# thegedge/StereoReconstruction

Measured on AMD Instinct MI355X. Metric: Mdisparity-hypotheses/s (WxHxD), higher is better.
Workload: dtype f64; 1 GPU; C3: synthetic rectified 1920x1080 pair, 256 depth levels, GeodesicWeight r=5; TwoView WTA both directions + cross-check; one pair per GPU; width=1920, height=1080, depth_levels=256, window_radius=5, weights=geodesic, pairs_per_gpu=1, pair_seed_rank0=1592590339, pair_seed_of_rank_r=seed + 0x10000*r, parallelism=single GPU

## Files before the change

profiles/gpu_busy.py:

```python
#!/usr/bin/env python3
import csv
import sys

rows = list(csv.DictReader(open(sys.argv[1])))
ev = sorted((int(r["Start_Timestamp"]), int(r["End_Timestamp"]), r["Kernel_Name"].split("(")[0][-60:]) for r in rows)
if len(sys.argv) > 4:
    hits = [i for i, e in enumerate(ev) if sys.argv[2] in e[2]]
    ev = ev[hits[int(sys.argv[3]) - 1] + 1: hits[int(sys.argv[4]) - 1] + 1]
t0 = ev[0][0]
span = max(e for _, e, _ in ev) - t0
busy, cur, gaps = 0, t0, []
for s, e, n in ev:
    if s > cur:
        gaps.append((s - cur, n))
    busy += max(0, e - max(s, cur))
    cur = max(cur, e)
print(f"dispatches {len(ev)}  span {span/1e6:.3f} ms  busy {busy/1e6:.3f} ms ({100*busy/span:.1f} %)  "
      f"idle {(span-busy)/1e6:.3f} ms in {len(gaps)} gaps")
for g, n in sorted(gaps, reverse=True)[:10]:
    print(f"  gap {g/1e3:8.1f} us  before {n}")
```

stereoreconstruction_amd/csrc/srh_api.hip:

```cpp
#include "srh_internal.hpp"
#include "srh_geom.hpp"
#include "srh_walk.hpp"

#include <algorithm>
#include <cassert>
#include <cstdarg>
#include <cstdio>
#include <cstdlib>
#include <cstring>
#include <map>
#include <mutex>
#include <string>
#include <utility>
#include <limits>
#include <vector>

using namespace srh;

static thread_local char g_err[512] = "";

static int fail(int code, const char *fmt, ...) {
	va_list ap;
	va_start(ap, fmt);
	vsnprintf(g_err, sizeof(g_err), fmt, ap);
	va_end(ap);
	return code;
}

#define HIP_TRY(expr)                                                                   \
	do {                                                                                \
		hipError_t e_ = (expr);                                                         \
		if (e_ != hipSuccess)                                                           \
			return fail(SRH_E_DEVICE, "%s: %s (%s:%d)", #expr, hipGetErrorString(e_), __FILE__, __LINE__); \
	} while (0)

static thread_local bool g_oom = false;
static thread_local size_t g_alloc_limit = 0;

struct PoolBlock { void *p; size_t bytes; int device; };
static std::mutex g_pool_mu;
static std::vector<PoolBlock> g_pool;
static size_t g_pool_bytes = 0, g_pool_cap = (size_t)65536 << 20;
static const size_t POOL_MIN_BYTES = (size_t)4 << 20;

static void pool_flush(int device) {
	std::vector<PoolBlock> out;
	{
		std::lock_guard<std::mutex> g(g_pool_mu);
		for (size_t k = 0; k < g_pool.size();)
			if (device < 0 || g_pool[k].device == device) { out.push_back(g_pool[k]); g_pool_bytes -= g_pool[k].bytes; g_pool[k] = g_pool.back(); g_pool.pop_back(); }
			else ++k;
	}
	int cur = 0;
	const bool have = hipGetDevice(&cur) == hipSuccess;
	for (const PoolBlock &b : out) { (void)hipSetDevice(b.device); (void)hipFree(b.p); }
	if (have) (void)hipSetDevice(cur);
}
static size_t pool_bytes_on(int device) {
	std::lock_guard<std::mutex> g(g_pool_mu);
	size_t b = 0;
	for (const PoolBlock &k : g_pool) if (k.device == device) b += k.bytes;
	return b;
}
static void pool_give(void *p, size_t bytes) {
	if (!p) return;
	int dev = 0;
	if (bytes >= POOL_MIN_BYTES && hipGetDevice(&dev) == hipSuccess) {
		std::lock_guard<std::mutex> g(g_pool_mu);
		if (g_pool_bytes + bytes <= g_pool_cap) { g_pool.push_back({p, bytes, dev}); g_pool_bytes += bytes; return; }
	}
	(void)hipFree(p);
}
static void *pool_take(size_t bytes, size_t *got) {
	int dev = 0;
	if (bytes < POOL_MIN_BYTES || hipGetDevice(&dev) != hipSuccess) return nullptr;
	std::lock_guard<std::mutex> g(g_pool_mu);
	size_t best = g_pool.size();
	for (size_t k = 0; k < g_pool.size(); ++k)
		if (g_pool[k].device == dev && g_pool[k].bytes >= bytes && g_pool[k].bytes <= bytes + bytes/2 &&
		    (best == g_pool.size() || g_pool[k].bytes < g_pool[best].bytes)) best = k;
	if (best == g_pool.size()) return nullptr;
	void *p = g_pool[best].p;
	*got = g_pool[best].bytes;
	g_pool_bytes -= g_pool[best].bytes;
	g_pool[best] = g_pool.back(); g_pool.pop_back();
	return p;
}

static hipError_t dev_alloc(void **p, size_t bytes, size_t *got) {
	if ((*p = pool_take(bytes, got))) return hipSuccess;
	hipError_t e = hipMalloc(p, bytes);
	if (e == hipErrorOutOfMemory) {
		(void)hipGetLastError();
		int dev = 0;
		if (hipGetDevice(&dev) == hipSuccess && pool_bytes_on(dev)) { pool_flush(dev); e = hipMalloc(p, bytes); }
	}
	if (e != hipSuccess) { *p = nullptr; (void)hipGetLastError(); return e; }
	*got = bytes;
	return hipSuccess;
}

template <class T>
struct DevBuf {
	T *p = nullptr;
	size_t n = 0, block = 0;
	DevBuf() = default;
	DevBuf(DevBuf &&o) noexcept { *this = std::move(o); }
	DevBuf &operator=(DevBuf &&o) noexcept {
		assert(!p && "a held block is released, not overwritten");
		p = o.p; n = o.n; block = o.block;
		o.p = nullptr; o.n = o.block = 0;
		return *this;
	}
	operator T *() const { return p; }
	T *operator->() const { return p; }
	size_t bytes() const { return block; }
	hipError_t alloc(size_t count) {
		void *q = nullptr;
		size_t got = 0;
		const hipError_t e = dev_alloc(&q, count*sizeof(T), &got);
		if (e == hipSuccess) { p = (T *)q; n = got/sizeof(T); block = got; }
		return e;
	}
	int ensure(size_t need) {
		if (n >= need) return SRH_OK;
		if (p) { (void)hipDeviceSynchronize(); release(); }
		if (g_alloc_limit && need*sizeof(T) > g_alloc_limit) {
			g_oom = true;
			return fail(SRH_E_DEVICE, "band buffer of %zu bytes refused (debug_alloc_limit_mb)", need*sizeof(T));
		}
		const hipError_t e = alloc(need);
		if (e == hipErrorOutOfMemory) g_oom = true;
		if (e != hipSuccess) return fail(SRH_E_DEVICE, "hipMalloc of a %zu-byte band buffer: %s", need*sizeof(T), hipGetErrorString(e));
		return SRH_OK;
	}
	void release() { pool_give(p, block); p = nullptr; n = block = 0; }
	void free() { if (p) (void)hipFree(p); p = nullptr; n = block = 0; }
};

struct BandBuffers {
	DevBuf<double> wbuf;
	DevBuf<double> cost;
	DevBuf<double> tnum;
	DevBuf<double> pconst;
	DevBuf<PixRange> prange;
	DevBuf<uint32_t> cflag;
	DevBuf<uint8_t> stpl;
	DevBuf<uint32_t> tileflag;
	DevBuf<int32_t> lcount;
	DevBuf<uint32_t> lcand;
	DevBuf<uint32_t> lrowinfo;
	DevBuf<int32_t> lmeta;
	DevBuf<uint32_t> mvs_wdesc;
	DevBuf<int32_t> mvs_nwin;
	template <class F> void each(F f) {
		f(wbuf); f(cost); f(tnum); f(pconst); f(prange); f(cflag); f(stpl); f(tileflag);
		f(lcount); f(lcand); f(lrowinfo); f(lmeta); f(mvs_wdesc); f(mvs_nwin);
	}
	size_t bytes() { size_t b = 0; each([&](auto &x) { b += x.bytes(); }); return b; }
	void release() { each([](auto &x) { x.release(); }); }
	void free() { each([](auto &x) { x.free(); }); }
};

struct ViewHost {
	int w = 0, h = 0;
	bool present = false;
	DevBuf<uint32_t> rgba;
	DevBuf<uint8_t>  mask;
	DevBuf<double>   gray, gray_tv, depth;
	DevBuf<double>   edges;
	DevBuf<uint8_t>  full;
	int              full_r = 0;
	DevBuf<double>   tvp;   bool tvp_valid = false;
	DevBuf<double>   geo5;  bool geo5_valid = false;
	bool             geo5_denied = false;
	DevBuf<uint8_t>  fullp; int fullp_r = 0;
	DevBuf<uint8_t>  fulls; int fulls_r = 0;
	DevBuf<double>   grayp; bool grayp_valid = false;
	DevBuf<uint8_t>  fullsp; int fullsp_r = 0;
	uint8_t   list_mode[SRH_MAX_VIEWS] = {0};
	DevBuf<uint32_t> act;
	std::vector<uint32_t> act_row, act_host;
	std::vector<uint8_t> hmask;
	bool act_valid = false;
	srh_camera cam;
	DevBuf<int32_t> wta_xy;
	DevBuf<double>  wta_cost;
	int wta_flags = 0, wta_oth = -1;
	DevBuf<double> peaks; int peaks_k = 0;
	DevBuf<double> mrf;
	DevBuf<double> sgm;
};

struct ProfEntry { double ms = 0; int64_t n = 0; };
struct PendingEvt { std::string name; hipEvent_t a, b; };

#ifndef SRH_MVS_SLOTS
#define SRH_MVS_SLOTS 2
#endif
struct MvsSlot {
	hipStream_t stream = nullptr;
	hipEvent_t ev = nullptr, done = nullptr;
	int *h_maxc = nullptr;
	bool own_buffers = false;
	BandBuffers band;
	DevBuf<Counters> d_cnt; DevBuf<int> d_span;
	bool pending = false;
	int view = -1, nneigh = 0, y0 = 0, y1 = 0, cmax = 0;
	int32_t neigh[SRH_MAX_NEIGH] = {0};
	srh_params p;
};

struct srh_context {
	int device = 0;
	hipStream_t own_stream = nullptr;
	hipStream_t stream = nullptr;
	ViewHost views[SRH_MAX_VIEWS];
	DevBuf<ViewDev> d_views;
	DevBuf<int32_t> d_slots;
	int32_t slots_host[SRH_MAX_VIEWS] = {0}; int slots_n = 0;
	DevBuf<Counters> d_cnt;
	DevBuf<int> d_span;
	BandBuffers band;
	hipStream_t mrf_stream[SRH_MAX_VIEWS] = { nullptr };
	void *mrf_host = nullptr;
	DevBuf<double> mrf_peaks;
	DevBuf<double> mrf;
	int mrf_w = 0, mrf_h = 0, mrf_k = 0;
	DevBuf<double> mvsgm;
	int mvsgm_w = 0, mvsgm_h = 0, mvsgm_k = 0;
	double *mvsgm_host = nullptr;
	DevBuf<double> tvmrf;
	DevBuf<double> tvmrf_costs;
	int tvmrf_w = 0, tvmrf_h = 0, tvmrf_l = 0;
	bool tvmrf_own_costs = false;
	DevBuf<double> tvsgm;
	DevBuf<double> tvsgm_costs;
	int tvsgm_w = 0, tvsgm_h = 0, tvsgm_l = 0;
	bool tvsgm_own_costs = false;
	int geodma = 1;
	int tscan_bound = 1;
	int tscan = 1;
	int strip = 1;
	int num_cus = 256;
	bool force_walk = false;
	int list_count_pass = 0;
	int list_cmax_hint = 0;
	int list_smax_hint = 0;
	int mvs_cmax_hint = 0;
	hipStream_t side_stream = nullptr;
	hipEvent_t side_go = nullptr, side_done = nullptr;
	int mvs_async = 1;
	MvsSlot mvs_slot[SRH_MVS_SLOTS];
	int mvs_turn = 0, mvs_last = -1;
	bool in_settle = false;
	int mvs_staged = 1;
	bool list_rows = true;
	void *comm = nullptr; int comm_ranks = 0, comm_rank = 0;
	size_t wbuf_budget = (size_t)32768 << 20;
	size_t budget_cap = 0;
	size_t budget_used = 0;
	size_t mem_limit = 0;
	int debug_trace = 0;
	size_t alloc_limit = 0;
	const volatile int *cancel = nullptr;
	srh_progress_fn progress = nullptr;
	void *user = nullptr;
	bool profiling = false;
	bool force_generic = false;
 	bool use_fused = false;
	int arith = 3;
	struct TvDefer { Counters *host = nullptr; int *span = nullptr; bool queued = false, strip = false, cert = false, lists = false, guessed = false;
	                 int cmax = 0, smax = 0, ref = -1, oth = -1; };
	TvDefer tv_defer[2];
	TvDefer *defer = nullptr;
	struct TvSlot {
		hipStream_t stream = nullptr;
		hipEvent_t go = nullptr, done = nullptr;
		DevBuf<Counters> d_cnt; DevBuf<int> d_span;
		BandBuffers band;
	} tv_slot;
	int tv_overlap = 1;
	int f32_form = 0;
	int rows_masked = 1;
	int side_weights = 1;
	int cert_form = 1;
	bool force_dense = false;
	std::map<std::string, ProfEntry> prof;
	std::vector<PendingEvt> pending;
	srh_stats stats;
	bool last_fused = false;
	int filter_invalid = 0;
	int filter_gap_width = 2;
	int filter_replay = 0;
	int cost_kind = SRH_COST_NCC;
	int sad_dense = 0;
	int wta_outputs = 0;
	DevBuf<double> fuse_result, fuse_scratch;
	FuseCloud fuse_out = { nullptr, nullptr, nullptr, nullptr, nullptr, nullptr };
	int64_t fuse_n = 0;
	bool fuse_valid = false;
};

static bool cancelled(srh_context *c) { return c->cancel && *c->cancel; }
static void progress(srh_context *c, int step, const char *stage) { if (c->progress) c->progress(step, stage, c->user); }

static int drain_profile(srh_context *c) {
	for (auto &p : c->pending) {
		float ms = 0;
		HIP_TRY(hipEventSynchronize(p.b));
		HIP_TRY(hipEventElapsedTime(&ms, p.a, p.b));
		ProfEntry &e = c->prof[p.name];
		e.ms += ms; e.n += 1;
		hipEventDestroy(p.a); hipEventDestroy(p.b);
	}
	c->pending.clear();
	return SRH_OK;
}

struct Scope {
	srh_context *c; PendingEvt p; bool on;
	Scope(srh_context *c_, const char *name) : c(c_), on(c_->profiling) {
		if (on) {
			p.name = name;
			hipEventCreate(&p.a); hipEventCreate(&p.b);
			hipEventRecord(p.a, c->stream);
		}
	}
	~Scope() {
		if (on) {
			hipEventRecord(p.b, c->stream);
			c->pending.push_back(p);
			if (c->pending.size() > 4096) drain_profile(c);
		}
	}
};


static int mvs_settle_all(srh_context *c);
static int check_slot(srh_context *c, int slot, bool must_exist, bool settle = true) {
	if (!c) return fail(SRH_E_INVALID, "null context");
	if (settle) { const int rc = mvs_settle_all(c); if (rc) return rc; }
	if (slot < 0 || slot >= SRH_MAX_VIEWS) return fail(SRH_E_INVALID, "view slot %d out of range [0,%d)", slot, SRH_MAX_VIEWS);
	if (must_exist && !c->views[slot].present) return fail(SRH_E_INVALID, "view slot %d has no image", slot);
	return SRH_OK;
}

static int check_params(const srh_params *p) {
	if (!p) return fail(SRH_E_INVALID, "null params");
	if (p->num_depth_levels < 2) return fail(SRH_E_INVALID, "num_depth_levels %d < 2", p->num_depth_levels);
	if (p->window_radius < 1 || p->window_radius > 15) return fail(SRH_E_INVALID, "window_radius %d outside [1,15]", p->window_radius);
	if (!(p->image_scale > 0)) return fail(SRH_E_INVALID, "image_scale must be > 0");
	if (p->weight_kind != SRH_WEIGHT_ADAPTIVE && p->weight_kind != SRH_WEIGHT_GEODESIC)
		return fail(SRH_E_INVALID, "weight_kind %d unknown", p->weight_kind);
	return SRH_OK;
}

extern "C" int srh_hw_queues_requested(void) {
	const char *s = getenv("GPU_MAX_HW_QUEUES");
	const int n = s ? atoi(s) : 0;
	return n > 0 ? n : 4;
}

extern "C" int srh_abi_version(void) { return SRH_ABI_VERSION; }
extern "C" const char *srh_build_id(void) {
	return
#include "build_id.inc"
	;
}
extern "C" const char *srh_last_error(void) { return g_err; }

extern "C" int srh_device_count(int *count) {
	if (!count) return fail(SRH_E_INVALID, "null count");
	int n = 0;
	hipError_t e = hipGetDeviceCount(&n);
	if (e != hipSuccess) { (void)hipGetLastError(); n = 0; }
	*count = n;
	return SRH_OK;
}

extern "C" void srh_params_twoview_defaults(srh_params *p) {
	memset(p, 0, sizeof(*p));
	p->min_depth = 10; p->max_depth = 100; p->num_depth_levels = 100;
	p->window_radius = 5;
	p->image_scale = 1.0;
	p->weight_kind = SRH_WEIGHT_GEODESIC;
	p->geodesic_iters = 3; p->geodesic_sigma = 50.0; p->geodesic_init = 1000000.0;
	p->adaptive_color_sigma = 10.0;
	p->weight_cutoff = 1e-10;
	p->bad_ret = 1000; p->max_color_diff = 120;
	p->second_best_factor = 0.95; p->wta_margin = 1e-10; p->inconsistency_thresh = 1;
	p->peak_threshold = 0.95;
	p->cross_check_threshold = 1.0;
	p->neighbour_min_dot = 0.2;
	p->top_k = 9; p->num_neighbours = 3;
}

extern "C" void srh_params_mvs_defaults(srh_params *p) {
	srh_params_twoview_defaults(p);
	p->window_radius = 2;
}

extern "C" int srh_cert_bound(const srh_params *p, int mvs, srh_cert_info *out) {
	if (!p || !out) return fail(SRH_E_INVALID, "null argument");
// ... 110 lines not shown
	if (plane_normal) {
		const Vec3 n = normalized(load3(plane_normal));
		c.plane_normal[0] = n.x; c.plane_normal[1] = n.y; c.plane_normal[2] = n.z;
		c.plane_dist = plane_dist;
		c.refr_index = refr_index;
	}
	c.is_refractive = (!near_zero(c.refr_index - 1) && !near_zero(c.plane_dist));
	*out = c;
	return SRH_OK;
}

extern "C" int srh_camera_from_p(const double Pin[12], const double dist[5], const double plane_normal[3],
                                 double plane_dist, double refr_index, srh_camera *out)
{
	if (!Pin || !out) return fail(SRH_E_INVALID, "null argument");
	const double n2 = (Pin[8]*Pin[8] + Pin[9]*Pin[9]) + Pin[10]*Pin[10];
	if (!(n2 > 0)) return fail(SRH_E_INVALID, "projection matrix with a zero third row");
	double P[3][4];
	for (int i = 0; i < 3; ++i) for (int j = 0; j < 4; ++j) P[i][j] = Pin[i*4 + j] / n2;
	double A[3][3], tau[3];
	for (int i = 0; i < 3; ++i) for (int j = 0; j < 3; ++j) A[i][j] = P[2 - j][i];
	for (int k = 0; k < 3; ++k) {
		const double c0 = A[k][k];
		double tailSq = 0;
		for (int i = k + 1; i < 3; ++i) tailSq += A[i][k]*A[i][k];
		double beta;
		if (tailSq <= std::numeric_limits<double>::min()) {
			tau[k] = 0; beta = c0;
			for (int i = k + 1; i < 3; ++i) A[i][k] = 0;
		} else {
			beta = sqrt(c0*c0 + tailSq);
			if (c0 >= 0) beta = -beta;
			for (int i = k + 1; i < 3; ++i) A[i][k] /= (c0 - beta);
			tau[k] = (beta - c0)/beta;
		}
		A[k][k] = beta;
		for (int j = k + 1; j < 3; ++j) {
			double tmp = 0;
			for (int i = k + 1; i < 3; ++i) tmp += A[i][k]*A[i][j];
			tmp += A[k][j];
			A[k][j] -= tau[k]*tmp;
			for (int i = k + 1; i < 3; ++i) A[i][j] -= tau[k]*A[i][k]*tmp;
		}
	}
	double Q[3][3] = {{1, 0, 0}, {0, 1, 0}, {0, 0, 1}};
	for (int k = 2; k >= 0; --k)
		for (int j = k; j < 3; ++j) {
			double tmp = 0;
			for (int i = k + 1; i < 3; ++i) tmp += A[i][k]*Q[i][j];
			tmp += Q[k][j];
			Q[k][j] -= tau[k]*tmp;
			for (int i = k + 1; i < 3; ++i) Q[i][j] -= tau[k]*A[i][k]*tmp;
		}
	double K[9], R[9];
	for (int i = 0; i < 3; ++i)
		for (int j = 0; j < 3; ++j) {
			R[i*3 + j] = Q[j][2 - i];
			K[i*3 + j] = (2 - j <= 2 - i) ? A[2 - j][2 - i] : 0.0;
		}
	for (int axis = 2; axis >= 0; --axis) {
		if (K[axis*3 + axis] < 0) {
			K[axis*3 + axis] = -K[axis*3 + axis];
			for (int j = 0; j < 3; ++j) R[axis*3 + j] = -R[axis*3 + j];
		}
		if (K[axis*3 + 2] < 0) K[axis*3 + 2] = -K[axis*3 + 2];
	}
	srh_camera tmpc;
	const double I3[9] = {1, 0, 0, 0, 1, 0, 0, 0, 1}, z3[3] = {0, 0, 0};
	int rc = srh_camera_from_krt(K, I3, z3, nullptr, nullptr, 0.0, 1.0, &tmpc);
	if (rc) return rc;
	const Vec3 t = matvec(tmpc.Kinv, v3(P[0][3], P[1][3], P[2][3]));
	const double tt[3] = { t.x, t.y, t.z };
	return srh_camera_from_krt(K, R, tt, dist, plane_normal, plane_dist, refr_index, out);
}

extern "C" int srh_mvs_neighbours(int nviews, const srh_camera *cams, const srh_params *p,
                                  int32_t *neigh, int32_t *count)
{
	if (nviews < 0 || !cams || !p || !neigh || !count) return fail(SRH_E_INVALID, "null argument");
	if (p->num_neighbours < 0) return fail(SRH_E_INVALID, "num_neighbours < 0");
	for (int v = 0; v < nviews; ++v) {
		std::vector<std::pair<double, int>> nearViews;
		for (int v2 = 0; v2 < nviews; ++v2) {
			if (v == v2) continue;
			if (fabs(dot(load3(cams[v].pdir), load3(cams[v2].pdir))) > p->neighbour_min_dot) {
				const Vec3 d = load3(cams[v].C) - load3(cams[v2].C);
				nearViews.push_back(std::make_pair(dot(d, d), v2));
			}
		}
		size_t end = nearViews.size();
		if ((size_t)p->num_neighbours < nearViews.size()) {
			std::sort(nearViews.begin(), nearViews.end());
			end = (size_t)p->num_neighbours;
		}
		for (size_t k = 0; k < end; ++k) neigh[(size_t)v*p->num_neighbours + k] = nearViews[k].second;
		count[v] = (int32_t)end;
	}
	return SRH_OK;
}

extern "C" int srh_create(int device, srh_context **out) {
	if (!out) return fail(SRH_E_INVALID, "null out");
	*out = nullptr;
	int n = 0;
	hipError_t e = hipGetDeviceCount(&n);
	if (e != hipSuccess || n <= 0) {
		(void)hipGetLastError();
		return fail(SRH_E_NO_DEVICE, "no HIP device available (%s); this library has no CPU path",
		            e != hipSuccess ? hipGetErrorString(e) : "device count 0");
	}
	if (device < 0 || device >= n) return fail(SRH_E_INVALID, "device ordinal %d outside [0,%d)", device, n);
	HIP_TRY(hipSetDevice(device));
	srh_context *c = new srh_context();
	c->device = device;
	memset(&c->stats, 0, sizeof(c->stats));
	{ int cus = 0; if (hipDeviceGetAttribute(&cus, hipDeviceAttributeMultiprocessorCount, device) == hipSuccess && cus > 0) c->num_cus = cus; }
	hipError_t e2 = hipStreamCreateWithFlags(&c->own_stream, hipStreamNonBlocking);
	if (e2 != hipSuccess) { delete c; return fail(SRH_E_DEVICE, "hipStreamCreate: %s", hipGetErrorString(e2)); }
	c->stream = c->own_stream;
	if (c->d_views.alloc(SRH_MAX_VIEWS) != hipSuccess || c->d_slots.alloc(SRH_MAX_VIEWS) != hipSuccess ||
	    c->d_cnt.alloc(1) != hipSuccess || c->d_span.alloc(4) != hipSuccess) {
		srh_destroy(c);
		return fail(SRH_E_DEVICE, "allocating the context tables failed");
	}
	if (hipMemsetAsync(c->d_views, 0, sizeof(ViewDev)*SRH_MAX_VIEWS, c->stream) != hipSuccess ||
	    hipMemsetAsync(c->d_cnt, 0, sizeof(Counters), c->stream) != hipSuccess ||
	    hipStreamSynchronize(c->stream) != hipSuccess) {
		srh_destroy(c);
		return fail(SRH_E_DEVICE, "initialising the context tables failed");
	}
	*out = c;
	return SRH_OK;
}

static void free_view(ViewHost &v) {
	if (v.rgba || v.gray || v.edges || v.tvp || v.geo5) (void)hipDeviceSynchronize();
	v.rgba.release(); v.mask.release(); v.gray.release(); v.gray_tv.release(); v.depth.release(); v.edges.release();
	v.full.release(); v.fulls.release(); v.grayp.release(); v.fullsp.release(); v.tvp.release(); v.geo5.release(); v.fullp.release(); v.act.release(); v.peaks.release(); v.mrf.release(); v.sgm.release();
	v.wta_xy.release(); v.wta_cost.release();
	v = ViewHost();
}

extern "C" void srh_destroy(srh_context *c) {
	if (!c) return;
	hipSetDevice(c->device);
	if (c->own_stream) hipStreamSynchronize(c->own_stream);
	for (MvsSlot &S : c->mvs_slot) {
		if (S.stream) { hipStreamSynchronize(S.stream); }
		S.pending = false;
	}
	if (c->side_stream) { hipStreamSynchronize(c->side_stream); hipStreamDestroy(c->side_stream); }
	if (c->side_go) hipEventDestroy(c->side_go);
	if (c->side_done) hipEventDestroy(c->side_done);
	drain_profile(c);
	for (MvsSlot &S : c->mvs_slot) {
		if (S.stream) hipStreamDestroy(S.stream);
		if (S.ev) hipEventDestroy(S.ev);
		if (S.done) hipEventDestroy(S.done);
		if (S.h_maxc) hipHostFree(S.h_maxc);
		S.band.release(); S.d_cnt.release(); S.d_span.release();
	}
	for (auto &v : c->views) free_view(v);
	c->d_views.release(); c->d_slots.release(); c->d_cnt.release(); c->d_span.release();
	(void)hipDeviceSynchronize();
	(void)hipStreamSynchronize(c->stream);
	if (c->tv_slot.stream) (void)hipStreamSynchronize(c->tv_slot.stream);
	c->band.release();
	for (auto &d : c->tv_defer) { if (d.host) hipHostFree(d.host); if (d.span) hipHostFree(d.span); }
	{
		srh_context::TvSlot &T = c->tv_slot;
		if (T.stream) { hipStreamSynchronize(T.stream); hipStreamDestroy(T.stream); }
		if (T.go) hipEventDestroy(T.go);
		if (T.done) hipEventDestroy(T.done);
		T.d_cnt.release(); T.d_span.release(); T.band.release();
	}
	c->mrf.release(); c->mrf_peaks.release(); c->mvsgm.release();
	c->tvmrf.release(); c->tvmrf_costs.release();
	c->tvsgm.release(); c->tvsgm_costs.release();
	c->fuse_result.release(); c->fuse_scratch.release();
	for (int i = 0; i < SRH_MAX_VIEWS; ++i) if (c->mrf_stream[i]) hipStreamDestroy(c->mrf_stream[i]);
	if (c->mrf_host) hipHostFree(c->mrf_host);
	if (c->mvsgm_host) hipHostFree(c->mvsgm_host);
	if (c->comm) (void)rccl_comm_destroy(c->comm);
	if (c->own_stream) hipStreamDestroy(c->own_stream);
	delete c;
}

extern "C" int srh_set_stream(srh_context *c, void *hip_stream) {
	if (!c) return fail(SRH_E_INVALID, "null context");
	{ const int rc = mvs_settle_all(c); if (rc) return rc; }
	c->stream = hip_stream ? (hipStream_t)hip_stream : c->own_stream;
	return SRH_OK;
}

extern "C" int srh_set_hooks(srh_context *c, const volatile int *cancel, srh_progress_fn progress_fn, void *user) {
	if (!c) return fail(SRH_E_INVALID, "null context");
	c->cancel = cancel; c->progress = progress_fn; c->user = user;
	return SRH_OK;
}

static void release_band_buffers(srh_context *c);

extern "C" int srh_set_option(srh_context *c, const char *name, long value) {
	if (!c || !name) return fail(SRH_E_INVALID, "null argument");
	{ const int rc = mvs_settle_all(c); if (rc) return rc; }
	if (!strcmp(name, "list_rows")) { c->list_rows = value != 0; return SRH_OK; }
	if (!strcmp(name, "list_count_pass")) { c->list_count_pass = value != 0; return SRH_OK; }
	if (!strcmp(name, "force_generic")) { c->force_generic = value != 0; c->force_walk = value == 2; return SRH_OK; }
	if (!strcmp(name, "fused")) { c->use_fused = value != 0; return SRH_OK; }
	if (!strcmp(name, "arith")) {
		if (value < 0 || value > 3) return fail(SRH_E_INVALID, "arith must be 0 (exact), 1 (fma), 2 (f32) or 3 (certified fma)");
		c->arith = (int)value; return SRH_OK;
	}
	if (!strcmp(name, "force_dense")) { c->force_dense = value != 0; return SRH_OK; }
	if (!strcmp(name, "cert_form")) {
		if (value != 1 && value != 2) return fail(SRH_E_INVALID, "cert_form must be 1 (one-pass) or 2 (two fused sweeps)");
		c->cert_form = (int)value; return SRH_OK;
	}
	if (!strcmp(name, "strip")) {
		if (value != 0 && value != 1 && value != 4 && value != 8) return fail(SRH_E_INVALID, "strip must be 0, 1, 4 or 8");
		c->strip = (int)value; return SRH_OK;
	}
	if (!strcmp(name, "mvs_staged")) { c->mvs_staged = value != 0; return SRH_OK; }
	if (!strcmp(name, "mvs_async")) { c->mvs_async = value != 0; return SRH_OK; }
	if (!strcmp(name, "band_budget_mb")) {
		if (value < 1) return fail(SRH_E_INVALID, "band_budget_mb must be >= 1");
		c->wbuf_budget = (size_t)value << 20;
		c->budget_cap = 0;
		return SRH_OK;
	}
	if (!strcmp(name, "mem_limit_mb")) { c->mem_limit = value > 0 ? (size_t)value << 20 : 0; return SRH_OK; }
	if (!strcmp(name, "debug_trace")) { c->debug_trace = (int)value; return SRH_OK; }
	if (!strcmp(name, "band_pool_mb")) {
		if (value < 0) return fail(SRH_E_INVALID, "band_pool_mb must be >= 0");
		{ std::lock_guard<std::mutex> g(g_pool_mu); g_pool_cap = (size_t)value << 20; }
		if (value == 0) pool_flush(-1);
		return SRH_OK;
	}
	if (!strcmp(name, "debug_alloc_limit_mb")) {
		c->alloc_limit = g_alloc_limit = value > 0 ? (size_t)value << 20 : 0;
		for (MvsSlot &S : c->mvs_slot) if (S.stream) HIP_TRY(hipStreamSynchronize(S.stream));
		if (c->side_stream) HIP_TRY(hipStreamSynchronize(c->side_stream));
		HIP_TRY(hipStreamSynchronize(c->stream));
		release_band_buffers(c);
		return SRH_OK;
	}
	if (!strcmp(name, "tv_overlap")) { c->tv_overlap = value != 0; return SRH_OK; }
	if (!strcmp(name, "filter_invalid")) {
		if (value < 0 || value > 3) return fail(SRH_E_INVALID, "filter_invalid must be 0..3 (SRH_FILTER_GAPS | SRH_FILTER_MEDIAN)");
		c->filter_invalid = (int)value; return SRH_OK;
	}
	if (!strcmp(name, "filter_gap_width")) { c->filter_gap_width = (int)value; return SRH_OK; }
	if (!strcmp(name, "filter_replay")) { c->filter_replay = value != 0; return SRH_OK; }
	if (!strcmp(name, "cost")) {
		if (value != SRH_COST_NCC && value != SRH_COST_SAD) return fail(SRH_E_INVALID, "cost must be 0 (SRH_COST_NCC) or 1 (SRH_COST_SAD)");
		c->cost_kind = (int)value; return SRH_OK;
	}
	if (!strcmp(name, "sad_dense")) { c->sad_dense = value != 0; return SRH_OK; }
	if (!strcmp(name, "wta_outputs")) {
		if (value != 0 && value != SRH_WTA_WINNERS && value != (SRH_WTA_WINNERS | SRH_WTA_COSTS))
			return fail(SRH_E_INVALID, "wta_outputs must be 0, 1 (SRH_WTA_WINNERS) or 3 (SRH_WTA_WINNERS | SRH_WTA_COSTS): the costs are those of the kept winners");
		c->wta_outputs = (int)value; return SRH_OK;
	}
	if (!strcmp(name, "tscan")) { c->tscan = value != 0; return SRH_OK; }
	if (!strcmp(name, "tscan_bound")) { c->tscan_bound = value != 0; return SRH_OK; }
	if (!strcmp(name, "geodma")) { c->geodma = value != 0; return SRH_OK; }
	if (!strcmp(name, "f32_form")) { c->f32_form = value != 0; return SRH_OK; }
	if (!strcmp(name, "rows_masked")) { c->rows_masked = (int)value; return SRH_OK; }
	if (!strcmp(name, "side_weights")) { c->side_weights = value != 0; return SRH_OK; }
	if (!strcmp(name, "debug_mvs_cmax_hint")) { c->mvs_cmax_hint = value > 0 ? (int)((value + 7) & ~7L) : 0; return SRH_OK; }
#ifdef SRH_EXPERIMENT
	if (!strcmp(name, "exp_repeat")) { exp_set((int)value, -1); return SRH_OK; }
	if (!strcmp(name, "exp_lds_pad")) { exp_set(-1, (int)value); return SRH_OK; }
	if (!strcmp(name, "exp_scan_mode")) { exp_set_scan((int)value); return SRH_OK; }
	if (!strcmp(name, "exp_walk_mode")) { exp_set_walk((int)value); return SRH_OK; }
	if (!strcmp(name, "exp_rows_mode")) { exp_set_rows((int)value); return SRH_OK; }
#endif
	return fail(SRH_E_INVALID, "unknown option '%s'", name);
}

extern "C" int srh_synchronize(srh_context *c) {
	if (!c) return fail(SRH_E_INVALID, "null context");
	HIP_TRY(hipSetDevice(c->device));
	{ const int rc = mvs_settle_all(c); if (rc) return rc; }
	HIP_TRY(hipStreamSynchronize(c->stream));
	return SRH_OK;
}

static int view_install(srh_context *c, int slot, int w, int h, const void *rgba, const void *mask, const uint8_t *hmask,
                        hipMemcpyKind kind, const srh_camera *cam)
{
	if (w <= 0 || h <= 0 || (size_t)w*h > ((size_t)1 << 30)) return fail(SRH_E_INVALID, "bad image size %dx%d", w, h);
	if (!rgba || !cam) return fail(SRH_E_INVALID, "null rgba / camera");
	if (w > SRH_MAX_VIEW_DIM || h > SRH_MAX_VIEW_DIM) return fail(SRH_E_UNSUPPORTED, "view of %dx%d: a side above %d (SRH_MAX_VIEW_DIM)", w, h, SRH_MAX_VIEW_DIM);
	HIP_TRY(hipSetDevice(c->device));
	ViewHost &v = c->views[slot];
	const size_t n = (size_t)w*h;
	if (!v.present || v.w != w || v.h != h) {
		HIP_TRY(hipStreamSynchronize(c->stream));
		free_view(v);
		HIP_TRY(v.rgba.alloc(n));
		HIP_TRY(v.mask.alloc(n));
		HIP_TRY(v.gray.alloc(n));
		HIP_TRY(v.gray_tv.alloc(n));
		HIP_TRY(v.depth.alloc(n));
		HIP_TRY(v.edges.alloc(4*n));
// ... 215 lines not shown
	if (!dev_ptr) return fail(SRH_E_INVALID, "null output");
	*dev_ptr = c->views[slot].depth;
	return SRH_OK;
}

static int check_wta_outputs(srh_context *c, int slot, bool costs) {
	const ViewHost &v = c->views[slot];
	if (!v.wta_flags) return fail(SRH_E_INVALID, "view slot %d holds no WTA outputs (option \"wta_outputs\" off, no WTA pass since the upload, or its depth map came from the MRF stage)", slot);
	if (costs && !(v.wta_flags & SRH_WTA_COSTS)) return fail(SRH_E_INVALID, "view slot %d kept the winners only (wta_outputs = 1): no cost planes", slot);
	return SRH_OK;
}

extern "C" int srh_view_wta_outputs_state(srh_context *c, int slot, int *flags, int *oth_slot) {
	int rc = check_slot(c, slot, true); if (rc) return rc;
	const ViewHost &v = c->views[slot];
	if (flags) *flags = v.wta_flags;
	if (oth_slot) *oth_slot = v.wta_flags ? v.wta_oth : -1;
	return SRH_OK;
}

extern "C" int srh_view_wta_outputs_device(srh_context *c, int slot, void **win_xy, void **runner_xy, void **min_cost, void **second_cost) {
	int rc = check_slot(c, slot, true); if (rc) return rc;
	if ((rc = check_wta_outputs(c, slot, min_cost || second_cost))) return rc;
	const ViewHost &v = c->views[slot];
	const size_t n = (size_t)v.w*v.h;
	if (win_xy) *win_xy = v.wta_xy;
	if (runner_xy) *runner_xy = v.wta_xy + 2*n;
	if (min_cost) *min_cost = v.wta_cost;
	if (second_cost) *second_cost = v.wta_cost + n;
	return SRH_OK;
}

extern "C" int srh_view_wta_outputs(srh_context *c, int slot, int32_t *win_xy, int32_t *runner_xy, double *min_cost, double *second_cost) {
	int rc = check_slot(c, slot, true); if (rc) return rc;
	if ((rc = check_wta_outputs(c, slot, min_cost || second_cost))) return rc;
	HIP_TRY(hipSetDevice(c->device));
	const ViewHost &v = c->views[slot];
	const size_t n = (size_t)v.w*v.h;
	if (win_xy) HIP_TRY(hipMemcpyAsync(win_xy, v.wta_xy, 2*n*sizeof(int32_t), hipMemcpyDeviceToHost, c->stream));
	if (runner_xy) HIP_TRY(hipMemcpyAsync(runner_xy, v.wta_xy + 2*n, 2*n*sizeof(int32_t), hipMemcpyDeviceToHost, c->stream));
	if (min_cost) HIP_TRY(hipMemcpyAsync(min_cost, v.wta_cost, n*sizeof(double), hipMemcpyDeviceToHost, c->stream));
	if (second_cost) HIP_TRY(hipMemcpyAsync(second_cost, v.wta_cost + n, n*sizeof(double), hipMemcpyDeviceToHost, c->stream));
	HIP_TRY(hipStreamSynchronize(c->stream));
	return SRH_OK;
}

extern "C" int srh_view_depth_copy_to_device(srh_context *c, int slot, void *dst_dev, size_t dst_bytes) {
	int rc = check_slot(c, slot, true); if (rc) return rc;
	if (!dst_dev) return fail(SRH_E_INVALID, "null destination");
	HIP_TRY(hipSetDevice(c->device));
	const ViewHost &v = c->views[slot];
	if (dst_bytes < (size_t)v.w*v.h*sizeof(double))
		return fail(SRH_E_INVALID, "destination of %zu bytes is smaller than the %dx%d depth map of slot %d", dst_bytes, v.w, v.h, slot);
	HIP_TRY(hipMemcpyAsync(dst_dev, v.depth, (size_t)v.w*v.h*sizeof(double), hipMemcpyDeviceToDevice, c->stream));
	return SRH_OK;
}

extern "C" int srh_view_depth_copy_from_device(srh_context *c, int slot, const void *src_dev, size_t src_bytes) {
	int rc = check_slot(c, slot, true); if (rc) return rc;
	if (!src_dev) return fail(SRH_E_INVALID, "null source");
	HIP_TRY(hipSetDevice(c->device));
	const ViewHost &v = c->views[slot];
	if (src_bytes < (size_t)v.w*v.h*sizeof(double))
		return fail(SRH_E_INVALID, "source of %zu bytes is smaller than the %dx%d depth map of slot %d", src_bytes, v.w, v.h, slot);
	HIP_TRY(hipMemcpyAsync(v.depth, src_dev, (size_t)v.w*v.h*sizeof(double), hipMemcpyDeviceToDevice, c->stream));
	return SRH_OK;
}

static size_t held_band_bytes(srh_context *c) {
	size_t b = c->band.bytes() + c->tv_slot.band.bytes();
	for (MvsSlot &S : c->mvs_slot) b += S.band.bytes();
	for (const ViewHost &v : c->views) b += v.geo5.bytes();
	return b;
}

static size_t band_budget(srh_context *c) {
	size_t b = c->wbuf_budget;
	if (c->budget_cap && b > c->budget_cap) b = c->budget_cap;
	size_t free_b = 0, total_b = 0;
	if (hipMemGetInfo(&free_b, &total_b) == hipSuccess) {
		size_t avail = free_b + held_band_bytes(c) + pool_bytes_on(c->device);
		if (c->mem_limit && avail > c->mem_limit) avail = c->mem_limit;
		if (b > avail/4) b = avail/4;
	} else (void)hipGetLastError();
	if (b < ((size_t)1 << 20)) b = (size_t)1 << 20;
	c->budget_used = b;
	return b;
}

static void release_band_buffers(srh_context *c) {
	pool_flush(c->device);
	c->band.free();
	for (MvsSlot &S : c->mvs_slot) S.band.free();
	c->tv_slot.band.free();
	for (ViewHost &v : c->views)
		if (v.geo5) { v.geo5.free(); v.geo5_valid = false; v.geo5_denied = true; }
}

template <class F>
static int with_thinner_bands(srh_context *c, F body) {
	for (;;) {
		g_oom = false;
		g_alloc_limit = c->alloc_limit;
		const int rc = body();
		if (rc != SRH_E_DEVICE || !g_oom) return rc;
		g_oom = false;
		const size_t used = c->budget_used;
		if (used <= ((size_t)1 << 20)) return rc;
		for (MvsSlot &S : c->mvs_slot) if (S.stream) (void)hipStreamSynchronize(S.stream);
		if (c->side_stream) (void)hipStreamSynchronize(c->side_stream);
		(void)hipStreamSynchronize(c->stream);
		if (c->tv_slot.stream) (void)hipStreamSynchronize(c->tv_slot.stream);
		release_band_buffers(c);
		c->budget_cap = used/2;
		c->stats.band_retries += 1;
	}
}

static int band_rows(srh_context *c, int W, int H, int T) {
	size_t rows = band_budget(c) / ((size_t)T*sizeof(double)*(size_t)W);
	if (rows < 1) rows = 1;
	if (rows > (size_t)H) rows = H;
	return (int)rows;
}

static int read_back(srh_context *c, void *host, const void *dev, size_t bytes) {
	HIP_TRY(hipMemcpyAsync(host, dev, bytes, hipMemcpyDeviceToHost, c->stream));
	HIP_TRY(hipStreamSynchronize(c->stream));
	return SRH_OK;
}

static int fetch_counters(srh_context *c, int used_dense) {
	Counters h;
	int rc;
	if ((rc = read_back(c, &h, c->d_cnt, sizeof(h)))) return rc;
	c->stats.n_pixels = (int64_t)h.n_pixels;
	c->stats.n_eval = (int64_t)h.n_eval;
	c->stats.n_eval_device = (int64_t)h.n_eval_device;
	c->stats.scan_tiles_template = (int64_t)h.scan_tiles_template;
	c->stats.scan_tiles_walked = (int64_t)h.scan_tiles_walked;
	c->stats.scan_tiles_bound = (int64_t)h.scan_tiles_bound;
	c->stats.mvs_waves_staged = (int64_t)h.mvs_waves_staged;
	c->stats.mvs_waves_listed = (int64_t)h.mvs_waves_listed;
	c->stats.used_dense_path = used_dense;
	c->stats.used_fused_kernel = c->last_fused ? 1 : 0;
#ifdef SRH_PROFILE_PHASES
	{
		unsigned long long g[8];
		geodesic_phases_fetch(g);
		if (g[7])
			fprintf(stderr, "[srh prof] geodesic kernel: %llu waves, cycles per wave: staging %.0f  sweeps %.0f  exp %.0f  rows out %.0f  pconst: first sweep %.0f  second sweep %.0f  rest %.0f\n",
			        g[7], (double)g[0]/g[7], (double)g[1]/g[7], (double)g[2]/g[7], (double)g[4]/g[7], (double)g[5]/g[7], (double)g[6]/g[7], (double)g[3]/g[7]);
	}
	if (h.dbg_waves && h.dbg_blocks && h.dbg_phase[3] && h.strip_ticket) {
		const double nw = (double)h.dbg_waves, nt = (double)h.dbg_blocks/nw;
		fprintf(stderr, "[srh dbg] strip: waves %llu, tiles/wave %.1f (%.1f with phase 2), cycles/wave %.0f | per tile: ticket %.0f  own requests %.0f  barriers %.0f  setup %.0f  "
		        "block loops %.0f  p2 lists %.0f  p2 blocks %.0f  p2 singles %.0f\n", h.dbg_waves, nt, (double)h.dbg_cycles/nw, (double)h.dbg_total_cycles/nw,
		        h.dbg_phase[0]/nw/nt, h.dbg_phase[1]/nw/nt, h.dbg_phase[2]/nw/nt, h.dbg_phase[3]/nw/nt, h.dbg_phase[4]/nw/nt,
		        h.dbg_phase[5]/nw/nt, h.dbg_phase[6]/nw/nt, h.dbg_phase[7]/nw/nt);
		static const char *names[8] = { "ticket", "own requests", "barriers", "setup", "block loops", "p2 lists", "p2 blocks", "p2 singles" };
		const int nwv = h.dbg_wave[8*4 + 4] ? 8 : 4;
		for (int k = 0; k < 8; ++k) {
			fprintf(stderr, "[srh dbg]   %-13s by wave:", names[k]);
			for (int w = 0; w < nwv; ++w) fprintf(stderr, " %8.0f", h.dbg_wave[8*k + w]/((double)h.dbg_blocks/nwv));
			fprintf(stderr, "\n");
		}
	} else
	if (h.dbg_waves && !c->last_fused)
		fprintf(stderr, "[srh dbg] dense: waves %llu, cycles/wave %.0f, fast blocks/wave %.1f, cycles/fast block %.0f\n",
		        h.dbg_waves, (double)h.dbg_total_cycles/h.dbg_waves, (double)h.dbg_blocks/h.dbg_waves,
		        h.dbg_blocks ? (double)h.dbg_cycles/h.dbg_blocks : 0.0);
	if (h.dbg_waves && !c->last_fused && !h.strip_ticket)
		fprintf(stderr, "[srh dbg] phases/wave: stage_w %.0f prologue %.0f sync %.0f stage_rt %.0f compute %.0f tail %.0f\n",
		        (double)h.dbg_phase[0]/h.dbg_waves, (double)h.dbg_phase[1]/h.dbg_waves, (double)h.dbg_phase[2]/h.dbg_waves,
		        (double)h.dbg_phase[3]/h.dbg_waves, (double)h.dbg_phase[4]/h.dbg_waves, (double)h.dbg_phase[5]/h.dbg_waves);
	if (h.dbg_waves && c->last_fused)
		fprintf(stderr, "[srh dbg] fused: %llu tiles, %llu with select-form work, %llu pixels with an unusable tap of their own\n",
		        h.dbg_waves, h.n_listed, h.n_slots);
	if (h.dbg_waves && c->last_fused)
		fprintf(stderr, "[srh dbg] fused, role wave cycles/tile: A geometry %.0f  B accept %.0f  C stage %.0f  D prologue %.0f  E1 blocks %.0f  E2 general %.0f  F wta %.0f  barriers %.0f | other waves: blocks %.0f barriers %.0f total %.0f\n",
		        (double)h.dbg_phase[0]/h.dbg_waves, (double)h.dbg_phase[1]/h.dbg_waves, (double)h.dbg_phase[2]/h.dbg_waves,
		        (double)h.dbg_phase[3]/h.dbg_waves, (double)h.dbg_phase[4]/h.dbg_waves, (double)h.dbg_phase[5]/h.dbg_waves,
		        (double)h.dbg_phase[6]/h.dbg_waves, (double)h.dbg_phase[7]/h.dbg_waves,
		        (double)h.dbg_cycles/(3.0*h.dbg_waves), (double)h.dbg_blocks/(3.0*h.dbg_waves), (double)h.dbg_total_cycles/(3.0*h.dbg_waves));
	if (h.dbg_phase[6] && !c->last_fused)
		fprintf(stderr, "[srh dbg] rows: tasks %llu fast %llu, rows/pixel %.2f, slots/px %.1f, wave iterations %llu all-fast %llu\n",
		        h.dbg_phase[6], h.dbg_phase[7], (double)h.dbg_cycles/(double)h.n_pixels, 8.0*h.dbg_phase[6]/(double)h.n_pixels,
		        h.dbg_blocks, h.dbg_total_cycles);
	if (h.dbg_phase[6] && !c->last_fused && h.dbg_wave[8])
		fprintf(stderr, "[srh dbg] rows cost kernel, wave tiles %llu: cycles per tile: staging %.0f  constants %.0f  phase 1 %.0f  p2 blocks %.0f  p2 singles %.0f | tiles with blocks %llu (%llu blocks: %.0f cycles per such tile), with singles %llu (%llu singles: %.0f cycles per such tile); rounds if the tile's tasks were dealt to its 64 lanes: %.2f per tile\n",
		        h.dbg_wave[8], (double)h.dbg_wave[0]/h.dbg_wave[8], (double)h.dbg_wave[1]/h.dbg_wave[8], (double)h.dbg_wave[2]/h.dbg_wave[8],
		        (double)h.dbg_wave[3]/h.dbg_wave[8], (double)h.dbg_wave[4]/h.dbg_wave[8], h.dbg_wave[9], h.dbg_wave[10],
		        h.dbg_wave[9] ? (double)h.dbg_wave[3]/h.dbg_wave[9] : 0.0, h.dbg_wave[11], h.dbg_wave[12], h.dbg_wave[11] ? (double)h.dbg_wave[4]/h.dbg_wave[11] : 0.0, (double)h.dbg_wave[13]/h.dbg_wave[8]);
#endif
	return SRH_OK;
}

static void run_weights(srh_context *c, int ref, int W, const srh_params &p, int by, int nr, size_t wstride,
                        double *pconst = nullptr, bool wimg = false) {
	if (p.weight_kind == SRH_WEIGHT_GEODESIC && !c->force_generic && wimg && c->geodma && p.window_radius == 5 && !c->views[ref].geo5_denied) {
		ViewHost &v = c->views[ref];
		bool ok = true;
		if (!v.geo5) {
			if (v.geo5.alloc(geo5_doubles(v.w, v.h)) != hipSuccess) ok = false;
			v.geo5_valid = false;
		}
		if (ok && !v.geo5_valid) {
			Scope s(c, "geo5_planes_kernel");
			launch_geo5_planes(c->stream, v.edges, v.gray_tv, v.mask, v.w, v.h, v.geo5);
			v.geo5_valid = true;
		}
		if (ok) {
			Scope s(c, "geodesic_dma_kernel");
			if (launch_geodesic_dma(c->stream, c->d_views, ref, W, v.geo5, p, by, nr, c->band.wbuf, pconst, c->num_cus)) return;
		}
	}
	if (p.weight_kind == SRH_WEIGHT_GEODESIC && !c->force_generic) {
		Scope s(c, "geodesic_reg_kernel");
		if (launch_geodesic_reg(c->stream, c->d_views, ref, W, c->views[ref].edges, p, by, nr, c->band.wbuf, wstride, pconst, wimg)) return;
	}
	if (p.weight_kind == SRH_WEIGHT_ADAPTIVE && !c->force_generic) {
		Scope s(c, "adaptive_reg_kernel");
		if (launch_adaptive_reg(c->stream, c->d_views, ref, W, p, by, nr, c->band.wbuf, wstride, pconst, wimg)) return;
	}
	Scope s(c, "weights_kernel");
	launch_weights(c->stream, c->d_views, ref, W, p, by, nr, c->band.wbuf, wstride, pconst, wimg);
}

static bool rig_is_row_aligned(const srh_camera &a, const srh_camera &b, double *fx_bx) {
	if (a.is_distorted || b.is_distorted || a.is_refractive || b.is_refractive) return false;
	for (int k = 0; k < 9; ++k) if (fabs(a.R[k] - b.R[k]) > 1e-13) return false;
	for (int k = 3; k < 9; ++k) if (fabs(a.K[k] - b.K[k]) > 1e-9*(1.0 + fabs(a.K[k]))) return false;
	if (fabs(a.K[1]) > 1e-12 || fabs(b.K[1]) > 1e-12 || fabs(a.K[3]) > 1e-12 || fabs(a.K[6]) > 1e-12 || fabs(a.K[7]) > 1e-12)
		return false;
	const Vec3 d = load3(b.C) - load3(a.C);
	const Vec3 bc = matvec(a.R, d);
	const double len = norm(bc);
	if (!(len > 0) || fabs(bc.y) > 1e-12*len || fabs(bc.z) > 1e-12*len) return false;
	*fx_bx = fabs(b.K[0]*bc.x);
	return true;
}

static int ensure_wta_planes(srh_context *c, int ref, int oth) {
	ViewHost &v = c->views[ref];
	if (!c->wta_outputs) { v.wta_flags = 0; return SRH_OK; }
	const size_t n = (size_t)v.w*v.h;
	if (v.wta_flags == c->wta_outputs && v.wta_oth == oth) return SRH_OK;
	if (!v.wta_xy) HIP_TRY(v.wta_xy.alloc(4*n));
	if ((c->wta_outputs & SRH_WTA_COSTS) && !v.wta_cost) HIP_TRY(v.wta_cost.alloc(2*n));
	HIP_TRY(hipMemsetAsync(v.wta_xy, 0xff, 4*n*sizeof(int32_t), c->stream));
	if (c->wta_outputs & SRH_WTA_COSTS) launch_fill(c->stream, v.wta_cost, 2*n, __builtin_inf());
	v.wta_flags = c->wta_outputs; v.wta_oth = oth;
	return SRH_OK;
}

static void estimate_list_capacity(const srh_camera &rc, const srh_camera &oc, int W, int H, int OW, int OH,
                                   const srh_params &p, int y0, int y1, int &cmax, int &smax, bool mvs = false)
{
	(void)H;
	const int D = p.num_depth_levels, NL = D < 9 ? D : 9, GX = 13, GY = 9;
	const Vec3 normal = load3(rc.pdir);
	long best_len = 0, best_rows = 0;
	for (int gy = 0; gy < GY; ++gy)
		for (int gx = 0; gx < GX; ++gx) {
			const int x = (int)((gx*(long)(W - 1))/(GX - 1)), y = y0 + (int)((gy*(long)(y1 - y0 - 1))/(GY - 1));
			const Ray ray = cam_unproject(rc, (x + 0.5)/p.image_scale, (y + 0.5)/p.image_scale);
			long len = 0, rows = 0;
			bool have = false;
			int px = 0, py = 0;
			for (int k = 0; k < NL; ++k) {
				const int d = NL > 1 ? (int)(((long)k*(D - 1))/(NL - 1)) : 0;
				Vec3 point = load3(rc.C);
				if (!point_from_depth(ray, normal, depth_from_label(p, mvs, d), point)) continue;
				if (!cam_project(oc, point)) continue;
				const double cxd = fmin(fmax(point.x*p.image_scale, -64.0), (double)OW + 64.0);
				const double cyd = fmin(fmax(point.y*p.image_scale, -64.0), (double)OH + 64.0);
				if (!(cxd == cxd) || !(cyd == cyd)) continue;
				const int ix = (int)cxd, iy = (int)cyd;
				if (have) {
					const long dx = labs((long)ix - px), dy = labs((long)iy - py);
					len += dx > dy ? dx : dy;
					rows += dy;
				}
				have = true; px = ix; py = iy;
			}
			if (len > best_len) best_len = len;
			if (rows > best_rows) best_rows = rows;
		}
	if (best_rows > SRH_ROWS_NR) best_rows = SRH_ROWS_NR;
	long cm = best_len + best_len/8 + (mvs ? 0 : (best_len < D - 1 ? best_len : D - 1)) + 40;
	if (cm > 65520) cm = 65520;
	cmax = (int)((cm + 7) & ~7L);
	long sm = cmax + 8*(best_rows + 2) + 32;
	if (sm > 65528) sm = 65528;
	smax = (int)((sm + 7) & ~7L);
}

static int ensure_tvp(srh_context *c, ViewHost &v) {
	if (!v.tvp) HIP_TRY(v.tvp.alloc(padded_size(v.w, v.h)));
	if (!v.tvp_valid) {
		Scope s(c, "padded_plane_kernel");
		launch_padded_plane(c->stream, v.gray_tv, v.w, v.h, v.tvp);
		v.tvp_valid = true;
	}
	return SRH_OK;
}

static int ensure_fulls(srh_context *c, ViewHost &v, int R) {
	if (v.fulls_r == R) return SRH_OK;
	if (!v.fulls) HIP_TRY(v.fulls.alloc((size_t)v.w*v.h));
	Scope s(c, "sad_full_window_kernel");
	launch_sad_full_window(c->stream, v.mask, v.w, v.h, R, v.fulls);
	v.fulls_r = R;
	v.fullsp_r = 0;
	return SRH_OK;
}

static int ensure_full(srh_context *c, ViewHost &v, int R) {
	if (v.full_r == R) return SRH_OK;
	Scope s(c, "full_window_kernel");
	uint32_t *stat = (uint32_t *)(v.full + full_stat_offset((size_t)v.w*v.h));
	HIP_TRY(hipMemsetAsync(stat, 0, 2*sizeof(uint32_t), c->stream));
	launch_full_window(c->stream, v.gray_tv, v.w, v.h, R, v.full, stat);
	v.full_r = R;
	return SRH_OK;
}

static int ensure_sad_planes(srh_context *c, ViewHost &v, int R) {
	int rc;
	if ((rc = ensure_tvp(c, v))) return rc;
	if (!v.grayp) HIP_TRY(v.grayp.alloc(padded_size(v.w, v.h)));
	if (!v.grayp_valid) {
		Scope s(c, "padded_gray_kernel");
		launch_padded_gray(c->stream, v.gray, v.mask, v.w, v.h, v.grayp);
		v.grayp_valid = true;
	}
	if ((rc = ensure_fulls(c, v, R))) return rc;
	if (!v.fullsp) HIP_TRY(v.fullsp.alloc(padded_size(v.w, v.h)));
	if (v.fullsp_r != R) {
		Scope s(c, "padded_bytes_kernel");
		launch_padded_bytes(c->stream, v.fulls, v.w, v.h, v.fullsp);
		v.fullsp_r = R;
	}
	return SRH_OK;
}


struct TvPlan { bool dense = false; int cstride = 0; bool fused = false; };
struct TvLists { int cmax = 0, smax = 0; bool rows_mode = false, guessed = false, cert = false; size_t lrows = 0; };
struct TvDense { int cstride = 0; bool strip = false, cert = false, tscan = false; size_t rows = 0; int lanes = 8; };

struct TvPass {
	srh_context *c = nullptr;
	int ref = 0, oth = 0;
	const srh_params *p = nullptr;
	int W = 0, H = 0, y0 = 0, y1 = 0, R = 0, T = 0;
	size_t budget = 0;
	bool sad = false;
	int32_t *wout = nullptr;

	size_t rows_per_band(size_t bytes) const;
	void winner_costs(int by, int nr, bool wimg_layout) const;
	TvPlan plan() const;
	int run_fused(bool &stands) const;
	int lists_prepare(TvLists &S) const;
	int lists_rows_band(const TvLists &S, int by, int nr) const;
	int lists_pass(TvLists &S) const;
	int run_lists(bool cert_ok, srh_context::TvDefer *defer) const;
	int dense_prepare(TvDense &D) const;
	void dense_band_inputs(const TvDense &D, int by, int nr) const;
	int dense_cost_pass(const TvDense &D, int by, int nr, int arith, bool raw) const;
	int run_dense(TvDense &D) const;
	int run_walk() const;
};

static int tv_pass_init(TvPass &P, srh_context *c, int ref, int oth, const srh_params *p, int y0, int y1) {
	if (ref == oth) return fail(SRH_E_INVALID, "ref and other view are the same slot");
	const ViewHost &L = c->views[ref], &Rv = c->views[oth];
	if (L.w != Rv.w || L.h != Rv.h)
		return fail(SRH_E_INVALID, "TwoViewStereo needs equal-sized views (%dx%d vs %dx%d; twoviewstereo.cpp:116-119)",
		            L.w, L.h, Rv.w, Rv.h);
	HIP_TRY(hipSetDevice(c->device));
	P.c = c; P.ref = ref; P.oth = oth; P.p = p;
	P.W = L.w; P.H = L.h;
	P.y0 = y0 < 0 ? 0 : y0;
	P.y1 = (y1 <= 0 || y1 > P.H) ? P.H : y1;
	P.R = p->window_radius;
	P.T = (2*P.R + 1)*(2*P.R + 1);
	P.sad = c->cost_kind == SRH_COST_SAD;
	if (P.y1 > P.y0) P.budget = band_budget(c);
	return SRH_OK;
}

size_t TvPass::rows_per_band(size_t bytes) const {
	return std::min(std::max<size_t>(budget/(bytes*(size_t)W), 1), (size_t)(y1 - y0));
}

void TvPass::winner_costs(int by, int nr, bool wimg_layout) const {
	if (!wout || !(c->wta_outputs & SRH_WTA_COSTS)) return;
	Scope s(c, "twoview_winner_costs_kernel");
	double *mc = c->views[ref].wta_cost;
	launch_twoview_winner_costs(c->stream, c->d_views, ref, oth, W, *p, sad, by, nr, c->band.wbuf, wimg_layout,
	                            wout, mc, mc + (size_t)W*H);
}

static int redo_capacity(size_t band_pixels) { return (int)std::min<size_t>(band_pixels, (size_t)1 << 30); }

static double disparity_span(const srh_params &p, double fx_bx) {
	return fx_bx*p.image_scale*fabs(1.0/p.min_depth - 1.0/p.max_depth);
}

TvPlan TvPass::plan() const {
	const ViewHost &L = c->views[ref], &Rv = c->views[oth];
	TvPlan pl;
	pl.dense = !c->force_generic && (!sad || c->sad_dense) && (R == 5 || R == 2);
	double fx_bx = 0;
	if (pl.dense && !rig_is_row_aligned(L.cam, Rv.cam, &fx_bx)) {
		const bool pinhole = !L.cam.is_distorted && !Rv.cam.is_distorted && !L.cam.is_refractive && !Rv.cam.is_refractive;
		if (c->force_dense && pinhole) fx_bx = (double)(W + 8)/disparity_span(*p, 1.0);
		else pl.dense = false;
	}
	if (!pl.dense) return pl;
	const double span = disparity_span(*p, fx_bx);
	if (!(p->min_depth > 0) || !(p->max_depth > 0) || !(span < 4096.0)) pl.dense = false;
	else pl.cstride = (((int)ceil(span) + 3) + 7) & ~7;
	if (pl.cstride > W + 8) pl.cstride = (W + 8 + 7) & ~7;
	if (sad && pl.dense && pl.cstride + SRH_WTILE > strip_chunk_columns()) pl.dense = false;
	pl.fused = pl.dense && !sad && c->use_fused && (c->arith == 0 || c->arith == 3) &&
	           p->num_depth_levels <= SRH_FUSED_MAXC && span + 1.0 <= (double)SRH_FUSED_MAXC;
	return pl;
}

int TvPass::run_fused(bool &stands) const {
	int rc;
	stands = false;
	HIP_TRY(hipMemsetAsync(c->d_cnt, 0, sizeof(Counters), c->stream));
	if ((rc = c->band.tnum.ensure((size_t)p->num_depth_levels))) return rc;
	{ Scope s(c, "pinhole_label_table_kernel");
	  launch_pinhole_label_table(c->stream, c->d_views, ref, *p, false, c->band.tnum); }
	const int rows = (int)rows_per_band((size_t)T*sizeof(double));
	if ((rc = c->band.wbuf.ensure(wbuf_doubles(W, rows, T)))) return rc;
	bool launched = true;
	for (int by = y0; by < y1 && launched; by += rows) {
		if (cancelled(c)) return fail(SRH_E_CANCELLED, "cancelled");
		const int nr = std::min(rows, y1 - by);
		run_weights(c, ref, W, *p, by, nr, SRH_WTILE);
		Scope s(c, "twoview_fused_kernel");
		launched = launch_twoview_fused(c->stream, c->d_views, ref, oth, W, *p, by, nr, c->band.wbuf, c->band.tnum, c->d_cnt, wout);
		if (launched) winner_costs(by, nr, false);
	}
	HIP_TRY(hipGetLastError());
	if (!launched) return SRH_OK;
	Counters hc;
	if ((rc = read_back(c, &hc, c->d_cnt, sizeof(hc)))) return rc;
	stands = hc.not_row_aligned == 0;
	return SRH_OK;
}


static bool tv_lists_fit(const int *mx, int cmax, int smax) {
	return mx[0] <= cmax && ((mx[1] + 7) & ~7) <= smax && mx[2] == 0;
}

static void tv_learn_lists(srh_context *c, int ref, int oth, bool guessed, int cmax, int smax, const int *mx, const Counters &h) {
	const int cm = guessed ? std::max(8, (mx[0] + 7) & ~7) : cmax;
	const int sm = guessed ? std::max(cm + 64, (mx[1] + 7) & ~7) : smax;
	if (cm > c->list_cmax_hint) c->list_cmax_hint = cm;
	if (sm > c->list_smax_hint) c->list_smax_hint = sm;
	c->views[ref].list_mode[oth] = (h.n_slots > 2.2*(double)h.n_listed) ? 2 : 1;
}

static int tv_defer_queue(srh_context *c, srh_context::TvDefer &d, bool lists, bool strip, bool cert) {
	HIP_TRY(hipMemcpyAsync(d.host, c->d_cnt, sizeof(Counters), hipMemcpyDeviceToHost, c->stream));
	if (lists) HIP_TRY(hipMemcpyAsync(d.span, c->d_span, 4*sizeof(int), hipMemcpyDeviceToHost, c->stream));
	d.queued = true; d.lists = lists; d.strip = strip; d.cert = cert;
	return SRH_OK;
}

int TvPass::lists_prepare(TvLists &S) const {
	int rc;
	if ((rc = c->band.lcount.ensure((size_t)(y1 - y0)*W))) return rc;
	ViewHost &O = c->views[oth];
	if ((rc = sad ? ensure_fulls(c, O, R) : ensure_full(c, O, R))) return rc;
	if ((rc = c->band.tnum.ensure((size_t)p->num_depth_levels))) return rc;
	{ Scope s(c, "label_plane_table_kernel");
	  launch_label_plane_table(c->stream, c->d_views, ref, *p, false, c->band.tnum); }
	int smax_guess = 0;
	S.cmax = c->list_cmax_hint;
	if (S.cmax <= 0 && c->list_count_pass) {
		HIP_TRY(hipMemsetAsync(c->d_span, 0, sizeof(int), c->stream));
		{ Scope s(c, "twoview_count_kernel");
		  launch_twoview_count(c->stream, c->d_views, ref, oth, W, *p, y0, y1 - y0, c->band.lcount, c->d_cnt, c->d_span, c->band.tnum); }
		int maxc = 0;
		if ((rc = read_back(c, &maxc, c->d_span, sizeof(int)))) return rc;
		S.cmax = std::max(8, (maxc + 7) & ~7);
	} else if (S.cmax <= 0) {
		estimate_list_capacity(c->views[ref].cam, O.cam, W, H, O.w, O.h, *p, y0, y1, S.cmax, smax_guess);
		S.guessed = true;
	}
	S.rows_mode = c->list_rows && W < 32768 && H < 32768;
	if (c->views[ref].list_mode[oth] == 2) S.rows_mode = false;
	S.smax = c->list_smax_hint > 0 ? c->list_smax_hint : (S.guessed ? smax_guess : S.cmax + 64);
	return SRH_OK;
}

int TvPass::lists_rows_band(const TvLists &S, int by, int nr) const {
	ViewHost &O = c->views[oth];
	int32_t *cnt_band = c->band.lcount + (size_t)(by - y0)*W;
	double *pconst = sad ? nullptr : (double *)c->band.pconst;
	if (!c->side_stream) {
		HIP_TRY(hipStreamCreateWithFlags(&c->side_stream, hipStreamNonBlocking));
		HIP_TRY(hipEventCreateWithFlags(&c->side_go, hipEventDisableTiming));
		HIP_TRY(hipEventCreateWithFlags(&c->side_done, hipEventDisableTiming));
	}
	HIP_TRY(hipEventRecord(c->side_go, c->stream));
	{ Scope s(c, "twoview_rows_list_kernel");
	  launch_twoview_rows_list(c->stream, c->d_views, ref, oth, W, *p, by, nr, c->band.lcand, S.cmax,
	                           cnt_band, c->band.lrowinfo, c->band.lmeta, S.smax, c->d_cnt, c->d_span, c->band.tnum); }
	if (c->side_weights) {
		HIP_TRY(hipStreamWaitEvent(c->side_stream, c->side_go, 0));
		std::swap(c->stream, c->side_stream);
		run_weights(c, ref, W, *p, by, nr, SRH_WTILE, pconst, true);
		std::swap(c->stream, c->side_stream);
		HIP_TRY(hipEventRecord(c->side_done, c->side_stream));
		HIP_TRY(hipStreamWaitEvent(c->stream, c->side_done, 0));
	} else run_weights(c, ref, W, *p, by, nr, SRH_WTILE, pconst, true);
	if (S.cert) HIP_TRY(hipMemsetAsync(c->band.cflag, 0, sizeof(uint32_t), c->stream));
	HIP_TRY(hipMemsetAsync(&c->d_cnt->strip_ticket, 0, 2*sizeof(unsigned int), c->stream));
	if (sad) {
		Scope s(c, "twoview_rows_sad_kernel");
		launch_twoview_rows_sad(c->stream, c->d_views, ref, oth, W, *p, by, nr, c->band.wbuf, O.fulls,
		                        c->band.lrowinfo, c->band.lmeta, c->band.cost, S.smax, c->d_cnt);
	} else {
		Scope s(c, "twoview_rows_cost_kernel");
		launch_twoview_rows_cost(c->stream, c->d_views, ref, oth, W, *p, by, nr, c->band.wbuf, O.full,
		                         c->band.lrowinfo, c->band.lmeta, c->band.cost, S.smax, c->d_cnt, S.cert ? (c->cert_form == 1 ? 5 : 3) : 0,
		                         pconst, S.cert && c->rows_masked ? O.tvp : nullptr, c->num_cus,
		                         c->rows_masked == 1 ? (const uint32_t *)(O.full + full_stat_offset((size_t)O.w*O.h)) : nullptr);
	}
	{ Scope s(c, "twoview_rows_scan_kernel");
	  launch_twoview_rows_scan(c->stream, c->d_views, ref, oth, W, *p, by, nr, cnt_band, c->band.lcand, S.cmax,
	                           c->band.lrowinfo, c->band.lmeta, c->band.cost, S.smax, S.cert ? c->band.cflag : nullptr, -1, c->d_cnt, wout); }
	if (S.cert) {
		const int cap = redo_capacity((size_t)nr*W);
		{ Scope s(c, "twoview_rows_refill_kernel");
		  launch_twoview_rows_refill(c->stream, W, O.w, *p, by, c->band.cflag, cap, c->band.wbuf, c->views[ref].tvp, O.tvp,
		                             c->band.lrowinfo, c->band.lmeta, c->band.cost, S.smax, c->d_cnt); }
		Scope s(c, "twoview_rows_rescan_kernel");
		launch_twoview_rows_scan(c->stream, c->d_views, ref, oth, W, *p, by, nr, cnt_band, c->band.lcand, S.cmax,
		                         c->band.lrowinfo, c->band.lmeta, c->band.cost, S.smax, c->band.cflag, cap, c->d_cnt, wout);
	}
	winner_costs(by, nr, true);
	return SRH_OK;
}

int TvPass::lists_pass(TvLists &S) const {
	int rc;
	HIP_TRY(hipMemsetAsync(c->d_cnt, 0, sizeof(Counters), c->stream));
	HIP_TRY(hipMemsetAsync(c->d_span, 0, 4*sizeof(int), c->stream));
	const bool rows_mode = S.rows_mode;
	const int ccap = rows_mode ? S.smax : S.cmax;
	const size_t per_px = (size_t)(rows_mode ? (2*R + 1)*wimg_wp(R) : T)*sizeof(double) + (size_t)ccap*sizeof(double) + (size_t)S.cmax*sizeof(uint32_t)
	                      + (rows_mode ? (SRH_ROWS_NR + 1)*sizeof(uint32_t) : 0);
	const size_t lrows = S.lrows = rows_per_band(per_px);
	if ((rc = c->band.wbuf.ensure(rows_mode ? wimg_doubles(W, (int)lrows, R) : wbuf_doubles(W, (int)lrows, T)))) return rc;
	const size_t px64 = (lrows*W + 63) & ~(size_t)63, px32 = lrows*(size_t)((W + 7)/8)*8;
	if ((rc = c->band.cost.ensure((rows_mode ? px32 : lrows*W)*(size_t)ccap))) return rc;
	if ((rc = c->band.lcand.ensure((rows_mode ? px64 : lrows*W)*(size_t)S.cmax))) return rc;
	if (rows_mode && !sad && (rc = c->band.pconst.ensure((lrows*(size_t)W + SRH_WTILE)*SRH_PC))) return rc;
	if (rows_mode) {
		if ((rc = c->band.lrowinfo.ensure(px64*(size_t)SRH_ROWS_NR))) return rc;
		if ((rc = c->band.lmeta.ensure(lrows*W))) return rc;
		if (S.cert && (rc = c->band.cflag.ensure(lrows*W + 1))) return rc;
		if (S.cert && ((rc = ensure_tvp(c, c->views[ref])) || (rc = ensure_tvp(c, c->views[oth])))) return rc;
	}
	for (int by = y0; by < y1; by += (int)lrows) {
		if (cancelled(c)) return fail(SRH_E_CANCELLED, "cancelled");
		const int nr = std::min((int)lrows, y1 - by);
		if (rows_mode) {
			if ((rc = lists_rows_band(S, by, nr))) return rc;
			continue;
		}
			int32_t *cnt_band = c->band.lcount + (size_t)(by - y0)*W;
			run_weights(c, ref, W, *p, by, nr, SRH_WTILE);
			{ Scope s(c, "twoview_list_kernel");
			  launch_twoview_list(c->stream, c->d_views, ref, oth, W, *p, by, nr, c->band.lcand, S.cmax,
			                      cnt_band, c->d_cnt, c->d_span, c->band.tnum); }
			if (sad) {
				Scope s(c, "twoview_list_sad_kernel");
				launch_twoview_list_sad(c->stream, c->d_views, ref, oth, W, *p, by, nr, c->band.wbuf,
				                        cnt_band, c->band.lcand, c->band.cost, S.cmax, c->d_cnt);
			} else {
				Scope s(c, "twoview_list_cost_kernel");
				launch_twoview_list_cost(c->stream, c->d_views, ref, oth, W, *p, by, nr, c->band.wbuf, c->views[oth].full,
				                         cnt_band, c->band.lcand, c->band.cost, S.cmax, c->d_cnt);
			}
			{ Scope s(c, "twoview_list_scan_kernel");
			  launch_twoview_list_scan(c->stream, c->d_views, ref, oth, W, *p, by, nr, cnt_band, c->band.lcand, c->band.cost, S.cmax, wout); }
			winner_costs(by, nr, false);
	}
	return SRH_OK;
}

int TvPass::run_lists(bool cert_ok, srh_context::TvDefer *defer) const {
	int rc;
	TvLists S;
	if ((rc = lists_prepare(S))) return rc;
	for (int pass = 0; pass < 6; ++pass) {
		S.cert = S.rows_mode && cert_ok;
		if ((rc = lists_pass(S))) return rc;
		if (defer && pass == 0 && S.rows_mode &&
		    ((c->list_cmax_hint > 0 && c->list_smax_hint > 0 && c->views[ref].list_mode[oth] == 1) ||
		     (S.guessed && c->views[ref].list_mode[oth] == 0))) {
			if ((rc = tv_defer_queue(c, *defer, true, false, S.cert))) return rc;
			defer->cmax = S.cmax; defer->smax = S.smax;
			defer->guessed = S.guessed; defer->ref = ref; defer->oth = oth;
			if (c->debug_trace) fprintf(stderr, "[srh trace] lists %d>%d queued unverified: cmax %d smax %d guessed %d\n", ref, oth, S.cmax, S.smax, (int)S.guessed);
			c->stats.used_strip_kernel = 0;
			c->stats.used_dense_path = 0;
			HIP_TRY(hipGetLastError());
			return SRH_OK;
		}
		int mx[4] = { 0, 0, 0, 0 };
		if ((rc = read_back(c, mx, c->d_span, sizeof(mx)))) return rc;
		const int maxc = mx[0];
		if (c->debug_trace) fprintf(stderr, "[srh trace] lists %d>%d verified pass %d: cmax %d smax %d guessed %d -> longest list %d, slots %d, rows over %d\n",
		                            ref, oth, pass, S.cmax, S.smax, (int)S.guessed, mx[0], mx[1], mx[2]);
		if (S.rows_mode) {
			const int need = (mx[1] + 7) & ~7;
			if (mx[2] || need > 65528) {
				S.rows_mode = false; c->views[ref].list_mode[oth] = 2;
				if (maxc > S.cmax) S.cmax = (maxc + 7) & ~7;
				continue;
			}
			if (tv_lists_fit(mx, S.cmax, S.smax)) {
				Counters hc;
				if ((rc = read_back(c, &hc, c->d_cnt, sizeof(hc)))) return rc;
				tv_learn_lists(c, ref, oth, S.guessed, S.cmax, S.smax, mx, hc);
				if (hc.cert_overflow != 0) { cert_ok = false; continue; }
				if (S.cert) { c->stats.n_certified = (int64_t)hc.n_pixels; c->stats.n_flagged = (int64_t)hc.n_flagged; }
				break;
			}
			if (maxc > S.cmax) { S.cmax = (maxc + 7) & ~7; if (need <= S.smax) S.smax = std::max(S.smax, S.cmax + 64); }
			if (need > S.smax) S.smax = need;
			S.guessed = false;
			continue;
		}
		if (maxc <= S.cmax) {
			const int cm = S.guessed ? std::max(8, (maxc + 7) & ~7) : S.cmax;
			if (cm > c->list_cmax_hint) c->list_cmax_hint = cm;
			break;
		}
		S.cmax = (maxc + 7) & ~7;
		S.guessed = false;
	}
	HIP_TRY(hipGetLastError());
	return SRH_OK;
}


int TvPass::dense_prepare(TvDense &D) const {
	int rc;
	D.tscan = c->tscan != 0;
	if ((rc = c->band.tnum.ensure((size_t)p->num_depth_levels + 8))) return rc;
	{ Scope s(c, "pinhole_label_table_kernel");
	  launch_pinhole_label_table(c->stream, c->d_views, ref, *p, false, c->band.tnum); }
	if (D.tscan) {
		if ((rc = c->band.stpl.ensure(scan_template_bytes()))) return rc;
		Scope s(c, "twoview_template_kernel");
		launch_scan_template(c->stream, c->d_views, ref, oth, *p, y0, y1 - y0, c->band.tnum, c->band.stpl);
	}
	for (int pass = 0; pass < 2; ++pass) {
		const int wdoubles = D.strip ? (2*R + 1)*wimg_wp(R) : T;
		D.rows = rows_per_band((size_t)wdoubles*sizeof(double) + (size_t)D.cstride*sizeof(double));
		if (D.strip && !sad && c->strip == 1 && (size_t)((W + SRH_WTILE - 1)/SRH_WTILE)*D.rows < (size_t)48*2*c->num_cus) D.strip = false;
		else break;
	}
	const size_t rows = D.rows;
	if ((rc = c->band.wbuf.ensure(D.strip ? wimg_doubles(W, (int)rows, R) : wbuf_doubles(W, (int)rows, T)))) return rc;
	if ((rc = c->band.cost.ensure(rows*(size_t)((W + 31)/32)*32*(size_t)D.cstride))) return rc;
	if ((rc = c->band.pconst.ensure((rows*(size_t)W + SRH_WTILE)*SRH_PC))) return rc;
	if ((rc = c->band.prange.ensure(rows*(size_t)W + SRH_WTILE))) return rc;
	if (D.tscan && (rc = c->band.tileflag.ensure(rows*(size_t)((W + 63)/64) + 1))) return rc;
	if (D.cert && (rc = c->band.cflag.ensure(rows*(size_t)W + 1))) return rc;
	D.lanes = D.strip ? strip_block_lanes(D.cstride, c->strip == 1 ? 0 : c->strip) : 8;
	if ((rc = ensure_tvp(c, c->views[ref])) || (rc = ensure_tvp(c, c->views[oth]))) return rc;
	if (D.strip && sad) {
		if ((rc = ensure_sad_planes(c, c->views[oth], R))) return rc;
	} else if (D.strip) {
		ViewHost &O = c->views[oth];
		if (!O.fullp) HIP_TRY(O.fullp.alloc(padded_size(O.w, O.h)));
		if (O.fullp_r != R) {
			Scope s(c, "padded_full_kernel");
			launch_padded_full(c->stream, O.gray_tv, O.w, O.h, R, O.fullp);
			O.fullp_r = R;
		}
	}
	return SRH_OK;
}

void TvPass::dense_band_inputs(const TvDense &D, int by, int nr) const {
	run_weights(c, ref, W, *p, by, nr, SRH_WTILE, !sad ? (double *)c->band.pconst : nullptr, D.strip);
	Scope s(c, "pixel_range_kernel");
	launch_pixel_range(c->stream, c->d_views, ref, oth, W, *p, by, nr, c->band.tnum, D.cstride, c->band.prange);
}

int TvPass::dense_cost_pass(const TvDense &D, int by, int nr, int arith, bool raw) const {
	const int cstride = D.cstride;
	const size_t wstride = SRH_WTILE;
	if (sad) {
		HIP_TRY(hipMemsetAsync(&c->d_cnt->strip_ticket, 0, 2*sizeof(unsigned int), c->stream));
		Scope s(c, "twoview_strip_sad_kernel");
		if (!launch_twoview_strip_sad(c->stream, W, H, *p, by, nr, c->band.wbuf, c->band.prange, c->views[ref].tvp,
		                              c->views[oth].grayp, c->views[oth].fullsp, c->band.cost, cstride, c->d_cnt, c->num_cus))
			return fail(SRH_E_UNSUPPORTED, "twoview_strip_sad_kernel: no instantiation for radius %d", R);
		return SRH_OK;
	}
	if (D.strip) {
		HIP_TRY(hipMemsetAsync(&c->d_cnt->strip_ticket, 0, 2*sizeof(unsigned int), c->stream));
		{ Scope s(c, "twoview_strip_cost_kernel");
		  launch_twoview_strip_cost(c->stream, c->d_views, ref, oth, W, H, *p, by, nr, c->band.wbuf, c->band.pconst, c->band.prange,
		                            c->views[ref].tvp, c->views[oth].tvp, c->views[oth].fullp, c->band.cost, cstride,
		                            c->d_cnt, arith, c->num_cus, D.lanes, raw); }
	} else {
		{ Scope s(c, "twoview_dense_cost_kernel");
		  if (arith == 2)
			launch_twoview_dense_cost_f32(c->stream, c->d_views, ref, oth, W, *p, by, nr, c->band.wbuf, wstride,
			                              c->band.tnum, c->band.cost, cstride, c->d_cnt, c->band.pconst, c->f32_form);
		  else
			launch_twoview_dense_cost(c->stream, c->d_views, ref, oth, W, *p, by, nr, c->band.wbuf, wstride,
			                          c->band.tnum, c->band.cost, cstride, c->d_cnt, c->band.pconst, arith, c->band.prange); }
	}
	Scope s(c, "twoview_lazy_fill_kernel");
	launch_twoview_lazy_fill(c->stream, c->d_views, ref, oth, W, *p, by, nr, c->band.prange, c->band.wbuf, wstride, c->views[ref].tvp,
	                         c->views[oth].tvp, D.strip, D.lanes, D.strip ? D.lanes == 8 : arith != 5, c->band.cost, cstride, c->d_cnt);
	return SRH_OK;
}

int TvPass::run_dense(TvDense &D) const {
	int rc;
	if ((rc = dense_prepare(D))) return rc;
	const int cost_arith = c->arith == 3 ? (D.cert ? (c->cert_form == 1 ? 5 : 3) : 0) : c->arith;
	for (int by = y0; by < y1; by += (int)D.rows) {
		if (cancelled(c)) return fail(SRH_E_CANCELLED, "cancelled");
		const int nr = std::min((int)D.rows, y1 - by);
		dense_band_inputs(D, by, nr);
		if (D.cert) HIP_TRY(hipMemsetAsync(c->band.cflag, 0, sizeof(uint32_t), c->stream));
		if ((rc = dense_cost_pass(D, by, nr, cost_arith, false))) return rc;
		{ Scope s(c, "twoview_scan_kernel");
		  launch_twoview_scan(c->stream, c->d_views, ref, oth, W, *p, by, nr, c->band.tnum, c->band.cost, D.cstride, c->d_cnt, c->band.prange,
		                      D.cert ? c->band.cflag : nullptr, -1, D.cert && D.strip ? c->band.pconst : nullptr, D.tscan ? c->band.stpl : nullptr, c->band.tileflag, c->num_cus, wout, c->tscan_bound); }
		if (D.cert) {
			const int cap = redo_capacity((size_t)nr*W);
			{ Scope s(c, "twoview_refill_kernel");
			  launch_twoview_refill(c->stream, W, *p, by, c->band.prange, c->band.cflag, cap, c->band.wbuf, D.strip, c->views[ref].tvp,
			                        c->views[oth].tvp, c->band.cost, D.cstride, c->d_cnt); }
			Scope s(c, "twoview_rescan_kernel");
			launch_twoview_scan(c->stream, c->d_views, ref, oth, W, *p, by, nr, c->band.tnum, c->band.cost, D.cstride, c->d_cnt, c->band.prange,
			                    c->band.cflag, cap, nullptr, nullptr, nullptr, c->num_cus, wout);
		}
		winner_costs(by, nr, D.strip);
	}
	HIP_TRY(hipGetLastError());
	return SRH_OK;
}

enum TvVerdict { TV_STANDS, TV_STRIP_OVERFLOW, TV_CERT_OVERFLOW, TV_NOT_ROW_ALIGNED };
static TvVerdict tv_dense_verdict(const Counters &h, bool strip) {
	if (strip && h.strip_overflow != 0) return TV_STRIP_OVERFLOW;
	if (h.cert_overflow != 0) return TV_CERT_OVERFLOW;
	return h.not_row_aligned == 0 ? TV_STANDS : TV_NOT_ROW_ALIGNED;
}

int TvPass::run_walk() const {
	int rc;
	const int rows = (int)rows_per_band((size_t)T*sizeof(double));
	if ((rc = c->band.wbuf.ensure(wbuf_doubles(W, rows, T)))) return rc;
	for (int by = y0; by < y1; by += rows) {
		if (cancelled(c)) return fail(SRH_E_CANCELLED, "cancelled");
		const int nr = std::min(rows, y1 - by);
		run_weights(c, ref, W, *p, by, nr, SRH_WTILE);
		{ Scope s(c, "twoview_generic_kernel");
		  launch_twoview_generic(c->stream, c->d_views, ref, oth, W, *p, by, nr, c->band.wbuf, SRH_WTILE, c->d_cnt, sad, wout); }
		winner_costs(by, nr, false);
	}
	HIP_TRY(hipGetLastError());
	return SRH_OK;
}

static int twoview_wta_run(srh_context *c, int ref, int oth, const srh_params *p, int y0, int y1) {
	int rc;
	TvPass P;
	if ((rc = tv_pass_init(P, c, ref, oth, p, y0, y1))) return rc;
	if (P.y1 <= P.y0) return SRH_OK;
	if ((rc = ensure_wta_planes(c, ref, oth))) return rc;
	P.wout = c->wta_outputs ? (int32_t *)c->views[ref].wta_xy : nullptr;
	const TvPlan plan = P.plan();

	c->last_fused = false;
	if (plan.fused) {
		bool stands = false;
		if ((rc = P.run_fused(stands))) return rc;
		if (stands) {
			c->stats.used_dense_path = 1;
			c->last_fused = true;
			return SRH_OK;
		}
	}

	bool dense = plan.dense;
	TvDense D;
	D.cstride = plan.cstride;
	D.strip = dense && (P.sad || (c->strip != 0 && c->arith != 2)) && plan.cstride + SRH_WTILE <= strip_chunk_columns();
	bool cert_ok = c->arith == 3 && !P.sad && cert_bound(*p).ok != 0;
	c->stats.n_certified = c->stats.n_flagged = 0;
	const bool lists = !c->force_walk && P.R <= 5 && P.W < 65536 && P.H < 65536 && p->wta_margin >= 0;
	for (int attempt = 0; attempt < 4; ++attempt) {
		HIP_TRY(hipMemsetAsync(c->d_cnt, 0, sizeof(Counters), c->stream));
		srh_context::TvDefer *defer = attempt == 0 ? c->defer : nullptr;
		if (!dense) {
			if ((rc = lists ? P.run_lists(cert_ok, defer) : P.run_walk())) return rc;
			if (lists && defer && defer->queued) return SRH_OK;
			break;
		}
		D.cert = cert_ok;
		if ((rc = P.run_dense(D))) return rc;
		if (defer) {
			if ((rc = tv_defer_queue(c, *defer, false, D.strip, cert_ok))) return rc;
			c->stats.used_strip_kernel = D.strip ? 1 : 0;
			c->stats.used_dense_path = 1;
			return SRH_OK;
		}
		Counters hc;
		if ((rc = read_back(c, &hc, c->d_cnt, sizeof(hc)))) return rc;
		const TvVerdict v = tv_dense_verdict(hc, D.strip);
		if (v == TV_STRIP_OVERFLOW) { D.strip = false; if (P.sad) dense = false; continue; }
		if (v == TV_CERT_OVERFLOW) { cert_ok = false; continue; }
		c->stats.n_certified = (int64_t)hc.n_certified; c->stats.n_flagged = (int64_t)hc.n_flagged;
		if (v == TV_STANDS) break;
		dense = false;
		D.strip = false;
	}
	c->stats.used_strip_kernel = D.strip ? 1 : 0;
	c->stats.used_dense_path = dense ? 1 : 0;
	return SRH_OK;
}

extern "C" int srh_twoview_wta(srh_context *c, int ref, int oth, const srh_params *p, int y0, int y1) {
	int rc;
	if ((rc = check_slot(c, ref, true)) || (rc = check_slot(c, oth, true)) || (rc = check_params(p))) return rc;
	return with_thinner_bands(c, [&] { return twoview_wta_run(c, ref, oth, p, y0, y1); });
}

extern "C" int srh_twoview_cost_rows(srh_context *c, int ref, int oth, const srh_params *p, int y0, int y1, int form, int raw,
                                     double *cost_out, size_t cost_doubles, int32_t *range_out, int *cstride_out, int *used_strip)
{
	int rc;
	if ((rc = check_slot(c, ref, true)) || (rc = check_slot(c, oth, true)) || (rc = check_params(p))) return rc;
	if (form != 0 && form != 3 && form != 5 && form != 1) return fail(SRH_E_INVALID, "form must be 0, 1, 3 or 5");
	if ((form == 3 || form == 5) && !cert_bound(*p).ok) return fail(SRH_E_UNSUPPORTED, "the parameters leave the error bound no room");
	const bool sad = c->cost_kind == SRH_COST_SAD;
	if (sad && !c->sad_dense) return fail(SRH_E_UNSUPPORTED, "cost rows of cost_sad exist on the dense plan only (option sad_dense)");
	if (sad && form != 0) return fail(SRH_E_INVALID, "cost_sad has the reference's arithmetic only: form must be 0");
	TvPass P;
	if ((rc = tv_pass_init(P, c, ref, oth, p, y0, y1))) return rc;
	const TvPlan plan = P.plan();
	if (P.y1 <= P.y0 || !plan.dense)
		return fail(SRH_E_UNSUPPORTED, "cost rows exist on the row-aligned dense plan only (radius 5 or 2, rectified pinhole pair)");
	c->last_fused = false;
	c->stats.n_certified = c->stats.n_flagged = 0;
	HIP_TRY(hipMemsetAsync(c->d_cnt, 0, sizeof(Counters), c->stream));
	TvDense D;
	D.cstride = plan.cstride;
	D.strip = (sad || c->strip != 0) && plan.cstride + SRH_WTILE <= strip_chunk_columns();
	D.cert = form != 0 && !sad && cert_bound(*p).ok != 0;
	if ((rc = P.dense_prepare(D))) return rc;
	if (cancelled(c)) return fail(SRH_E_CANCELLED, "cancelled");
	const int nr = std::min((int)D.rows, P.y1 - P.y0);
	P.dense_band_inputs(D, P.y0, nr);
	if (nr != P.y1 - P.y0) return fail(SRH_E_UNSUPPORTED, "cost rows: the rows asked for do not fit one band (%d of %d)", nr, P.y1 - P.y0);
	if (cost_out) {
		const size_t nd = (size_t)nr*((P.W + 31)/32)*32*(size_t)D.cstride;
		if (cost_doubles < nd) return fail(SRH_E_INVALID, "cost rows: buffer of %zu doubles, %zu needed", cost_doubles, nd);
		HIP_TRY(hipMemsetAsync(c->band.cost, 0xff, nd*sizeof(double), c->stream));
		if ((rc = P.dense_cost_pass(D, P.y0, nr, form, raw != 0))) return rc;
		HIP_TRY(hipMemcpyAsync(cost_out, c->band.cost, nd*sizeof(double), hipMemcpyDeviceToHost, c->stream));
		if (range_out) HIP_TRY(hipMemcpyAsync(range_out, c->band.prange, (size_t)nr*P.W*sizeof(PixRange), hipMemcpyDeviceToHost, c->stream));
		HIP_TRY(hipStreamSynchronize(c->stream));
	}
	if (cstride_out) *cstride_out = D.cstride;
	if (used_strip) *used_strip = D.strip ? 1 : 0;
	return SRH_OK;
}

extern "C" int srh_twoview_pair_costs(srh_context *c, int ref, int oth, const srh_params *p, int kind, int n,
                                      const int32_t *xy, double *out)
{
	int rc;
	if ((rc = check_slot(c, ref, true)) || (rc = check_slot(c, oth, true)) || (rc = check_params(p))) return rc;
	if (kind != SRH_COST_NCC && kind != SRH_COST_SAD) return fail(SRH_E_INVALID, "kind must be SRH_COST_NCC or SRH_COST_SAD");
	if (n < 0 || (n > 0 && (!xy || !out))) return fail(SRH_E_INVALID, "null pairs or output");
	if (p->window_radius > 5) return fail(SRH_E_UNSUPPORTED, "pair costs take window radii up to 5");
	if (n == 0) return SRH_OK;
	const ViewHost &L = c->views[ref];
	for (int k = 0; k < n; ++k)
		if (xy[4*k] < 0 || xy[4*k + 1] < 0 || xy[4*k] >= L.w || xy[4*k + 1] >= L.h)
			return fail(SRH_E_INVALID, "pair %d: reference pixel (%d, %d) outside the %dx%d view", k, xy[4*k], xy[4*k + 1], L.w, L.h);
	HIP_TRY(hipSetDevice(c->device));
	DevBuf<int32_t> dxy; DevBuf<double> dout;
	HIP_TRY(dxy.alloc((size_t)4*n));
	HIP_TRY(dout.alloc((size_t)n));
	HIP_TRY(hipMemcpyAsync(dxy, xy, (size_t)4*n*sizeof(int32_t), hipMemcpyHostToDevice, c->stream));
	{ Scope s(c, "pair_costs_kernel");
	  launch_pair_costs(c->stream, c->d_views, ref, oth, *p, kind == SRH_COST_SAD, n, dxy, dout); }
	HIP_TRY(hipGetLastError());
	HIP_TRY(hipMemcpyAsync(out, dout, (size_t)n*sizeof(double), hipMemcpyDeviceToHost, c->stream));
	HIP_TRY(hipStreamSynchronize(c->stream));
	dxy.free(); dout.free();
	return SRH_OK;
}

extern "C" int srh_debug_exp(srh_context *c, const double *x, int n, double *kernel_out, double *library_out) {
	if (!c || !x || !kernel_out || !library_out || n < 1) return fail(SRH_E_INVALID, "null argument");
	HIP_TRY(hipSetDevice(c->device));
	DevBuf<double> d;
	HIP_TRY(d.alloc((size_t)n*3));
	hipError_t e = hipMemcpyAsync(d, x, (size_t)n*sizeof(double), hipMemcpyHostToDevice, c->stream);
	if (e == hipSuccess) {
		launch_geo_exp_probe(c->stream, d, n, d + n, d + 2*(size_t)n);
		e = hipMemcpyAsync(kernel_out, d + n, (size_t)n*sizeof(double), hipMemcpyDeviceToHost, c->stream);
	}
	if (e == hipSuccess) e = hipMemcpyAsync(library_out, d + 2*(size_t)n, (size_t)n*sizeof(double), hipMemcpyDeviceToHost, c->stream);
	if (e == hipSuccess) e = hipStreamSynchronize(c->stream);
	d.free();
	if (e != hipSuccess) return fail(SRH_E_DEVICE, "srh_debug_exp: %s", hipGetErrorString(e));
	return SRH_OK;
}

extern "C" int srh_twoview_cross_check(srh_context *c, int left, int right, const srh_params *p) {
	int rc;
	if ((rc = check_slot(c, left, true)) || (rc = check_slot(c, right, true)) || (rc = check_params(p))) return rc;
	const ViewHost &L = c->views[left], &Rv = c->views[right];
	if (L.w != Rv.w || L.h != Rv.h) return fail(SRH_E_INVALID, "TwoViewStereo needs equal-sized views");
	HIP_TRY(hipSetDevice(c->device));
	{ Scope s(c, "twoview_cross_check_kernel"); launch_twoview_cross_check(c->stream, c->d_views, left, right, L.w, L.h, *p); }
	{ Scope s(c, "twoview_cross_check_kernel"); launch_twoview_cross_check(c->stream, c->d_views, right, left, L.w, L.h, *p); }
	HIP_TRY(hipGetLastError());
	return SRH_OK;
}

static void tv_slot_swap(srh_context *c) {
	srh_context::TvSlot &T = c->tv_slot;
	std::swap(c->stream, T.stream);
	std::swap(c->band, T.band);
	std::swap(c->d_cnt, T.d_cnt); std::swap(c->d_span, T.d_span);
}

static bool tv_pass_stands(const srh_context::TvDefer &d) {
	const Counters &h = *d.host;
	if (d.lists) return tv_lists_fit(d.span, d.cmax, d.smax) && h.cert_overflow == 0;
	return tv_dense_verdict(h, d.strip) == TV_STANDS;
}

static int twoview_filter(srh_context *c, int left, int right, const srh_params *p);

extern "C" int srh_twoview_compute(srh_context *c, int left, int right, const srh_params *p,
                                   double *left_out, double *right_out)
{
	int rc;
	if ((rc = check_slot(c, left, true)) || (rc = check_slot(c, right, true)) || (rc = check_params(p))) return rc;
	HIP_TRY(hipSetDevice(c->device));
	for (auto &d : c->tv_defer) {
		if (!d.host) HIP_TRY(hipHostMalloc((void **)&d.host, sizeof(Counters)));
		if (!d.span) HIP_TRY(hipHostMalloc((void **)&d.span, 4*sizeof(int)));
		d.queued = false; d.lists = false; d.guessed = false;
	}
	if (c->tv_overlap) {
		srh_context::TvSlot &T = c->tv_slot;
		if (!T.stream) {
			HIP_TRY(hipStreamCreateWithFlags(&T.stream, hipStreamNonBlocking));
			HIP_TRY(hipEventCreateWithFlags(&T.go, hipEventDisableTiming));
			HIP_TRY(hipEventCreateWithFlags(&T.done, hipEventDisableTiming));
			HIP_TRY(T.d_cnt.alloc(1));
			HIP_TRY(T.d_span.alloc(4));
		}
		if (c->cost_kind == SRH_COST_SAD && c->sad_dense && (p->window_radius == 5 || p->window_radius == 2))
			for (int k = 0; k < 2; ++k)
				if ((rc = ensure_sad_planes(c, c->views[k == 0 ? left : right], p->window_radius))) return rc;
		if ((p->window_radius == 5 || p->window_radius == 2) &&
		    ((rc = ensure_tvp(c, c->views[left])) || (rc = ensure_tvp(c, c->views[right])))) return rc;
		if ((rc = ensure_wta_planes(c, left, right)) || (rc = ensure_wta_planes(c, right, left))) return rc;
		HIP_TRY(hipEventRecord(T.go, c->stream));
	}
	progress(c, 1, "Computing cost volume for left image...");
	auto deferred_wta = [&](int k, int ref, int oth) { c->defer = &c->tv_defer[k]; const int r = srh_twoview_wta(c, ref, oth, p, 0, 0); c->defer = nullptr; return r; };
	if ((rc = deferred_wta(0, left, right))) return rc;
	if (cancelled(c)) return fail(SRH_E_CANCELLED, "cancelled");
	progress(c, 3, "Computing cost volume for right image...");
	if (c->tv_overlap && c->tv_defer[0].queued) {
		srh_context::TvSlot &T = c->tv_slot;
		HIP_TRY(hipStreamWaitEvent(T.stream, T.go, 0));
		tv_slot_swap(c);
		rc = deferred_wta(1, right, left);
		const hipError_t e = rc ? hipStreamSynchronize(c->stream) : hipEventRecord(T.done, c->stream);
		tv_slot_swap(c);
		if (rc) return rc;
		if (e != hipSuccess) return fail(SRH_E_DEVICE, "second TwoView pass: %s", hipGetErrorString(e));
		HIP_TRY(hipStreamWaitEvent(c->stream, T.done, 0));
		HIP_TRY(hipMemcpyAsync(c->d_cnt, T.d_cnt, sizeof(Counters), hipMemcpyDeviceToDevice, c->stream));
	} else {
		if ((rc = deferred_wta(1, right, left))) return rc;
	}
	if (cancelled(c)) return fail(SRH_E_CANCELLED, "cancelled");
	srh_context::TvDefer &d0 = c->tv_defer[0], &d1 = c->tv_defer[1];
	if (d0.queued && d1.queued) {
		progress(c, 5, "Detecting inconsistencies...");
		if ((rc = srh_twoview_cross_check(c, left, right, p))) return rc;
		const ViewHost &L = c->views[left], &Rv = c->views[right];
		if (left_out && !c->filter_invalid) HIP_TRY(hipMemcpyAsync(left_out, L.depth, (size_t)L.w*L.h*sizeof(double), hipMemcpyDeviceToHost, c->stream));
		if (right_out && !c->filter_invalid) HIP_TRY(hipMemcpyAsync(right_out, Rv.depth, (size_t)Rv.w*Rv.h*sizeof(double), hipMemcpyDeviceToHost, c->stream));
		HIP_TRY(hipStreamSynchronize(c->stream));
		if (c->debug_trace)
			for (srh_context::TvDefer *d : { &d0, &d1 })
				fprintf(stderr, "[srh trace] unverified pass %d>%d: lists %d cmax %d smax %d guessed %d -> longest %d slots %d rows over %d cert_overflow %llu stands %d\n",
				        d->ref, d->oth, (int)d->lists, d->cmax, d->smax, (int)d->guessed, d->span[0], d->span[1], d->span[2],
				        (unsigned long long)d->host->cert_overflow, (int)tv_pass_stands(*d));
		if (tv_pass_stands(d0) && tv_pass_stands(d1)) {
			for (srh_context::TvDefer *d : { &d0, &d1 })
				if (d->lists && d->guessed) {
					tv_learn_lists(c, d->ref, d->oth, true, d->cmax, d->smax, d->span, *d->host);
					d->guessed = false;
				}
// ... 1629 lines not shown
```

stereoreconstruction_amd/csrc/srh_dense.hip:

```cpp
#include "srh_internal.hpp"
#include "srh_geom.hpp"
#include "srh_walk.hpp"

#include <algorithm>
#include <type_traits>
#include <utility>

namespace srh {

__device__ __forceinline__ double color_dist_u(uint32_t a, uint32_t b) {
	const double dr = (double)((int)(a & 255u) - (int)(b & 255u));
	const double dg = (double)((int)((a >> 8) & 255u) - (int)((b >> 8) & 255u));
	const double db = (double)((int)((a >> 16) & 255u) - (int)((b >> 16) & 255u));
	return sqrt(dr*dr + dg*dg + db*db);
}

__global__ void edge_planes_kernel(const uint32_t *__restrict__ rgba, int W, int H, double *__restrict__ edges)
{
	const size_t n = (size_t)W*H;
	const double inf = __builtin_inf();
	for (size_t i = (size_t)blockIdx.x*blockDim.x + threadIdx.x; i < n; i += (size_t)gridDim.x*blockDim.x) {
		const int x = (int)(i % (size_t)W), y = (int)(i / (size_t)W);
		const uint32_t c = rgba[i];
		edges[0*n + i] = (x + 1 < W) ? color_dist_u(rgba[i + 1], c) : inf;
// ... 1080 lines not shown
#pragma unroll
					for (int col = 0; col < WS; ++col) av[col] = CS.lt[0][i + col];
#pragma unroll
					for (int j = 0; j < DC_NCB; ++j) { mR[j] = acc[j]/tw; s1[j] = 0.0; s3[j] = 0.0; }
					__builtin_amdgcn_s_waitcnt(0xC07F);
#pragma unroll 1
					for (int row = 0; row < WS; ++row) {
						const int nrow = row + 1 < WS ? row + 1 : 0;
						const double2 *rp = reinterpret_cast<const double2 *>(&CS.rt[nrow][rc]);
						const double2 *wp = reinterpret_cast<const double2 *>(&CS.w[i][nrow*WP]);
						const double *lp = &CS.lt[nrow][i];
#pragma unroll
						for (int col = 0; col < WS; ++col) {
							const double wt = wv[col];
							if (FMA) {
								const double a = __builtin_fma(wt, av[col], -mL);
								double bb[DC_NCB];
#pragma unroll
								for (int j = 0; j < DC_NCB; ++j) bb[j] = __builtin_fma(wt, r[col + j], -mR[j]);
								__builtin_amdgcn_sched_barrier(0);
#pragma unroll
								for (int j = 0; j < DC_NCB; ++j) { s1[j] = __builtin_fma(a, bb[j], s1[j]); s3[j] = __builtin_fma(bb[j], bb[j], s3[j]); }
							} else {
							double bb[DC_NCB], u1[DC_NCB], u3[DC_NCB];
							const double pa = wt*av[col];
#pragma unroll
							for (int j = 0; j < DC_NCB; ++j) bb[j] = wt*r[col + j];
							__builtin_amdgcn_sched_barrier(0);
							const double a = pa - mL;
#pragma unroll
							for (int j = 0; j < DC_NCB; ++j) bb[j] = bb[j] - mR[j];
							__builtin_amdgcn_sched_barrier(0);
#pragma unroll
							for (int j = 0; j < DC_NCB; ++j) { u1[j] = a*bb[j]; u3[j] = bb[j]*bb[j]; }
							__builtin_amdgcn_sched_barrier(0);
#pragma unroll
							for (int j = 0; j < DC_NCB; ++j) { s1[j] += u1[j]; s3[j] += u3[j]; }
							}
							__builtin_amdgcn_sched_barrier(0);
							av[col] = lp[col];
							if (col & 1) {
								const double2 v = rp[col >> 1]; r[col - 1] = v.x; r[col] = v.y;
								const double2 u = wp[col >> 1]; wv[col - 1] = u.x; wv[col] = u.y;
							}
							__builtin_amdgcn_sched_barrier(0);
						}
#pragma unroll
						for (int m = (WS - 1)/2; m < NR/2; ++m) { const double2 v = rp[m]; r[2*m] = v.x; r[2*m + 1] = v.y; }
						wv[WS - 1] = CS.w[i][nrow*WP + WS - 1];
					}
#pragma unroll
					for (int j = 0; j < DC_NCB; ++j) {
						const int c = c0 + j;
						if (c >= lo && c <= hi && CS.rfull[rc + j] != 0) {
							const double v = 255*(1.0 - fabs(s1[j]) / sqrt(s2 * s3[j]));
							if (CERT) crow[(size_t)(c - e.xmin)*DC_TP] = !(s3[j] >= sig3) ? __builtin_nan("") : (v > cb.m_hi ? P.max_color_diff : v);
							else crow[(size_t)(c - e.xmin)*DC_TP] = (v < P.max_color_diff) ? v : P.max_color_diff;
						}
						__builtin_amdgcn_sched_barrier(0);
					}
#ifdef SRH_PROFILE_PHASES
					t_fast += __builtin_readcyclecounter() - t0; ++n_fast;
#endif
				}
			}
		}
		const bool need_general = s_need_pix != 0 || s_need_col != 0;
		for (int base = 0; need_general && base < DC_TP*DC_CHUNK; base += Smem::GL_CAP) {
			if (tid == 0) S.glist_n = 0;
			__syncthreads();
			for (int p = base + tid; p < base + Smem::GL_CAP && p < DC_TP*DC_CHUNK; p += DC_THREADS) {
				const int pi = p / DC_CHUNK, k = p % DC_CHUNK;
				const int c = cs + k;
				if (c < S.pxmin[pi] || c > S.pxmax[pi]) continue;
				if (CS.lall[pi] && CS.rfull[k]) continue;
				S.glist[atomicAdd(&S.glist_n, 1)] = (unsigned short)(pi*512 + k);
			}
			__syncthreads();
			const int nl = S.glist_n;
			for (int q = tid; q < nl; q += DC_THREADS) {
				const int pi = S.glist[q] >> 9, k = S.glist[q] & 511;
				++n_dev;
				cost[((size_t)blockIdx.x*cstride + (cs + k - S.pxmin[pi]))*DC_TP + pi] =
					dense_cost_general<R, DC_NCB, DC_CHUNK>(CS, pi, k, P.weight_cutoff, P.bad_ret, P.max_color_diff);
			}
		}
	}
	SRH_STAMP(4);
	block_count_add(&cnt->n_eval_device, n_dev);
	SRH_STAMP(5);
#ifdef SRH_PROFILE_PHASES
	if ((tid & 63) == 0) {
		for (int k = 0; k < 8; ++k) atomicAdd(&cnt->dbg_phase[k], ph[k]);
		atomicAdd(&cnt->dbg_cycles, t_fast);
		atomicAdd(&cnt->dbg_blocks, n_fast);
		atomicAdd(&cnt->dbg_total_cycles, (unsigned long long)(__builtin_readcyclecounter() - t_begin));
		atomicAdd(&cnt->dbg_waves, 1ull);
	}
#endif
#undef SRH_STAMP
}

template <int R, int NCB, int CHUNK, int MINW, int AR>
static void launch_dense_variant(hipStream_t st, dim3 grid, const ViewDev *views, int ref, int oth, const srh_params &P,
                                 int y0, int nrows, const double *wbuf, size_t wstride,
                                 const double *tnum, double *cost, int cstride, Counters *cnt, const double *pconst, const PixRange *prange)
{
	typedef DenseSmem<R, NCB, CHUNK> Smem;
	size_t lds = sizeof(Smem);
#ifdef SRH_EXPERIMENT
	lds += (size_t)g_exp_lds_pad;
#endif
	(void)hipFuncSetAttribute((const void *)twoview_dense_cost_kernel<R, NCB, CHUNK, MINW, AR>,
	                          hipFuncAttributeMaxDynamicSharedMemorySize, (int)lds);
	hipLaunchKernelGGL((twoview_dense_cost_kernel<R, NCB, CHUNK, MINW, AR>), grid, dim3(DC_THREADS), lds, st,
	                   views, ref, oth, P, y0, nrows, wbuf, wstride, tnum, cost, cstride, cnt, pconst, cert_bound(P), prange);
}

bool launch_twoview_dense_cost(hipStream_t st, const ViewDev *views, int ref, int oth, int width, const srh_params &P,
                               int y0, int nrows, const double *wbuf, size_t wstride,
                               const double *tnum, double *cost, int cstride, Counters *cnt, const double *pconst, int arith,
                               const PixRange *prange)
{
	const int tiles = (width + DC_TP - 1)/DC_TP;
	const dim3 grid((unsigned)(tiles*nrows));
#define SRH_ARGS st, grid, views, ref, oth, P, y0, nrows, wbuf, wstride, tnum, cost, cstride, cnt, pconst, prange
	switch (P.window_radius) {
	case 5:
		if (arith == 5) launch_dense_variant<5, 8, 320, 2, 5>(SRH_ARGS);
		else if (arith == 3) launch_dense_variant<5, 8, 320, 2, 3>(SRH_ARGS);
		else if (arith == 1) launch_dense_variant<5, 8, 320, 2, 1>(SRH_ARGS);
		else launch_dense_variant<5, 8, 320, 2, 0>(SRH_ARGS);
		return true;
	case 2:
		if (arith == 5) launch_dense_variant<2, 8, 320, 2, 5>(SRH_ARGS);
		else if (arith == 3) launch_dense_variant<2, 8, 320, 2, 3>(SRH_ARGS);
		else if (arith == 1) launch_dense_variant<2, 8, 320, 2, 1>(SRH_ARGS);
		else launch_dense_variant<2, 8, 320, 2, 0>(SRH_ARGS);
		return true;
	default: return false;
	}
#undef SRH_ARGS
}

#define SC_TW 64
#ifndef SC_QN
#define SC_QN 8
#endif
#ifndef SC_OCC
#define SC_OCC 6
#endif
#define SC_MW 1024

__global__ void twoview_lazy_fill_kernel(const ViewDev *__restrict__ views, int ref, int oth, srh_params P, int y0, int nrows,
                                         const PixRange *__restrict__ prange, const double *__restrict__ wbuf, size_t wstride,
                                         int ncb, int lanes, int pad, double *__restrict__ cost, int cstride, Counters *__restrict__ cnt)
{
	const ViewDev &L = views[ref];
	const ViewDev &Rv = views[oth];
	const int W = L.w;
	const size_t q = (size_t)blockIdx.x*blockDim.x + threadIdx.x;
	unsigned n_lazy = 0;
	if (q < (size_t)nrows*W) {
		const int x = (int)(q % W), trow = (int)(q / W), y = y0 + trow;
		const PixRange pr = prange[q];
		if (pr.hi >= pr.lo) {
			const int cover = dense_cover_hi(pr.lo, pr.hi, ncb, lanes, pad != 0);
			if (cover < pr.hi) {
				const int R = P.window_radius, T = (2*R + 1)*(2*R + 1);
				const double *wq = wbuf + wbuf_offset(W, T, trow, x);
				double *crow = cost + ((size_t)trow*((W + DC_TP - 1)/DC_TP) + (x/DC_TP))*(size_t)cstride*DC_TP + (x % DC_TP);
				for (int c = cover + 1; c <= pr.hi; ++c) {
					crow[(size_t)(c - pr.lo)*DC_TP] = tv_cost(L, Rv, wq, wstride, P, x, y, c, y);
					++n_lazy;
				}
			}
		}
	}
	block_count_add(&cnt->n_eval_device, n_lazy);
}

template <int R>
__global__ __launch_bounds__(256)
void twoview_lazy_fill_planes_kernel(int W, srh_params P, int y0, int nrows, const PixRange *__restrict__ prange,
                                     const double *__restrict__ wbuf, int wimg, const double *__restrict__ ref_tvp,
                                     const double *__restrict__ oth_tvp, int ncb, int lanes, int pad,
                                     double *__restrict__ cost, int cstride, Counters *__restrict__ cnt)
{
	const size_t q = (size_t)blockIdx.x*blockDim.x + threadIdx.x;
	unsigned n_lazy = 0;
	if (q < (size_t)nrows*W) {
		const int x = (int)(q % W), trow = (int)(q / W), y = y0 + trow;
		const PixRange pr = prange[q];
		const int cover = pr.hi >= pr.lo ? dense_cover_hi(pr.lo, pr.hi, ncb, lanes, pad != 0) : pr.hi;
		if (cover < pr.hi) {
			const int SP = padded_stride(W);
			const WindowAt wa = window_at<R>(wbuf, wimg, W, trow, x);
			const double *lp = ref_tvp + (size_t)(y + SRH_PADY - R)*SP + (x + SRH_PADL - R);
			double *crow = cost + ((size_t)trow*((W + DC_TP - 1)/DC_TP) + (x/DC_TP))*(size_t)cstride*DC_TP + (x % DC_TP);
			for (int c = cover + 1; c <= pr.hi; ++c) {
				const double *rp = oth_tvp + (size_t)(y + SRH_PADY - R)*SP + (c + SRH_PADL - R);
				crow[(size_t)(c - pr.lo)*DC_TP] = window_exact_cost<R>(wa.wq, wa.wrow, wa.wcol, lp, rp, SP, SP, P);
				++n_lazy;
			}
		}
	}
	block_count_add(&cnt->n_eval_device, n_lazy);
}

template <int R>
__global__ __launch_bounds__(64)
void twoview_refill_kernel(int W, srh_params P, int y0, const PixRange *__restrict__ prange, const uint32_t *__restrict__ cflag, int cap,
                           const double *__restrict__ wbuf, int wimg, const double *__restrict__ ref_tvp, const double *__restrict__ oth_tvp,
                           double *__restrict__ cost, int cstride, Counters *__restrict__ cnt)
{
	const uint32_t nflag = cflag[0];
	if (blockIdx.x == 0 && threadIdx.x == 0 && nflag > (uint32_t)cap) atomicAdd(&cnt->cert_overflow, 1ull);
	unsigned n = 0;
	for (uint32_t f = blockIdx.x; f < nflag && f < (uint32_t)cap; f += gridDim.x) {
		const uint32_t q = cflag[1 + f];
		const int x = (int)(q % (uint32_t)W), trow = (int)(q / (uint32_t)W), y = y0 + trow;
		const PixRange pr = prange[q];
		const int SP = padded_stride(W);
		const WindowAt wa = window_at<R>(wbuf, wimg, W, trow, x);
		const double *lp = ref_tvp + (size_t)(y + SRH_PADY - R)*SP + (x + SRH_PADL - R);
		double *crow = cost + ((size_t)trow*((W + DC_TP - 1)/DC_TP) + (x/DC_TP))*(size_t)cstride*DC_TP + (x % DC_TP);
		for (int c = pr.lo + (int)threadIdx.x; c <= pr.hi; c += 64) {
			const double *rp = oth_tvp + (size_t)(y + SRH_PADY - R)*SP + (c + SRH_PADL - R);
			crow[(size_t)(c - pr.lo)*DC_TP] = window_exact_cost<R>(wa.wq, wa.wrow, wa.wcol, lp, rp, SP, SP, P);
			++n;
		}
	}
	block_count_add(&cnt->n_eval_device, n);
}

bool launch_twoview_refill(hipStream_t st, int width, const srh_params &P, int y0, const PixRange *prange, const uint32_t *cflag, int cap,
                           const double *wbuf, bool wimg, const double *ref_tvp, const double *oth_tvp, double *cost, int cstride, Counters *cnt)
{
	if (cap <= 0) return true;
	if (P.window_radius == 5)
		hipLaunchKernelGGL(twoview_refill_kernel<5>, dim3((unsigned)(cap < 8192 ? cap : 8192)), dim3(64), 0, st, width, P, y0, prange, cflag, cap, wbuf, wimg ? 1 : 0, ref_tvp, oth_tvp, cost, cstride, cnt);
	else if (P.window_radius == 2)
		hipLaunchKernelGGL(twoview_refill_kernel<2>, dim3((unsigned)(cap < 8192 ? cap : 8192)), dim3(64), 0, st, width, P, y0, prange, cflag, cap, wbuf, wimg ? 1 : 0, ref_tvp, oth_tvp, cost, cstride, cnt);
	else return false;
	return true;
}

void launch_twoview_lazy_fill(hipStream_t st, const ViewDev *views, int ref, int oth, int width, const srh_params &P,
                              int y0, int nrows, const PixRange *prange, const double *wbuf, size_t wstride,
                              const double *ref_tvp, const double *oth_tvp, bool wimg,
                              int lanes, bool padded, double *cost, int cstride, Counters *cnt)
{
	const size_t n = (size_t)nrows*width;
	const dim3 grid((unsigned)((n + 255)/256)), block(256);
	const int pad = padded ? 1 : 0;
	if (ref_tvp && P.window_radius == 5)
		hipLaunchKernelGGL(twoview_lazy_fill_planes_kernel<5>, grid, block, 0, st, width, P, y0, nrows, prange, wbuf, wimg ? 1 : 0, ref_tvp, oth_tvp, 8, lanes, pad, cost, cstride, cnt);
	else if (ref_tvp && P.window_radius == 2)
		hipLaunchKernelGGL(twoview_lazy_fill_planes_kernel<2>, grid, block, 0, st, width, P, y0, nrows, prange, wbuf, wimg ? 1 : 0, ref_tvp, oth_tvp, 8, lanes, pad, cost, cstride, cnt);
	else
		hipLaunchKernelGGL(twoview_lazy_fill_kernel, grid, block, 0, st, views, ref, oth, P, y0, nrows, prange, wbuf, wstride, 8, lanes, pad, cost, cstride, cnt);
}

__device__ __forceinline__ unsigned wave_sum_u32(unsigned v) {
#pragma unroll
	for (int d = 1; d < 64; d <<= 1) v += (unsigned)__shfl_xor((int)v, d);
	return v;
}
__device__ __forceinline__ int wave_min_i32(int v) {
#pragma unroll
	for (int d = 1; d < 64; d <<= 1) { const int o = __shfl_xor(v, d); v = o < v ? o : v; }
	return v;
}
__device__ __forceinline__ int wave_max_i32(int v) {
#pragma unroll
	for (int d = 1; d < 64; d <<= 1) { const int o = __shfl_xor(v, d); v = o > v ? o : v; }
	return v;
}

struct TwoViewScanState {
	double minCost, secondBest;
	int wcol;
	int pcol;
};

template <bool CERT, bool LISTED, bool WTA>
__device__ __forceinline__
void twoview_scan_tile(const int bid, const ViewDev *__restrict__ views, int ref, int oth, const srh_params &P,
                       int y0, int nrows, const double *__restrict__ tnum,
                       const double *__restrict__ cost, int cstride,
                       Counters *__restrict__ cnt, const PixRange *__restrict__ prange,
                       uint32_t *__restrict__ cflag, int nlist, const CertBound &cb, const double *__restrict__ pexact,
                       int32_t *__restrict__ wout)
{
	const ViewDev &L = views[ref];
	const ViewDev &Rv = views[oth];
	const int W = L.w, OW = Rv.w, OH = Rv.h;
	const int tiles_per_row = (W + SC_TW - 1)/SC_TW;
	const int tid = threadIdx.x;
	int trow, x;
	bool listed_on = true;
	if (LISTED) {
		const uint32_t nflag = cflag[0];
		const int k = bid*SC_TW + tid;
		listed_on = k < nlist && (uint32_t)k < nflag;
		const uint32_t q = listed_on ? cflag[1 + k] : 0u;
		trow = (int)(q / (uint32_t)W); x = (int)(q % (uint32_t)W);
	} else {
		trow = bid / tiles_per_row;
		x = (bid % tiles_per_row)*SC_TW + tid;
	}
	const int y = y0 + trow;

	__shared__ unsigned short queue[SC_QN][SC_TW];
	__shared__ __align__(16) unsigned char mrow_raw[SC_MW + 16];

	unsigned n_eval = 0, n_pix = 0, bad = 0, n_flag = 0;
	const bool active = listed_on && x < W && L.mask[(size_t)y*W + x] == 1;
	Ray ray;
	int lo = 0, hi = -1;
	if (active) {
		ray = cam_unproject(L.cam, (x + 0.5) / P.image_scale, (y + 0.5) / P.image_scale);
		const PixRange pr = prange[(size_t)trow*W + x];
		lo = pr.lo; hi = pr.hi;
	}
	const int umin = LISTED ? 2147483647 : wave_min_i32(hi >= lo ? lo : 2147483647);
	const unsigned char *mrow = mrow_raw;
	if (umin != 2147483647 && y >= 0 && y < OH) {
		const size_t first = (size_t)y*OW + (size_t)umin, a0 = first & ~(size_t)3, total = (size_t)OW*OH;
		mrow = mrow_raw + (first - a0);
		const size_t at = a0 + (size_t)tid*16;
		uint32_t v[4];
#pragma unroll
		for (int k = 0; k < 4; ++k)
			v[k] = (at + 4*k + 4 <= total) ? *reinterpret_cast<const uint32_t *>(Rv.mask + at + 4*k) : 0u;
		if (at + 16 > total) {
#pragma unroll
			for (int k = 0; k < 4; ++k) {
				uint32_t w = 0;
				for (int b2 = 0; b2 < 4; ++b2) if (at + 4*k + b2 < total) w |= (uint32_t)Rv.mask[at + 4*k + b2] << (8*b2);
				v[k] = w;
			}
		}
		uint4 q; q.x = v[0]; q.y = v[1]; q.z = v[2]; q.w = v[3];
		*reinterpret_cast<uint4 *>(mrow_raw + tid*16) = q;
	}
	__syncthreads();

	double depth = __builtin_nan("");
	int owin = -1, orun = -1;
	if (active) {
		n_pix = 1;
		const double *crow = cost + ((size_t)trow*((W + DC_TP - 1)/DC_TP) + (x/DC_TP))*(size_t)cstride*DC_TP + (x % DC_TP);
		TwoViewScanState st = { __builtin_inf(), __builtin_inf(), -1, -1 };
		int qn = 0;
		bool px_sure = false;
		if (CERT && pexact) { const double *pc = pexact + ((size_t)trow*W + x)*SRH_PC; px_sure = cert_pixel_exact(cb, pc[2], pc[3]); }

		auto flush = [&](int count) {
			int col[SC_QN];
			double c[SC_QN];
#pragma unroll
			for (int k = 0; k < SC_QN; ++k) col[k] = queue[k][tid];
#pragma unroll
			for (int k = 0; k < SC_QN; ++k)
#ifdef SRH_EXPERIMENT
				c[k] = (k < count && g_exp_scan_mode != 1) ? crow[(size_t)col[k]*DC_TP] : (double)col[k];
#else
				c[k] = (k < count) ? crow[(size_t)col[k]*DC_TP] : __builtin_inf();
#endif
#pragma unroll
			for (int k = 0; k < SC_QN; ++k) {
				if (k < count) {
					const double cv = c[k];
					if (CERT) {
						const double t = cv + P.wta_margin;
						if (!(fabs(t - st.minCost) > 2.5*cb.e0) && col[k] != st.wcol &&
						    !(cert_sure(cv, P.max_color_diff, cb.m_hi) && cert_sure(st.minCost, P.max_color_diff, cb.m_hi)) &&
						    !(px_sure && cv == cv)) n_flag = 1;
					}
					if (cv + P.wta_margin < st.minCost) {
						st.secondBest = st.minCost;
						st.minCost = cv;
						if (WTA) st.pcol = st.wcol;
						st.wcol = col[k];
					}
				}
			}
		};

		const Vec3 nrm = normalized(load3(L.cam.pdir));
		const double nd = dot(nrm, ray.dir);
		if (!(fabs(nd) < 1e-10)) {
			double x1 = __builtin_nan(""), y1 = __builtin_nan("");
			int jx1 = 0, jy1 = 0;
			const SharedDivisor nd_sd = shared_divisor(nd);
#ifdef SRH_EXPERIMENT
			const int exp_nd = g_exp_scan_mode == 2 ? 2 : P.num_depth_levels;
			for (int d = 0; d < exp_nd; ++d) {
#else
			for (int d = 0; d < P.num_depth_levels; ++d) {
#endif
				double x2, y2;
				if (!pinhole_project_label_sd(ray, nd_sd, tnum[d], Rv.cam, P.image_scale, x2, y2)) continue;
				if (isnan_d(x1)) { x1 = x2; y1 = y2; jx1 = trunc_sat(x2); jy1 = trunc_sat(y2); continue; }
				const double dx = x2 - x1, dy = y2 - y1;
				if (!(dx*dx + dy*dy >= 1)) continue;
				const int ix0 = jx1, iy0 = jy1, ix1 = trunc_sat(x2), iy1 = trunc_sat(y2);
				jx1 = ix1; jy1 = iy1;
				const int a = ix0 < ix1 ? ix0 : ix1, b = ix0 < ix1 ? ix1 : ix0;
				if (iy0 == y && iy1 == y && a >= lo && b <= hi) {
					for (int tx = a; tx <= b; ++tx) {
						const int k = tx - umin;
						const bool white = (!LISTED && k >= 0 && k < SC_MW - 4) ? (mrow[k] == 1) : (Rv.mask[(size_t)y*OW + tx] == 1);
// ... 298 lines not shown
		if (__any(active && !good)) return false;
		if (!use_bound || __any(active && !bpass)) {
			if (active) {
				const Ray ray = cam_unproject(L.cam, (x + 0.5) / P.image_scale, (y + 0.5) / P.image_scale);
				const TsPixel pp = ts_pixel_setup(ray, L.cam, Rv.cam, P.image_scale, tpl->tabs, tpl->tmin, tpl->tmax, y);
				good = tscan_verify_labels(pp.fp, pp.nd, pp.eU, pp.dyU, P.image_scale, x, D, tpl, tnum);
			}
			if (__any(active && !good)) return false;
		} else by_bound = true;
	}
	int lo = 0;
	if (active) {
		const PixRange pr = prange[(size_t)trow*W + x];
		lo = pr.lo;
		const int hi = pr.hi;
		int wlo = x + smin, whi = x + smax;
		if (whi == -1) whi = 0;
		if (wlo < 0) wlo = 0;
		if (whi > OW - 1) whi = OW - 1;
		good = true;
		if (nS > 0 && whi >= wlo) good = lo <= wlo && hi >= whi;
		if (y < 0 || y >= OH) good = false;
	}
	if (__any(active && !good)) return false;

	const int mbase = xt + smin, mlen = nS > 0 ? SC_TW + (smax - smin) + 1 : 0;
	for (int k = tid; k < mlen; k += SC_TW) {
		const int tx = mbase + k;
		smask[k] = ((unsigned)tx < (unsigned)OW) ? Rv.mask[(size_t)y*OW + tx] : (unsigned char)0;
	}
	__syncthreads();

	unsigned n_eval = 0, n_flag = 0;
	double depth = __builtin_nan("");
	int owin = -1, orun = -1;
	if (active) {
		n_pix_acc += 1;
		const double *crow = cost + ((size_t)trow*((W + DC_TP - 1)/DC_TP) + (x/DC_TP))*(size_t)cstride*DC_TP + (x % DC_TP);
		double minCost = __builtin_inf(), secondBest = __builtin_inf();
		int wcol = -1, pcol = -1;
		bool px_sure = false;
		if (CERT && pexact) { const double *pc = pexact + ((size_t)trow*W + x)*SRH_PC; px_sure = cert_pixel_exact(cb, pc[2], pc[3]); }
		const int xm = tid - smin;
		const int xlo = x - lo;
		int nSe = nS;
#ifdef SRH_EXPERIMENT
		if (g_exp_scan_mode == 4 || g_exp_scan_mode == 5) nSe = 0;
#endif
		auto lookups = [&](auto left_c) {
			constexpr bool LEFT = decltype(left_c)::value;
			const int32_t *seq = LEFT ? tpl->S : tpl->F;
			const int nE = nSe == 0 ? 0 : (LEFT ? nS : tpl->nF);
			for (int j0 = 0; j0 < nE; j0 += TS_U) {
				int sv[TS_U], kk[TS_U], mu[TS_U];
				unsigned char mb[TS_U];
				double c[TS_U];
				{
					const int4 sa = reinterpret_cast<const int4 *>(&seq[j0])[0], sb = reinterpret_cast<const int4 *>(&seq[j0])[1];
					sv[0] = sa.x; sv[1] = sa.y; sv[2] = sa.z; sv[3] = sa.w; sv[4] = sb.x; sv[5] = sb.y; sv[6] = sb.z; sv[7] = sb.w;
				}
#pragma unroll
				for (int u = 0; u < TS_U; ++u) {
					int s;
					if (LEFT) {
						s = (sv[u] << 3) >> 3;
						s += ((sv[u] & 0x40000000) && x + s == -1) ? 1 : 0;
						mu[u] = 1;
					} else {
						s = (sv[u] << 8) >> 8;
						mu[u] = sv[u] >> 24;
					}
					sv[u] = s;
					mb[u] = smask[xm + s];
				}
#pragma unroll
				for (int u = 0; u < TS_U; ++u) {
					const bool white = j0 + u < nE && mb[u] == 1;
					n_eval += white ? (unsigned)mu[u] : 0u;
					kk[u] = white ? xlo + sv[u] : -1;
					c[u] = crow[(unsigned)(white ? kk[u] : 0)*(unsigned)DC_TP];
				}
#pragma unroll
				for (int u = 0; u < TS_U; ++u) {
					const bool on = kk[u] >= 0;
					const double cv = c[u];
					const double t = on ? cv + P.wta_margin : __builtin_inf();
					if (CERT) {
						const bool nearby = on && !(fabs(t - minCost) > 2.5*cb.e0);
						if (__any(nearby)) {
							if (nearby && kk[u] != wcol &&
							    !(cert_sure(cv, P.max_color_diff, cb.m_hi) && cert_sure(minCost, P.max_color_diff, cb.m_hi)) &&
							    !(px_sure && cv == cv)) n_flag = 1;
						}
					}
					if (t < minCost) { secondBest = minCost; minCost = cv; if (WTA) pcol = wcol; wcol = kk[u]; }
				}
			}
		};
		if (xt + smin < 0 || !(P.wta_margin >= 0.0)) lookups(std::true_type()); else lookups(std::false_type());
		if (wcol >= 0) depth = candidate_depth(L.cam, Rv.cam, P, cam_unproject(L.cam, (x + 0.5) / P.image_scale, (y + 0.5) / P.image_scale), lo + wcol, y);
		if (minCost > P.second_best_factor*secondBest) depth = __builtin_inf();
		if (CERT && wcol >= 0) {
			const double rhs = P.second_best_factor*secondBest;
			const double tol = __builtin_fma(fmin(fabs(rhs), 1e300), 1e-15, (1.0 + fabs(P.second_best_factor))*cb.e0);
			if (!(fabs(minCost - rhs) > tol) && !px_sure &&
			    !(cert_sure(minCost, P.max_color_diff, cb.m_hi) && cert_sure(secondBest, P.max_color_diff, cb.m_hi))) n_flag = 1;
		}
		if (CERT && n_flag) cflag[1 + atomicAdd(&cflag[0], 1u)] = (uint32_t)((size_t)trow*W + x);
		if (WTA) { owin = wcol >= 0 ? lo + wcol : -1; orun = pcol >= 0 ? lo + pcol : -1; }
	}
	if (x < W) L.depth[(size_t)y*W + x] = depth;
	if (WTA && x < W) wta_store(wout, (size_t)W*L.h, (size_t)y*W + x, owin, owin >= 0 ? y : -1, orun, orun >= 0 ? y : -1);
	n_eval_acc += n_eval; n_flag_acc += n_flag;
	return true;
}

template <bool CERT, bool WTA>
__global__ __launch_bounds__(SC_TW, (CERT && WTA) ? 6 : 7)
void twoview_tscan_kernel(const ViewDev *__restrict__ views, int ref, int oth, srh_params P,
                          int y0, int nrows, const double *__restrict__ tnum,
                          const double *__restrict__ cost, int cstride,
                          Counters *__restrict__ cnt, const PixRange *__restrict__ prange,
                          uint32_t *__restrict__ cflag, CertBound cb, const double *__restrict__ pexact,
                          const ScanTemplate *__restrict__ tpl, uint32_t *__restrict__ tilelist, int32_t *__restrict__ wout, int use_bound)
{
	__shared__ unsigned char smask[SC_TW + TS_MAXSPAN + 16];
	const int W = views[ref].w;
	const int ntiles = ((W + SC_TW - 1)/SC_TW)*nrows;
	const int tid = threadIdx.x;
	const bool tok = tpl->ok != 0;
	unsigned n_eval = 0, n_pix = 0, n_flag = 0, n_tpl = 0, n_walk = 0, n_bound = 0;
	for (int bid = blockIdx.x; bid < ntiles; bid += gridDim.x) {
		bool by_bound = false;
		const bool done = tok && twoview_tscan_tile<CERT, WTA>(bid, views, ref, oth, P, y0, nrows, tnum, cost, cstride, cnt, prange, cflag, cb, pexact,
		                                                      tpl, smask, n_eval, n_pix, n_flag, wout, use_bound, by_bound);
		if (!done) { if (tid == 0) tilelist[1 + atomicAdd(&tilelist[0], 1u)] = (uint32_t)bid; ++n_walk; } else { ++n_tpl; n_bound += by_bound ? 1u : 0u; }
		__syncthreads();
	}
	if (!cnt) return;
	n_eval = wave_sum_u32(n_eval); n_pix = wave_sum_u32(n_pix); n_flag = wave_sum_u32(n_flag);
	if (tid == 0) {
		if (n_eval) atomicAdd(&cnt->n_eval, (unsigned long long)n_eval);
		if (n_pix) atomicAdd(&cnt->n_pixels, (unsigned long long)n_pix);
		if (CERT && n_pix) atomicAdd(&cnt->n_certified, (unsigned long long)n_pix);
		if (CERT && n_flag) atomicAdd(&cnt->n_flagged, (unsigned long long)n_flag);
		if (n_tpl) atomicAdd(&cnt->scan_tiles_template, (unsigned long long)n_tpl);
		if (n_walk) atomicAdd(&cnt->scan_tiles_walked, (unsigned long long)n_walk);
		if (n_bound) atomicAdd(&cnt->scan_tiles_bound, (unsigned long long)n_bound);
	}
}

#define RSW_MAXD 1024
#define RSW_MAXC 6144
template <bool WTA>
__global__ __launch_bounds__(64)
void twoview_rescan_wave_kernel(const ViewDev *__restrict__ views, int ref, int oth, srh_params P, int y0,
                                const double *__restrict__ tnum, const double *__restrict__ cost, int cstride,
                                const PixRange *__restrict__ prange, const uint32_t *__restrict__ cflag, int cap,
                                Counters *__restrict__ cnt, int32_t *__restrict__ wout)
{
	const ViewDev &L = views[ref];
	const ViewDev &Rv = views[oth];
	const int W = L.w, OW = Rv.w, OH = Rv.h;
	const int lane = threadIdx.x;
	__shared__ double sx[RSW_MAXD], sy[RSW_MAXD];
	__shared__ unsigned short scol[RSW_MAXC];
	__shared__ double scost[RSW_MAXC];
	__shared__ unsigned char smask[4096 + 64];
	__shared__ int s_n;
	const uint32_t nflag = cflag[0];
	for (uint32_t f = blockIdx.x; f < nflag && f < (uint32_t)cap; f += gridDim.x) {
		const uint32_t q = cflag[1 + f];
		const int x = (int)(q % (uint32_t)W), trow = (int)(q / (uint32_t)W), y = y0 + trow;
		const PixRange pr = prange[q];
		const int lo = pr.lo, hi = pr.hi;
		const Ray ray = cam_unproject(L.cam, (x + 0.5) / P.image_scale, (y + 0.5) / P.image_scale);
		const Vec3 nrm = normalized(load3(L.cam.pdir));
		const double nd = dot(nrm, ray.dir);
		const bool walk = !(fabs(nd) < 1e-10);
		if (walk) {
			const SharedDivisor nd_sd = shared_divisor(nd);
			for (int d = lane; d < P.num_depth_levels; d += 64) {
				double x2, y2;
				const bool ok = pinhole_project_label_sd(ray, nd_sd, tnum[d], Rv.cam, P.image_scale, x2, y2);
				sx[d] = ok ? x2 : __builtin_nan("");
				sy[d] = ok ? y2 : 0.0;
			}
		}
		const int span = hi >= lo ? hi - lo + 1 : 0;
		for (int k = lane; k < span && k < 4096; k += 64) smask[k] = (y >= 0 && y < OH) ? Rv.mask[(size_t)y*OW + lo + k] : 0;
		__syncthreads();
		if (lane == 0) {
			int n = 0;
			bool over = false;
			if (walk) {
				double x1 = __builtin_nan(""), y1 = __builtin_nan("");
				for (int d = 0; d < P.num_depth_levels && !over; ++d) {
					const double x2 = sx[d], y2 = sy[d];
					if (isnan_d(x2)) continue;
					if (isnan_d(x1)) { x1 = x2; y1 = y2; continue; }
					const double dx = x2 - x1, dy = y2 - y1;
					if (!(dx*dx + dy*dy >= 1)) continue;
					const int ix0 = trunc_sat(x1), iy0 = trunc_sat(y1), ix1 = trunc_sat(x2), iy1 = trunc_sat(y2);
					const int a = ix0 < ix1 ? ix0 : ix1, b = ix0 < ix1 ? ix1 : ix0;
					if (iy0 == y && iy1 == y && a >= lo && b <= hi) {
						for (int tx = a; tx <= b; ++tx) {
							const int k = tx - lo;
							const bool white = k < 4096 ? (smask[k] == 1) : (Rv.mask[(size_t)y*OW + tx] == 1);
							if (white) { if (n < RSW_MAXC) scol[n] = (unsigned short)k; else over = true; ++n; }
						}
					} else {
						LineWalk lw;
						lw.begin(ix0, iy0, ix1, iy1, OW, OH);
						while (lw.has_next()) {
							int tx, ty;
							lw.current(tx, ty);
							if (tx >= 0 && ty >= 0 && tx < OW && ty < OH && Rv.mask[(size_t)ty*OW + tx] == 1 &&
							    ty == y && tx >= lo && tx <= hi) {
								if (n < RSW_MAXC) scol[n] = (unsigned short)(tx - lo); else over = true;
								++n;
							}
							lw.next();
						}
					}
					x1 = x2; y1 = y2;
				}
			}
			if (over) { atomicAdd(&cnt->cert_overflow, 1ull); n = RSW_MAXC; }
			s_n = n;
		}
		__syncthreads();
		const int n = s_n;
		const double *crow = cost + ((size_t)trow*((W + DC_TP - 1)/DC_TP) + (x/DC_TP))*(size_t)cstride*DC_TP + (x % DC_TP);
		for (int k = lane; k < n; k += 64) scost[k] = crow[(size_t)scol[k]*DC_TP];
		__syncthreads();
		if (lane == 0) {
			double minCost = __builtin_inf(), secondBest = __builtin_inf();
			int wcol = -1, pcol = -1;
			for (int k = 0; k < n; ++k) {
				const double cv = scost[k];
				if (cv + P.wta_margin < minCost) { secondBest = minCost; minCost = cv; if (WTA) pcol = wcol; wcol = scol[k]; }
			}
			double depth = __builtin_nan("");
			if (wcol >= 0) depth = candidate_depth(L.cam, Rv.cam, P, ray, lo + wcol, y);
			if (minCost > P.second_best_factor*secondBest) depth = __builtin_inf();
			L.depth[(size_t)y*W + x] = depth;
			if (WTA) wta_store(wout, (size_t)W*L.h, (size_t)y*W + x, wcol >= 0 ? lo + wcol : -1, wcol >= 0 ? y : -1,
			                   pcol >= 0 ? lo + pcol : -1, pcol >= 0 ? y : -1);
		}
		__syncthreads();
	}
}

void launch_scan_template(hipStream_t st, const ViewDev *views, int ref, int oth, const srh_params &P, int y0, int nrows,
                          const double *tnum, void *tpl)
{
	hipLaunchKernelGGL(twoview_template_kernel, dim3(1), dim3(256), 0, st, views, ref, oth, P, y0, nrows, tnum, (ScanTemplate *)tpl);
}

void launch_twoview_scan(hipStream_t st, const ViewDev *views, int ref, int oth, int width, const srh_params &P,
                         int y0, int nrows, const double *tnum, const double *cost, int cstride,
                         Counters *cnt, const PixRange *prange, uint32_t *cflag, int nlist, const double *pexact,
                         const void *tpl, uint32_t *tilelist, int num_cus, int32_t *wout, int tscan_bound)
{
	const int tiles = (width + SC_TW - 1)/SC_TW;
	const CertBound cb = cert_bound(P);
	const ScanTemplate *tp = (const ScanTemplate *)tpl;
	if (!tp) tilelist = nullptr;
	const unsigned pgrid = (unsigned)std::min<long long>((long long)tiles*nrows, (long long)num_cus*4*8);
	const unsigned wgrid = tp ? (unsigned)std::min<long long>((long long)tiles*nrows, (long long)num_cus*4*4) : (unsigned)(tiles*nrows);
	if (tp) (void)hipMemsetAsync(tilelist, 0, sizeof(uint32_t), st);
#define SRH_TSCAN(C_, W_, FLAG_, PEX_)                                                                         \
	hipLaunchKernelGGL((twoview_tscan_kernel<C_, W_>), dim3(pgrid), dim3(SC_TW), 0, st,                        \
	                   views, ref, oth, P, y0, nrows, tnum, cost, cstride, cnt, prange, FLAG_, cb, PEX_, tp, tilelist, wout, tscan_bound)
#define SRH_SCAN(C_, L_, W_, GRID_, FLAG_, NL_, PEX_, TL_)                                                     \
	hipLaunchKernelGGL((twoview_scan_kernel<C_, L_, W_>), dim3(GRID_), dim3(SC_TW), 0, st,                     \
	                   views, ref, oth, P, y0, nrows, tnum, cost, cstride, cnt, prange, FLAG_, NL_, cb, PEX_, TL_, wout)
	if (!cflag) {
		if (tp) { if (wout) SRH_TSCAN(false, true, nullptr, nullptr); else SRH_TSCAN(false, false, nullptr, nullptr); }
		if (wout) SRH_SCAN(false, false, true, wgrid, nullptr, 0, nullptr, tilelist);
		else      SRH_SCAN(false, false, false, wgrid, nullptr, 0, nullptr, tilelist);
	} else if (nlist < 0) {
		if (tp) { if (wout) SRH_TSCAN(true, true, cflag, pexact); else SRH_TSCAN(true, false, cflag, pexact); }
		if (wout) SRH_SCAN(true, false, true, wgrid, cflag, 0, pexact, tilelist);
		else      SRH_SCAN(true, false, false, wgrid, cflag, 0, pexact, tilelist);
	} else if (nlist > 0 && P.num_depth_levels <= RSW_MAXD && cstride <= 4096) {
		const dim3 rgrid((unsigned)(nlist < 2048 ? nlist : 2048));
		if (wout) hipLaunchKernelGGL(twoview_rescan_wave_kernel<true>, rgrid, dim3(64), 0, st,
		                             views, ref, oth, P, y0, tnum, cost, cstride, prange, cflag, nlist, cnt, wout);
		else      hipLaunchKernelGGL(twoview_rescan_wave_kernel<false>, rgrid, dim3(64), 0, st,
		                             views, ref, oth, P, y0, tnum, cost, cstride, prange, cflag, nlist, cnt, wout);
	} else if (nlist > 0) {
		const unsigned lgrid = (unsigned)((nlist + SC_TW - 1)/SC_TW);
		if (wout) SRH_SCAN(false, true, true, lgrid, cflag, nlist, nullptr, nullptr);
		else      SRH_SCAN(false, true, false, lgrid, cflag, nlist, nullptr, nullptr);
	}
#undef SRH_TSCAN
#undef SRH_SCAN
}

}
```

stereoreconstruction_amd/csrc/srh_internal.hpp:

```cpp
#pragma once

#include <hip/hip_runtime.h>
#include <stdint.h>

#include "stereo_recon_hip.h"

namespace srh {

struct ViewDev {
	int32_t w, h;
	const uint32_t *rgba;
	const uint8_t  *mask;
	const double   *gray;
	const double   *gray_tv;
	double         *depth;
	srh_camera      cam;
};

#define SRH_WTILE 32
__host__ __device__ inline size_t wbuf_doubles(int W, int nrows, int T) {
	return (size_t)nrows*((W + SRH_WTILE - 1)/SRH_WTILE)*SRH_WTILE*T;
}
__host__ __device__ inline size_t wbuf_offset(int W, int T, int band_row, int x) {
	const size_t tile = (size_t)band_row*((W + SRH_WTILE - 1)/SRH_WTILE) + x/SRH_WTILE;
	return tile*(size_t)T*SRH_WTILE + (x % SRH_WTILE);
}

__host__ __device__ inline int wimg_wp(int R) { return ((2*R + 1) + 1) & ~1; }
__host__ __device__ inline int wimg_row_stride(int R) { return SRH_WTILE*wimg_wp(R); }
__host__ __device__ inline size_t wimg_doubles(int W, int nrows, int R) {
	return (size_t)nrows*((W + SRH_WTILE - 1)/SRH_WTILE)*SRH_WTILE*(size_t)((2*R + 1)*wimg_wp(R));
}
__host__ __device__ inline size_t wimg_offset(int W, int R, int band_row, int x) {
	const size_t tile = (size_t)band_row*((W + SRH_WTILE - 1)/SRH_WTILE) + x/SRH_WTILE;
	return tile*SRH_WTILE*(size_t)((2*R + 1)*wimg_wp(R)) + (size_t)(x % SRH_WTILE)*wimg_wp(R);
}
#define SRH_PADL 8
#define SRH_PADR 344
#define SRH_PADY 8
__host__ __device__ inline int padded_stride(int w) { return w + SRH_PADL + SRH_PADR; }
__host__ __device__ inline size_t padded_size(int w, int h) { return (size_t)padded_stride(w)*(size_t)(h + 2*SRH_PADY); }
struct PixRange { int32_t lo, hi; };

struct CertBound {
	double e0, m_hi, k1, k2, room;
	double zmax2;
	int ok;
	__host__ __device__ inline double sigma3(double s2) const {
		const double d = room - k2/sqrt(s2);
		if (!(d > 0)) return __builtin_inf();
		const double b = k1/d;
		return b*b*(1.0 + 0x1p-20);
	}
};
__host__ __device__ inline bool cert_sure(double x, double clamp, double m_hi) { return x == clamp || x > m_hi; }
__host__ __device__ inline bool cert_pixel_exact(const CertBound &cb, double sum2, double all_taps_usable) {
	return !(all_taps_usable != 0.0) || !(cb.sigma3(sum2) < __builtin_inf());
}
#ifdef __HIPCC__
__device__ __forceinline__ double onepass_finish(double P, double Q, double U, double SA, double itw, double s2, double TT,
                                                 double sig3, double zmax2, bool &okc)
{
	const double m = P*itw, p2 = P + P;
	const double s3 = __builtin_fma(-m, __builtin_fma(-TT, m, p2), U);
	const double s1 = __builtin_fma(-m, SA, Q);
	const double q3 = __builtin_fma(m, __builtin_fma(TT, m, p2), U);
	const double x = s2*s3;
	const double y0 = __builtin_amdgcn_rsq(x);
	const double e = __builtin_fma(-(x*y0), y0, 1.0);
	const double y1 = __builtin_fma(y0*e, __builtin_fma(0.375, e, 0.5), y0);
	const bool c1 = s3 >= sig3, c2 = s3*zmax2 >= q3, c3 = __builtin_fabs(e) <= 0x1p-20;
	okc = c1 & c2 & c3;
	return __builtin_fma(-255.0, __builtin_fabs(s1)*y1, 255.0);
}
#endif
inline CertBound cert_bound(const srh_params &P, bool mvs = false) {
	const double u = 0x1p-53, G = 256.0;
	const int T = (2*P.window_radius + 1)*(2*P.window_radius + 1);
	auto gamma = [&](int k) { return k*u/(1.0 - k*u); };
	const double eps_b = gamma(T + 4)*G, eps_a = 2*u*G, rt = sqrt((double)T);
	const double scale = mvs ? 1.0 : 255.0;
	CertBound c;
	c.e0 = mvs ? 0x1p-36 : 0x1p-26;
	c.k1 = 2*scale*1.01*3*eps_b*rt;
	c.k2 = 2*scale*1.01*eps_a*rt;
	const double k3 = 2*scale*1.01*2*gamma(T) + (mvs ? 40 : 2600)*u;
	c.room = c.e0 - k3;
	c.m_hi = P.max_color_diff + c.e0;
	{
		const double g = gamma(T + 6), rhs = (c.e0/2 - 2600*u)/(scale*1.01*g);
		const double z = rhs > 0 ? (-3.0 + sqrt(9.0 + 4*2.002*rhs))/(2*2.002) : 0.0;
		c.zmax2 = z*z*(1.0 - 0x1p-20);
	}
	const bool weights_ok = P.weight_kind == SRH_WEIGHT_GEODESIC ? P.geodesic_sigma > 0 : P.adaptive_color_sigma > 0;
	if (mvs) { c.ok = c.room > 0 && weights_ok && fabs(P.peak_threshold) <= 1e5; return c; }
	c.ok = c.room > 0 && c.m_hi > P.max_color_diff && P.max_color_diff <= 1e5 && fabs(P.bad_ret) <= 1e5 &&
	       P.wta_margin >= 0 && P.wta_margin <= 1e5 && fabs(P.second_best_factor) <= 1e5 && weights_ok;
	return c;
}

#ifdef __HIPCC__
__device__ __forceinline__ void wta_store(int32_t *__restrict__ wout, size_t npix, size_t pv, int wx, int wy, int rx, int ry) {
	*reinterpret_cast<int2 *>(wout + 2*pv) = make_int2(wx, wy);
	*reinterpret_cast<int2 *>(wout + 2*(npix + pv)) = make_int2(rx, ry);
}
#endif
void launch_twoview_winner_costs(hipStream_t st, const ViewDev *views, int ref, int oth, int width, const srh_params &P, bool sad,
                                 int y0, int nrows, const double *wbuf, bool wimg, const int32_t *wout,
                                 double *min_cost, double *second_cost);

struct Counters {
	unsigned long long n_pixels;
	unsigned long long n_eval;
	unsigned long long n_eval_device;
	unsigned long long not_row_aligned;
	unsigned long long n_listed, n_slots;
	unsigned long long strip_overflow;
	unsigned long long n_certified, n_flagged;
	unsigned long long cert_overflow;
	unsigned long long scan_tiles_template, scan_tiles_walked;
	unsigned long long scan_tiles_bound;
	unsigned long long mvs_waves_staged, mvs_waves_listed;
	unsigned int strip_ticket, strip_ticket_border;
	unsigned long long dbg_cycles, dbg_blocks, dbg_total_cycles, dbg_waves;
	unsigned long long dbg_phase[8];
	unsigned long long dbg_wave[64];
};

#define SRH_MAX_NEIGH 8
struct NeighList { int32_t n[SRH_MAX_NEIGH]; };
inline NeighList make_neigh_list(const int32_t *neigh, int nneigh) {
	NeighList l;
	for (int i = 0; i < SRH_MAX_NEIGH; ++i) l.n[i] = (i < nneigh) ? neigh[i] : 0;
	return l;
}

struct Extent { int32_t xmin, xmax; };

void launch_prep_view(hipStream_t st, const uint32_t *rgba, const uint8_t *mask, int w, int h,
                      double *gray, double *gray_tv);
void launch_fill(hipStream_t st, double *p, size_t n, double v);
#define SRH_PC 6
void launch_weights(hipStream_t st, const ViewDev *views, int ref, int width, const srh_params &P,
                    int y0, int nrows, double *wbuf, size_t wstride, double *pconst = nullptr, bool wimg = false);
void launch_twoview_generic(hipStream_t st, const ViewDev *views, int ref, int oth, int width, const srh_params &P,
                            int y0, int nrows, const double *wbuf, size_t wstride, Counters *cnt, bool sad = false,
                            int32_t *wout = nullptr);
void launch_twoview_cross_check(hipStream_t st, const ViewDev *views, int self, int other, int w, int h,
                                const srh_params &P);
void launch_mvs_generic(hipStream_t st, const ViewDev *views, int ref, const int32_t *neigh, int nneigh, int width,
                        const srh_params &P, int y0, int nrows, const double *wbuf, size_t wstride,
                        double *peaks, double *best, Counters *cnt);
void launch_mvs_cross_check(hipStream_t st, const ViewDev *views, const int32_t *slots_dev, int nviews,
                            int view_index, int w, int h, const srh_params &P);

void launch_edge_planes(hipStream_t st, const uint32_t *rgba, int w, int h, double *edges);
void launch_geo_exp_probe(hipStream_t st, const double *x, int n, double *kout, double *lout);
size_t geo5_doubles(int w, int h);
void launch_geo5_planes(hipStream_t st, const double *edges, const double *gray_tv, const uint8_t *mask, int w, int h, double *out);
bool launch_geodesic_dma(hipStream_t st, const ViewDev *views, int ref, int width, const double *geo5, const srh_params &P,
                         int y0, int nrows, double *wbuf, double *pconst, int num_cus);
bool launch_geodesic_reg(hipStream_t st, const ViewDev *views, int ref, int width, const double *edges,
                         const srh_params &P, int y0, int nrows, double *wbuf, size_t wstride, double *pconst = nullptr,
                         bool wimg = false);
bool launch_adaptive_reg(hipStream_t st, const ViewDev *views, int ref, int width, const srh_params &P, int y0, int nrows,
                         double *wbuf, size_t wstride, double *pconst = nullptr, bool wimg = false);
void launch_label_plane_table(hipStream_t st, const ViewDev *views, int ref, const srh_params &P, bool mvs, double *tdist);
void launch_pinhole_label_table(hipStream_t st, const ViewDev *views, int ref, const srh_params &P, bool mvs, double *tnum);
bool launch_twoview_dense_cost_f32(hipStream_t st, const ViewDev *views, int ref, int oth, int width, const srh_params &P,
                                   int y0, int nrows, const double *wbuf, size_t wstride,
                                   const double *tnum, double *cost, int cstride, Counters *cnt, const double *pconst, int form = 0);
bool launch_twoview_dense_cost(hipStream_t st, const ViewDev *views, int ref, int oth, int width, const srh_params &P,
                               int y0, int nrows, const double *wbuf, size_t wstride,
                               const double *tnum, double *cost, int cstride, Counters *cnt, const double *pconst, int arith = 0,
                               const PixRange *prange = nullptr);
void launch_twoview_scan(hipStream_t st, const ViewDev *views, int ref, int oth, int width, const srh_params &P,
                         int y0, int nrows, const double *tnum, const double *cost, int cstride,
                         Counters *cnt, const PixRange *prange, uint32_t *cflag = nullptr, int nlist = -1,
                         const double *pexact = nullptr,
                         const void *tpl = nullptr, uint32_t *tilelist = nullptr,
                         int num_cus = 256, int32_t *wout = nullptr,
                         int tscan_bound = 1);
size_t scan_template_bytes();
void launch_scan_template(hipStream_t st, const ViewDev *views, int ref, int oth, const srh_params &P, int y0, int nrows,
                          const double *tnum, void *tpl);
bool launch_twoview_refill(hipStream_t st, int width, const srh_params &P, int y0, const PixRange *prange, const uint32_t *cflag, int cap,
                           const double *wbuf, bool wimg, const double *ref_tvp, const double *oth_tvp, double *cost, int cstride, Counters *cnt);
void launch_twoview_lazy_fill(hipStream_t st, const ViewDev *views, int ref, int oth, int width, const srh_params &P,
                              int y0, int nrows, const PixRange *prange, const double *wbuf, size_t wstride,
                              const double *ref_tvp, const double *oth_tvp,
                              bool wimg,
                              int lanes, bool padded,
                              double *cost, int cstride, Counters *cnt);

void launch_padded_plane(hipStream_t st, const double *gray_tv, int w, int h, double *out);
void launch_padded_full(hipStream_t st, const double *gray_tv, int w, int h, int R, uint8_t *out);
void launch_pixel_range(hipStream_t st, const ViewDev *views, int ref, int oth, int width, const srh_params &P,
                        int y0, int nrows, const double *tnum, int cstride, PixRange *prange);
int  strip_chunk_columns();
int  strip_block_lanes(int cstride, int form);
bool launch_twoview_strip_cost(hipStream_t st, const ViewDev *views, int ref, int oth, int width, int height,
                               const srh_params &P, int y0, int nrows, const double *wimg, const double *pconst,
                               const PixRange *prange, const double *ref_tvp, const double *oth_tvp,
                               const uint8_t *oth_fullp, double *cost, int cstride, Counters *cnt, int arith, int num_cus,
                               int lanes, bool raw = false);

#ifdef SRH_PROFILE_PHASES
void geodesic_phases_fetch(unsigned long long out[8]);
#endif
#ifdef SRH_EXPERIMENT
void exp_set(int repeat, int lds_pad);
void exp_set_scan(int mode);
void exp_set_walk(int mode);
void exp_set_rows(int mode);
#endif

#define SRH_FUSED_MAXC 256
bool launch_twoview_fused(hipStream_t st, const ViewDev *views, int ref, int oth, int width, const srh_params &P,
                          int y0, int nrows, const double *wbuf, const double *tnum, Counters *cnt, int32_t *wout = nullptr);

void launch_twoview_count(hipStream_t st, const ViewDev *views, int ref, int oth, int width, const srh_params &P,
                          int y0, int nrows, int32_t *count, Counters *cnt, int *max_count, const double *tdist);
void launch_twoview_list(hipStream_t st, const ViewDev *views, int ref, int oth, int width, const srh_params &P,
                         int y0, int nrows, uint32_t *cand, int cmax, int32_t *count, Counters *cnt, int *max_count,
                         const double *tdist);
void launch_full_window(hipStream_t st, const double *gray_tv, int w, int h, int R, uint8_t *full, uint32_t *stat = nullptr);
inline size_t full_stat_offset(size_t npix) { return (npix + 15) & ~(size_t)15; }
bool launch_twoview_list_cost(hipStream_t st, const ViewDev *views, int ref, int oth, int width, const srh_params &P,
                              int y0, int nrows, const double *wbuf, const uint8_t *full_oth,
                              const int32_t *count, const uint32_t *cand, double *cost, int cmax, Counters *cnt);
void launch_twoview_list_scan(hipStream_t st, const ViewDev *views, int ref, int oth, int width, const srh_params &P,
                              int y0, int nrows, const int32_t *count, const uint32_t *cand, const double *cost, int cmax,
                              int32_t *wout = nullptr);
void mvs_staging_shape(int *maxw, size_t *desc_words_per_wave);
void launch_mvs_walk(hipStream_t st, const ViewDev *views, int ref, const int32_t *neigh, int nneigh, int width,
                     const srh_params &P, int y0, int nrows, const double *tnum, uint32_t *cand, int cmax, int32_t *count,
                     Counters *cnt, int *max_count, uint32_t *wdesc, int32_t *nwin, const uint32_t *act, int nact, bool peaks,
                     bool fast_pinhole = false);
void launch_mvs_staged_cost(hipStream_t st, const ViewDev *views, int ref, const int32_t *neigh, int nneigh, int width,
                            const srh_params &P, int y0, int nrows, const double *wbuf, size_t wstride,
                            const uint32_t *cand, int cmax, const int32_t *count, double *best,
                            const uint32_t *wdesc, const int32_t *nwin, Counters *cnt, const uint32_t *act, int nact,
                            double *unit_peaks, bool cert = false);
void launch_mvs_list_cost(hipStream_t st, const ViewDev *views, int ref, const int32_t *neigh, int nneigh, int width,
                          const srh_params &P, int y0, int nrows, const double *wbuf, size_t wstride,
                          const uint32_t *cand, int cmax, const int32_t *count, double *best,
                          double *unit_peaks, bool peaks, const int32_t *nwin, const uint32_t *act, int nact);
void launch_mvs_combine(hipStream_t st, const ViewDev *views, int ref, int nneigh, int width, const srh_params &P,
                        int y0, int nrows, const double *best, const double *unit_peaks, double *peaks);
void launch_filter_gaps(hipStream_t st, const double *D, double *G, int w, int h, int gap, unsigned long long *cnt);
void launch_filter_holes(hipStream_t st, const uint8_t *mask, double *D, int w, int h, bool median, uint32_t *holes,
                         unsigned long long *cnt);
void launch_filter_median(hipStream_t st, const ViewDev *views, int slot, const srh_params &P, const double *G,
                          const uint32_t *holes, int nholes, double *D, unsigned long long *cnt);
void launch_sad_full_window(hipStream_t st, const uint8_t *mask, int w, int h, int R, uint8_t *full);
bool launch_twoview_rows_sad(hipStream_t st, const ViewDev *views, int ref, int oth, int width, const srh_params &P,
                             int y0, int nrows, const double *wbuf, const uint8_t *full_sad_oth,
                             const uint32_t *rowinfo, const int32_t *meta, double *cost, int smax, Counters *cnt);
void launch_twoview_list_sad(hipStream_t st, const ViewDev *views, int ref, int oth, int width, const srh_params &P,
                             int y0, int nrows, const double *wbuf, const int32_t *count, const uint32_t *cand,
                             double *cost, int cmax, Counters *cnt);
void launch_padded_gray(hipStream_t st, const double *gray, const uint8_t *mask, int w, int h, double *out);
void launch_padded_bytes(hipStream_t st, const uint8_t *in, int w, int h, uint8_t *out);
bool launch_twoview_strip_sad(hipStream_t st, int width, int height, const srh_params &P, int y0, int nrows,
                              const double *wimg, const PixRange *prange, const double *ref_tvp, const double *oth_grayp,
                              const uint8_t *oth_fullp, double *cost, int cstride, Counters *cnt, int num_cus);
void launch_pair_costs(hipStream_t st, const ViewDev *views, int ref, int oth, const srh_params &P, bool sad, int n,
                       const int32_t *xy, double *out);
void launch_point_cloud(hipStream_t st, const ViewDev *views, int slot, int w, int h, const srh_params &P,
                        double *xyz, uint8_t *rgb, uint8_t *valid, unsigned long long *counts);
struct FuseViewDev { const double *pts; const uint8_t *valid; uint8_t *claimed; };
struct FuseCloud { double *xyz, *nrm; int32_t *src; uint8_t *rgb, *nviews, *flags; };
#define SRH_FUSE_BLOCK 256
void launch_fuse_view(hipStream_t st, const ViewDev *views, const int32_t *slots_dev, int nviews, int vi, int w, int h,
                      const srh_params &P, double thr, double gap, int min_views, const FuseViewDev *fv,
                      uint8_t *emit, FuseCloud stage, uint32_t *block_counts, unsigned long long *counters);
void launch_fuse_scan(hipStream_t st, const uint32_t *block_counts, int nblocks, unsigned long long *block_offs,
                      unsigned long long *counters);
void launch_fuse_scatter(hipStream_t st, int vi, size_t npix, const uint8_t *emit, FuseCloud stage,
                         const unsigned long long *block_offs, FuseCloud out, unsigned long long cap);
struct MrfLayout {
	double *pz, *D, *Mh, *Mv, *partial, *energy;
	unsigned long long *hand; size_t hand_words;
	unsigned *status, *sync;
	int32_t *ans;
	int nparts, nbands;
	size_t sync_words, total_doubles;
};
size_t mrf_scratch_doubles(int w, int h);
void launch_mrf_layout(double *buf, int w, int h, MrfLayout &lay);
hipError_t launch_mrf_setup(hipStream_t st, double *buf, int w, int h, int K, double beta, double lambda, double phiu,
                            const double *peaks, MrfLayout &lay);
hipError_t launch_mrf_sweep(hipStream_t st, double *buf, int w, int h, int K, double psiu, int sweep);
hipError_t launch_mrf_energy(hipStream_t st, double *buf, int w, int h, int K, double psiu);
hipError_t launch_mrf_depth(hipStream_t st, const ViewDev *views, int slot, double *buf, int w, int h, int K);
hipError_t launch_mrf_data(hipStream_t st, size_t n, int K, double beta, double lambda, double phiu, const double *peaks, double *D, double *pz);
hipError_t launch_mrf_labels_energy(hipStream_t st, int w, int h, int K, double psiu, const double *D, const double *pz, const int32_t *ans,
                                    double *partial, int nparts, double *energy);
hipError_t launch_mrf_labels_depth(hipStream_t st, const ViewDev *views, int slot, int K, const double *pz, const int32_t *ans, size_t n);
struct MvsSgmLayout {
	double *pz, *D, *S, *partial, *energy;
	int32_t *ans;
	int nparts;
	size_t total_doubles;
};
size_t mvs_sgm_scratch_doubles(int w, int h);
void mvs_sgm_layout(double *buf, int w, int h, MvsSgmLayout &lay);
hipError_t launch_mvs_sgm_setup(hipStream_t st, double *buf, int w, int h, int K, double beta, double lambda, double phiu, const double *peaks);
hipError_t launch_mvs_sgm_path(hipStream_t st, double *buf, int w, int h, int K, double psiu, int k, bool first);
hipError_t launch_mvs_sgm_readoff(hipStream_t st, const ViewDev *views, int slot, double *buf, int w, int h, int K);
hipError_t launch_mvs_sgm_energy(hipStream_t st, double *buf, int w, int h, int K, double psiu);
struct TvMrfLayout {
	double *Mh, *Mv, *trash, *partial, *energy;
	unsigned long long *hand; size_t hand_words;
	unsigned *status, *sync;
	int32_t *ans;
	int nparts, nbands;
	size_t sync_words, total_doubles;
};
size_t twoview_mrf_scratch_doubles(int w, int h, int L);
void launch_twoview_mrf_layout(double *buf, int w, int h, int L, TvMrfLayout &lay);
hipError_t launch_twoview_mrf_setup(hipStream_t st, double *buf, int w, int h, int L, TvMrfLayout &lay);
hipError_t launch_twoview_mrf_sweep(hipStream_t st, double *buf, const double *costs, int w, int h, int L, double lambda, double smax, int sweep);
hipError_t launch_twoview_mrf_energy(hipStream_t st, double *buf, const double *costs, int w, int h, int L, double lambda, double smax);
hipError_t launch_twoview_mrf_depth(hipStream_t st, const ViewDev *views, int slot, const srh_params &P, double *buf, int w, int h, int L);
hipError_t launch_twoview_labels_energy(hipStream_t st, const double *costs, const int32_t *ans, double *partial, int nparts, double *energy,
                                        int w, int h, int L, double lambda, double smax);
struct TvSgmLayout {
	double *S, *partial, *energy;
	int32_t *ans;
	int nparts;
	size_t total_doubles;
};
size_t twoview_sgm_scratch_doubles(int w, int h, int L);
void twoview_sgm_layout(double *buf, int w, int h, int L, TvSgmLayout &lay);
hipError_t launch_twoview_sgm_path(hipStream_t st, double *buf, const double *costs, int w, int h, int L, double lambda, double smax, int k, bool first);
hipError_t launch_twoview_sgm_readoff(hipStream_t st, const ViewDev *views, int slot, const srh_params &P, double *buf, int w, int h, int L);
hipError_t launch_twoview_sgm_energy(hipStream_t st, double *buf, const double *costs, int w, int h, int L, double lambda, double smax);
hipError_t launch_twoview_label_costs(hipStream_t st, const ViewDev *views, int ref, int oth, int width, const srh_params &P, bool sad,
                                      int y0, int nrows, double fill, double *cost, int32_t *pixel);
void launch_epipolar_preview(hipStream_t st, const ViewDev *views, int ref, int oth, double zmin, double zmax, int nd,
                             int nq, const double *xy, double *out, int32_t *counts);
void launch_refraction_error(hipStream_t st, const ViewDev *views, int v1, int v2, int n, const double *p1, const double *p2, double *err);
void launch_epipolar_curves(hipStream_t st, const ViewDev *views, int ref, int oth, const srh_params &P, int mvs,
                            int nq, const int32_t *xy, int32_t *out, int cap, int32_t *counts);

#define SRH_ROWS_NR 32
void launch_twoview_rows_list(hipStream_t st, const ViewDev *views, int ref, int oth, int width, const srh_params &P,
                              int y0, int nrows, uint32_t *cand, int cmax, int32_t *count, uint32_t *rowinfo,
                              int32_t *meta, int smax, Counters *cnt, int *maxes, const double *tdist);
bool launch_twoview_rows_cost(hipStream_t st, const ViewDev *views, int ref, int oth, int width, const srh_params &P,
// ... 32 lines not shown
```

stereoreconstruction_amd/csrc/srh_strip.hip:

```cpp
#include "srh_internal.hpp"
#include "srh_geom.hpp"
#include "srh_walk.hpp"

#include <type_traits>

namespace srh {

#ifdef SRH_EXPERIMENT
__device__ int g_strip_exp_repeat = 1;
void strip_exp_set(int repeat) { (void)hipMemcpyToSymbol(HIP_SYMBOL(g_strip_exp_repeat), &repeat, sizeof(int)); }
#endif

#define ST_TP 32
#define ST_NCB 8
#define ST_CHUNK 320
#define ST_BROWS 1

typedef __attribute__((address_space(3))) void st_lds_void;
typedef __attribute__((address_space(1))) const void st_gbl_void;
typedef __attribute__((address_space(3))) volatile int st_lds_vint;

__global__ void padded_plane_kernel(const double *__restrict__ gray_tv, int W, int H, double *__restrict__ out)
{
	const int SP = padded_stride(W), HP = H + 2*SRH_PADY;
	const size_t n = (size_t)SP*HP;
	const double nan = __builtin_nan("");
	for (size_t k = (size_t)blockIdx.x*blockDim.x + threadIdx.x; k < n; k += (size_t)gridDim.x*blockDim.x) {
		const int x = (int)(k % (size_t)SP) - SRH_PADL, y = (int)(k / (size_t)SP) - SRH_PADY;
		out[k] = (x >= 0 && y >= 0 && x < W && y < H) ? gray_tv[(size_t)y*W + x] : nan;
	}
}

void launch_padded_plane(hipStream_t st, const double *gray_tv, int w, int h, double *out) {
	size_t n = padded_size(w, h);
	size_t b = (n + 255)/256; if (b > 4096) b = 4096;
	hipLaunchKernelGGL(padded_plane_kernel, dim3((unsigned)b), dim3(256), 0, st, gray_tv, w, h, out);
}

__global__ void padded_full_kernel(const double *__restrict__ gray_tv, int W, int H, int R, uint8_t *__restrict__ out)
{
	const int SP = padded_stride(W), HP = H + 2*SRH_PADY;
	const size_t n = (size_t)SP*HP;
	for (size_t k = (size_t)blockIdx.x*blockDim.x + threadIdx.x; k < n; k += (size_t)gridDim.x*blockDim.x) {
		const int x = (int)(k % (size_t)SP) - SRH_PADL, y = (int)(k / (size_t)SP) - SRH_PADY;
		bool ok = x - R >= 0 && y - R >= 0 && x + R < W && y + R < H;
		for (int row = -R; ok && row <= R; ++row)
			for (int col = -R; col <= R; ++col) {
				const double v = gray_tv[(size_t)(y + row)*W + (x + col)];
				ok = ok && (v == v);
			}
		out[k] = ok ? 1 : 0;
	}
}

void launch_padded_full(hipStream_t st, const double *gray_tv, int w, int h, int R, uint8_t *out) {
	size_t n = padded_size(w, h);
	size_t b = (n + 255)/256; if (b > 4096) b = 4096;
	hipLaunchKernelGGL(padded_full_kernel, dim3((unsigned)b), dim3(256), 0, st, gray_tv, w, h, R, out);
}

__global__ void pixel_range_kernel(const ViewDev *__restrict__ views, int ref, int oth, srh_params P, int y0, int nrows,
                                   const double *__restrict__ tnum, int cstride, PixRange *__restrict__ prange)
{
	const ViewDev &L = views[ref];
	const int W = L.w;
	const size_t q = (size_t)blockIdx.x*blockDim.x + threadIdx.x;
	if (q >= (size_t)nrows*W) return;
	const int x = (int)(q % W), y = y0 + (int)(q / W);
	int lo = 0, hi = -1;
	if (L.mask[(size_t)y*W + x] == 1) {
		const Ray ray = cam_unproject(L.cam, (x + 0.5) / P.image_scale, (y + 0.5) / P.image_scale);
		pinhole_column_range(ray, L.cam, views[oth], P, tnum, cstride, lo, hi);
	}
	PixRange r; r.lo = lo; r.hi = hi;
	prange[q] = r;
}

void launch_pixel_range(hipStream_t st, const ViewDev *views, int ref, int oth, int width, const srh_params &P,
                        int y0, int nrows, const double *tnum, int cstride, PixRange *prange)
{
	const size_t n = (size_t)nrows*width;
	hipLaunchKernelGGL(pixel_range_kernel, dim3((unsigned)((n + 255)/256)), dim3(256), 0, st,
	                   views, ref, oth, P, y0, nrows, tnum, cstride, prange);
}

int strip_chunk_columns() { return ST_CHUNK; }

struct StripArgs {
	int W, H, y0, nrows;
	const double *wimg;
	const double *pconst;
	const PixRange *prange;
	const double *ref_tvp, *oth_tvp;
	const uint8_t *oth_fullp;
	double *cost; int cstride;
	Counters *cnt;
	int n1, n2;
	int nitems;
	double weight_cutoff, bad_ret, max_color_diff;
	CertBound cb;
	int redo;
};

static void strip_items(StripArgs &a) {
	a.n1 = ((a.nrows*3/4)/16)*16;
	a.n2 = a.n1 + (((a.nrows - a.n1)*2/3)/8)*8;
	const int nseg = a.n1/16 + (a.n2 - a.n1)/8 + (a.nrows - a.n2 + 3)/4;
	a.nitems = nseg*((a.W + ST_TP - 1)/ST_TP);
}

template <int R, int NBUF>
struct StripSmem {
	static constexpr int WS = 2*R + 1;
	static constexpr int T = WS*WS;
	static constexpr int WP = (WS + 1) & ~1;
	static constexpr int WPIX = WS*WP;
	static constexpr int RW = ST_CHUNK + 2*R + ST_NCB + 2;
	static constexpr int LW = (ST_TP + 2*R + 1) & ~1;
	static constexpr int NS = WS + 1;
	static constexpr int FW = (RW + 4 + 15) & ~15;
	static constexpr int NBMAX = ST_CHUNK/ST_NCB + 1;
	static constexpr int GL_CAP = 3072;
	static constexpr int GL_SINGLES = GL_CAP - ST_TP*NBMAX;
	alignas(16) double w[NBUF][WS][ST_TP][WP];
	alignas(16) double rt[NS][RW];
	alignas(16) double rto[NBUF == 2 ? NS : 1][RW];
	alignas(16) double lt[NS][LW];
	alignas(16) double pc[2][ST_TP][SRH_PC];
	alignas(16) PixRange pr[2][ST_TP];
	alignas(16) unsigned char full[2][FW];
	unsigned short glist[GL_CAP];
	int glist_n, gsingle_n;
	int item;
	unsigned long long badcols[ST_CHUNK/64 + 2];
	int simd[8];
	int prog[NBUF == 2 ? 8 : 1][64];
	static_assert(ST_CHUNK <= 512 && ST_TP <= 64, "work-list entry = pixel*512 + column in 16 bits");
	static_assert(RW % 2 == 0 && LW % 2 == 0 && WP % 2 == 0, "16-byte rows");
	static_assert(RW - R + 4 <= SRH_PADR + 1, "padded planes cover every staged piece");
};

__device__ __forceinline__ void st_dma16(const void *src, void *dst, int nbytes, int lane) {
	for (int off = 0; off < nbytes; off += 1024) {
		if (off + lane*16 < nbytes)
			__builtin_amdgcn_global_load_lds((st_gbl_void *)((const char *)src + off + lane*16),
			                                 (st_lds_void *)((char *)dst + off), 16, 0, 0);
	}
}
__device__ __forceinline__ void st_dma4(const void *src, void *dst, int nbytes, int lane) {
	for (int off = 0; off < nbytes; off += 256) {
		if (off + lane*4 < nbytes)
			__builtin_amdgcn_global_load_lds((st_gbl_void *)((const char *)src + off + lane*4),
			                                 (st_lds_void *)((char *)dst + off), 4, 0, 0);
	}
}

template <int R, int NBUF>
__device__ __noinline__ double strip_cost_general(const StripSmem<R, NBUF> &S, int wb, int s0, int i, int rc,
                                                  double weight_cutoff, double bad_ret, double max_color_diff)
{
	typedef StripSmem<R, NBUF> Smem;
	constexpr int WS = Smem::WS, NS = Smem::NS;
	double meanL = 0, meanR = 0, totalWeight = 0.0;
#pragma unroll 1
	for (int row = 0; row < WS; ++row) {
		const int sl = s0 + row >= NS ? s0 + row - NS : s0 + row;
		double gl[WS], gr[WS], wt[WS];
#pragma unroll
		for (int col = 0; col < WS; ++col) { gl[col] = S.lt[sl][i + col]; gr[col] = S.rt[sl][rc + col]; wt[col] = S.w[wb][row][i][col]; }
#pragma unroll
		for (int col = 0; col < WS; ++col) {
			const bool ok = gl[col] == gl[col] && gr[col] == gr[col] && wt[col] > weight_cutoff;
			const double pl = wt[col]*gl[col], pr = wt[col]*gr[col];
			meanL += ok ? pl : 0.0;
			meanR += ok ? pr : 0.0;
			totalWeight += ok ? wt[col] : 0.0;
		}
	}
	if (totalWeight < 1e-10) return bad_ret;
	meanL /= totalWeight;
	meanR /= totalWeight;
	double sum1 = 0, sum2 = 0, sum3 = 0;
#pragma unroll 1
	for (int row = 0; row < WS; ++row) {
		const int sl = s0 + row >= NS ? s0 + row - NS : s0 + row;
		double gl[WS], gr[WS], wt[WS];
#pragma unroll
		for (int col = 0; col < WS; ++col) { gl[col] = S.lt[sl][i + col]; gr[col] = S.rt[sl][rc + col]; wt[col] = S.w[wb][row][i][col]; }
#pragma unroll
		for (int col = 0; col < WS; ++col) {
			const bool ok = gl[col] == gl[col] && gr[col] == gr[col] && wt[col] > weight_cutoff;
			const double a = wt[col]*gl[col] - meanL;
			const double b = wt[col]*gr[col] - meanR;
			const double ab = a*b, aa = a*a, bb = b*b;
			sum1 += ok ? ab : 0.0;
			sum2 += ok ? aa : 0.0;
			sum3 += ok ? bb : 0.0;
		}
	}
	const double v = 255*(1.0 - fabs(sum1) / sqrt(sum2 * sum3));
	return (v < max_color_diff) ? v : max_color_diff;
}

template <int R, int NBUF>
__device__ __noinline__ void strip_select_block(const StripSmem<R, NBUF> &S, int wb, int s0, int pi, int rc, unsigned store,
                                                double *__restrict__ dst, double weight_cutoff, double bad_ret, double max_color_diff,
                                                int ra, int rb)
{
	typedef StripSmem<R, NBUF> Smem;
	constexpr int WS = Smem::WS, NS = Smem::NS, NCB = ST_NCB, NR = NCB + 2*R;
	double mLs[NCB], mRs[NCB], tws[NCB];
#pragma unroll
	for (int j = 0; j < NCB; ++j) { mLs[j] = 0.0; mRs[j] = 0.0; tws[j] = 0.0; }
#pragma unroll 1
	for (int row = ra; row < rb; ++row) {
		const int sl = s0 + row >= NS ? s0 + row - NS : s0 + row;
		double rr[NR], rv[NR];
		const double2 *rp = reinterpret_cast<const double2 *>((NBUF == 2 && (rc & 1)) ? &S.rto[sl][rc - 1] : &S.rt[sl][rc]);
#pragma unroll
		for (int m = 0; m < NR/2; ++m) { const double2 v = rp[m]; rr[2*m] = v.x; rr[2*m + 1] = v.y; }
#pragma unroll
		for (int m = 0; m < NR; ++m) { const bool okr = rr[m] == rr[m]; rv[m] = okr ? 1.0 : 0.0; rr[m] = okr ? rr[m] : 0.0; }
#pragma unroll
		for (int col = 0; col < WS; ++col) {
			const double gl = S.lt[sl][pi + col], wt = S.w[wb][row][pi][col];
			const bool okl = gl == gl && wt > weight_cutoff;
			const double w0 = okl ? wt : 0.0, pl0 = okl ? wt*gl : 0.0;
#pragma unroll
			for (int j = 0; j < NCB; ++j) {
				mLs[j] += pl0*rv[col + j];
				mRs[j] += w0*rr[col + j];
				tws[j] += w0*rv[col + j];
			}
		}
	}
#pragma unroll
// ... 691 lines not shown
```

Measured before the change: 47620 Mhyp/s.

## Overlap band inputs on side stream, compact lazy-fill list, fuse redo kernel

When side weights are enabled, the label table, pixel-range and scan-template kernels now run on a side stream concurrently with the weight computation, joined back by events. The pixel-range kernel also builds a compacted list of pixels that need lazy fill, using a wave ballot and one atomic per wave, so the lazy-fill kernels loop over only those pixels instead of launching over every pixel. The refill-plus-rescan pair for certified bands is replaced by a single fused redo kernel, and the old rescan wave path is removed. These changes add event synchronisation, an extra memset and atomics, and a profiling script extension.

After: 48300 Mhyp/s (median of 6 runs). 1.01x the previous value.

```diff
diff --git a/profiles/gpu_busy.py b/profiles/gpu_busy.py
--- a/profiles/gpu_busy.py
+++ b/profiles/gpu_busy.py
@@ -2,15 +2,36 @@
 import csv
 import sys
 
-rows = list(csv.DictReader(open(sys.argv[1])))
-ev = sorted((int(r["Start_Timestamp"]), int(r["End_Timestamp"]), r["Kernel_Name"].split("(")[0][-60:]) for r in rows)
-if len(sys.argv) > 4:
-    hits = [i for i, e in enumerate(ev) if sys.argv[2] in e[2]]
-    ev = ev[hits[int(sys.argv[3]) - 1] + 1: hits[int(sys.argv[4]) - 1] + 1]
+SMALL = 8
+
+argv = sys.argv[1:]
+timeline = bool(argv) and argv[0] == "--timeline"
+if timeline:
+    argv = argv[1:]
+rows = list(csv.DictReader(open(argv[0])))
+
+
+def stream_of(r):
+    return r.get("Stream_Id") or r.get("Queue_Id") or "?"
+
+
+def workgroups(r):
+    n = 1
+    for ax in "XYZ":
+        g, w = int(r.get("Grid_Size_" + ax) or 1), int(r.get("Workgroup_Size_" + ax) or 1)
+        n *= max(1, (g + w - 1)//max(1, w))
+    return n
+
+
+ev = sorted((int(r["Start_Timestamp"]), int(r["End_Timestamp"]), r["Kernel_Name"].split("(")[0][-60:], stream_of(r), workgroups(r))
+            for r in rows)
+if len(argv) > 3:
+    hits = [i for i, e in enumerate(ev) if argv[1] in e[2]]
+    ev = ev[hits[int(argv[2]) - 1] + 1: hits[int(argv[3]) - 1] + 1]
 t0 = ev[0][0]
-span = max(e for _, e, _ in ev) - t0
+span = max(e[1] for e in ev) - t0
 busy, cur, gaps = 0, t0, []
-for s, e, n in ev:
+for s, e, n, _, _ in ev:
     if s > cur:
         gaps.append((s - cur, n))
     busy += max(0, e - max(s, cur))
@@ -19,3 +40,16 @@
       f"idle {(span-busy)/1e6:.3f} ms in {len(gaps)} gaps")
 for g, n in sorted(gaps, reverse=True)[:10]:
     print(f"  gap {g/1e3:8.1f} us  before {n}")
+
+if timeline:
+    print(f"{'start us':>10} {'end us':>10} {'us':>9}  {'stream':>6} {'wgs':>7} {'beside':>6}  kernel")
+    for s, e, n, st, wg in ev:
+        beside = sum(1 for s2, e2, *_ in ev if s2 < e and e2 > s) - 1
+        print(f"{(s-t0)/1e3:10.1f} {(e-t0)/1e3:10.1f} {(e-s)/1e3:9.1f}  {st:>6} {wg:7d} {beside:6d}  {n}")
+    cuts = sorted({t for s, e, *_ in ev for t in (s, e)})
+    small_only = 0
+    for a, b in zip(cuts, cuts[1:]):
+        live = [wg for s, e, _, _, wg in ev if s <= a and e >= b]
+        if live and max(live) <= SMALL:
+            small_only += b - a
+    print(f"only dispatches of <= {SMALL} workgroups running: {small_only/1e3:.1f} us of {span/1e3:.1f} us")
diff --git a/stereoreconstruction_amd/csrc/srh_api.hip b/stereoreconstruction_amd/csrc/srh_api.hip
--- a/stereoreconstruction_amd/csrc/srh_api.hip
+++ b/stereoreconstruction_amd/csrc/srh_api.hip
@@ -144,6 +144,7 @@
 	DevBuf<double> tnum;
 	DevBuf<double> pconst;
 	DevBuf<PixRange> prange;
+	DevBuf<uint32_t> filllist;
 	DevBuf<uint32_t> cflag;
 	DevBuf<uint8_t> stpl;
 	DevBuf<uint32_t> tileflag;
@@ -154,7 +155,7 @@
 	DevBuf<uint32_t> mvs_wdesc;
 	DevBuf<int32_t> mvs_nwin;
 	template <class F> void each(F f) {
-		f(wbuf); f(cost); f(tnum); f(pconst); f(prange); f(cflag); f(stpl); f(tileflag);
+		f(wbuf); f(cost); f(tnum); f(pconst); f(prange); f(filllist); f(cflag); f(stpl); f(tileflag);
 		f(lcount); f(lcand); f(lrowinfo); f(lmeta); f(mvs_wdesc); f(mvs_nwin);
 	}
 	size_t bytes() { size_t b = 0; each([&](auto &x) { b += x.bytes(); }); return b; }
@@ -250,6 +251,7 @@
 	int mvs_cmax_hint = 0;
 	hipStream_t side_stream = nullptr;
 	hipEvent_t side_go = nullptr, side_done = nullptr;
+	hipEvent_t side_tpl = nullptr;
 	int mvs_async = 1;
 	MvsSlot mvs_slot[SRH_MVS_SLOTS];
 	int mvs_turn = 0, mvs_last = -1;
@@ -666,6 +668,7 @@
 	if (c->side_stream) { hipStreamSynchronize(c->side_stream); hipStreamDestroy(c->side_stream); }
 	if (c->side_go) hipEventDestroy(c->side_go);
 	if (c->side_done) hipEventDestroy(c->side_done);
+	if (c->side_tpl) hipEventDestroy(c->side_tpl);
 	drain_profile(c);
 	for (MvsSlot &S : c->mvs_slot) {
 		if (S.stream) hipStreamDestroy(S.stream);
@@ -1187,6 +1190,10 @@
 			fprintf(stderr, "[srh prof] geodesic kernel: %llu waves, cycles per wave: staging %.0f  sweeps %.0f  exp %.0f  rows out %.0f  pconst: first sweep %.0f  second sweep %.0f  rest %.0f\n",
 			        g[7], (double)g[0]/g[7], (double)g[1]/g[7], (double)g[2]/g[7], (double)g[4]/g[7], (double)g[5]/g[7], (double)g[6]/g[7], (double)g[3]/g[7]);
 	}
+	if (h.dbg_redo[4])
+		fprintf(stderr, "[srh prof] redo kernel: %llu pixels, cycles per pixel (first wave): projections + mask %.0f  walk %.0f  wait for the columns %.0f  "
+		        "running minimum %.0f | second wave: columns %.0f\n", h.dbg_redo[4], (double)h.dbg_redo[0]/h.dbg_redo[4], (double)h.dbg_redo[1]/h.dbg_redo[4],
+		        (double)h.dbg_redo[2]/h.dbg_redo[4], (double)h.dbg_redo[3]/h.dbg_redo[4], (double)h.dbg_redo[5]/h.dbg_redo[4]);
 	if (h.dbg_waves && h.dbg_blocks && h.dbg_phase[3] && h.strip_ticket) {
 		const double nw = (double)h.dbg_waves, nt = (double)h.dbg_blocks/nw;
 		fprintf(stderr, "[srh dbg] strip: waves %llu, tiles/wave %.1f (%.1f with phase 2), cycles/wave %.0f | per tile: ticket %.0f  own requests %.0f  barriers %.0f  setup %.0f  "
@@ -1383,7 +1390,8 @@
 
 struct TvPlan { bool dense = false; int cstride = 0; bool fused = false; };
 struct TvLists { int cmax = 0, smax = 0; bool rows_mode = false, guessed = false, cert = false; size_t lrows = 0; };
-struct TvDense { int cstride = 0; bool strip = false, cert = false, tscan = false; size_t rows = 0; int lanes = 8; };
+struct TvDense { int cstride = 0; bool strip = false, cert = false, tscan = false; size_t rows = 0; int lanes = 8;
+                 bool tables_pending = false, tpl_wait = false; };
 
 struct TvPass {
 	srh_context *c = nullptr;
@@ -1403,7 +1411,9 @@
 	int lists_pass(TvLists &S) const;
 	int run_lists(bool cert_ok, srh_context::TvDefer *defer) const;
 	int dense_prepare(TvDense &D) const;
-	void dense_band_inputs(const TvDense &D, int by, int nr) const;
+	void dense_tables(const TvDense &D, bool table, bool tpl) const;
+	bool dense_fill_padded(const TvDense &D, int arith) const;
+	int dense_band_inputs(TvDense &D, int by, int nr, int arith) const;
 	int dense_cost_pass(const TvDense &D, int by, int nr, int arith, bool raw) const;
 	int run_dense(TvDense &D) const;
 	int run_walk() const;
@@ -1698,13 +1708,10 @@
 	int rc;
 	D.tscan = c->tscan != 0;
 	if ((rc = c->band.tnum.ensure((size_t)p->num_depth_levels + 8))) return rc;
-	{ Scope s(c, "pinhole_label_table_kernel");
-	  launch_pinhole_label_table(c->stream, c->d_views, ref, *p, false, c->band.tnum); }
-	if (D.tscan) {
-		if ((rc = c->band.stpl.ensure(scan_template_bytes()))) return rc;
-		Scope s(c, "twoview_template_kernel");
-		launch_scan_template(c->stream, c->d_views, ref, oth, *p, y0, y1 - y0, c->band.tnum, c->band.stpl);
-	}
+	if (D.tscan && (rc = c->band.stpl.ensure(scan_template_bytes()))) return rc;
+	D.tables_pending = c->side_weights != 0;
+	D.tpl_wait = false;
+	if (!D.tables_pending) dense_tables(D, true, true);
 	for (int pass = 0; pass < 2; ++pass) {
 		const int wdoubles = D.strip ? (2*R + 1)*wimg_wp(R) : T;
 		D.rows = rows_per_band((size_t)wdoubles*sizeof(double) + (size_t)D.cstride*sizeof(double));
@@ -1716,6 +1723,7 @@
 	if ((rc = c->band.cost.ensure(rows*(size_t)((W + 31)/32)*32*(size_t)D.cstride))) return rc;
 	if ((rc = c->band.pconst.ensure((rows*(size_t)W + SRH_WTILE)*SRH_PC))) return rc;
 	if ((rc = c->band.prange.ensure(rows*(size_t)W + SRH_WTILE))) return rc;
+	if (!sad && (rc = c->band.filllist.ensure(rows*(size_t)W + 1))) return rc;
 	if (D.tscan && (rc = c->band.tileflag.ensure(rows*(size_t)((W + 63)/64) + 1))) return rc;
 	if (D.cert && (rc = c->band.cflag.ensure(rows*(size_t)W + 1))) return rc;
 	D.lanes = D.strip ? strip_block_lanes(D.cstride, c->strip == 1 ? 0 : c->strip) : 8;
@@ -1734,10 +1742,55 @@
 	return SRH_OK;
 }
 
-void TvPass::dense_band_inputs(const TvDense &D, int by, int nr) const {
+void TvPass::dense_tables(const TvDense &D, bool table, bool tpl) const {
+	if (table) {
+		Scope s(c, "pinhole_label_table_kernel");
+		launch_pinhole_label_table(c->stream, c->d_views, ref, *p, false, c->band.tnum);
+	}
+	if (tpl && D.tscan) {
+		Scope s(c, "twoview_template_kernel");
+		launch_scan_template(c->stream, c->d_views, ref, oth, *p, y0, y1 - y0, c->band.tnum, c->band.stpl);
+	}
+}
+
+bool TvPass::dense_fill_padded(const TvDense &D, int arith) const { return D.strip ? D.lanes == 8 : arith != 5; }
+
+int TvPass::dense_band_inputs(TvDense &D, int by, int nr, int arith) const {
+	uint32_t *filllist = sad ? nullptr : (uint32_t *)c->band.filllist;
+	const bool side = c->side_weights != 0;
+	if (side) {
+		if (!c->side_stream) {
+			HIP_TRY(hipStreamCreateWithFlags(&c->side_stream, hipStreamNonBlocking));
+			HIP_TRY(hipEventCreateWithFlags(&c->side_go, hipEventDisableTiming));
+			HIP_TRY(hipEventCreateWithFlags(&c->side_done, hipEventDisableTiming));
+		}
+		if (!c->side_tpl) HIP_TRY(hipEventCreateWithFlags(&c->side_tpl, hipEventDisableTiming));
+		HIP_TRY(hipEventRecord(c->side_go, c->stream));
+	}
 	run_weights(c, ref, W, *p, by, nr, SRH_WTILE, !sad ? (double *)c->band.pconst : nullptr, D.strip);
-	Scope s(c, "pixel_range_kernel");
-	launch_pixel_range(c->stream, c->d_views, ref, oth, W, *p, by, nr, c->band.tnum, D.cstride, c->band.prange);
+	const bool tables = side && D.tables_pending;
+	D.tables_pending = false;
+	if (side) {
+		HIP_TRY(hipStreamWaitEvent(c->side_stream, c->side_go, 0));
+		std::swap(c->stream, c->side_stream);
+		if (tables) dense_tables(D, true, false);
+	}
+	hipError_t e = filllist ? hipMemsetAsync(filllist, 0, sizeof(uint32_t), c->stream) : hipSuccess;
+	{ Scope s(c, "pixel_range_kernel");
+	  launch_pixel_range(c->stream, c->d_views, ref, oth, W, *p, by, nr, c->band.tnum, D.cstride, c->band.prange,
+	                     D.lanes, dense_fill_padded(D, arith), filllist); }
+	if (side) {
+		if (e == hipSuccess) e = hipEventRecord(c->side_done, c->stream);
+		if (tables && D.tscan) {
+			dense_tables(D, false, true);
+			if (e == hipSuccess) e = hipEventRecord(c->side_tpl, c->stream);
+			D.tpl_wait = true;
+		}
+		std::swap(c->stream, c->side_stream);
+		if (e == hipSuccess) e = hipStreamWaitEvent(c->stream, c->side_done, 0);
+	}
+	if (e != hipSuccess) return fail(SRH_E_DEVICE, "dense band inputs: %s", hipGetErrorString(e));
+	return SRH_OK;
 }
 
 int TvPass::dense_cost_pass(const TvDense &D, int by, int nr, int arith, bool raw) const {
@@ -1767,8 +1820,8 @@
 			                          c->band.tnum, c->band.cost, cstride, c->d_cnt, c->band.pconst, arith, c->band.prange); }
 	}
 	Scope s(c, "twoview_lazy_fill_kernel");
-	launch_twoview_lazy_fill(c->stream, c->d_views, ref, oth, W, *p, by, nr, c->band.prange, c->band.wbuf, wstride, c->views[ref].tvp,
-	                         c->views[oth].tvp, D.strip, D.lanes, D.strip ? D.lanes == 8 : arith != 5, c->band.cost, cstride, c->d_cnt);
+	launch_twoview_lazy_fill(c->stream, c->d_views, ref, oth, W, *p, by, nr, c->band.prange, c->band.filllist, c->band.wbuf, wstride, c->views[ref].tvp,
+	                         c->views[oth].tvp, D.strip, D.lanes, dense_fill_padded(D, arith), c->band.cost, cstride, c->d_cnt);
 	return SRH_OK;
 }
 
@@ -1779,20 +1832,27 @@
 	for (int by = y0; by < y1; by += (int)D.rows) {
 		if (cancelled(c)) return fail(SRH_E_CANCELLED, "cancelled");
 		const int nr = std::min((int)D.rows, y1 - by);
-		dense_band_inputs(D, by, nr);
+		if ((rc = dense_band_inputs(D, by, nr, cost_arith))) return rc;
 		if (D.cert) HIP_TRY(hipMemsetAsync(c->band.cflag, 0, sizeof(uint32_t), c->stream));
 		if ((rc = dense_cost_pass(D, by, nr, cost_arith, false))) return rc;
+		if (D.tpl_wait) { HIP_TRY(hipStreamWaitEvent(c->stream, c->side_tpl, 0)); D.tpl_wait = false; }
 		{ Scope s(c, "twoview_scan_kernel");
 		  launch_twoview_scan(c->stream, c->d_views, ref, oth, W, *p, by, nr, c->band.tnum, c->band.cost, D.cstride, c->d_cnt, c->band.prange,
 		                      D.cert ? c->band.cflag : nullptr, -1, D.cert && D.strip ? c->band.pconst : nullptr, D.tscan ? c->band.stpl : nullptr, c->band.tileflag, c->num_cus, wout, c->tscan_bound); }
 		if (D.cert) {
 			const int cap = redo_capacity((size_t)nr*W);
-			{ Scope s(c, "twoview_refill_kernel");
-			  launch_twoview_refill(c->stream, W, *p, by, c->band.prange, c->band.cflag, cap, c->band.wbuf, D.strip, c->views[ref].tvp,
-			                        c->views[oth].tvp, c->band.cost, D.cstride, c->d_cnt); }
-			Scope s(c, "twoview_rescan_kernel");
-			launch_twoview_scan(c->stream, c->d_views, ref, oth, W, *p, by, nr, c->band.tnum, c->band.cost, D.cstride, c->d_cnt, c->band.prange,
-			                    c->band.cflag, cap, nullptr, nullptr, nullptr, c->num_cus, wout);
+			if (twoview_redo_takes(*p, D.cstride)) {
+				Scope s(c, "twoview_redo_kernel");
+				launch_twoview_redo(c->stream, c->d_views, ref, oth, W, *p, by, c->band.tnum, c->band.wbuf, D.strip, c->views[ref].tvp,
+				                    c->views[oth].tvp, c->band.cost, D.cstride, c->band.prange, c->band.cflag, cap, c->d_cnt, wout);
+			} else {
+				{ Scope s(c, "twoview_refill_kernel");
+				  launch_twoview_refill(c->stream, W, *p, by, c->band.prange, c->band.cflag, cap, c->band.wbuf, D.strip, c->views[ref].tvp,
+				                        c->views[oth].tvp, c->band.cost, D.cstride, c->d_cnt); }
+				Scope s(c, "twoview_rescan_kernel");
+				launch_twoview_scan(c->stream, c->d_views, ref, oth, W, *p, by, nr, c->band.tnum, c->band.cost, D.cstride, c->d_cnt, c->band.prange,
+				                    c->band.cflag, cap, nullptr, nullptr, nullptr, c->num_cus, wout);
+			}
 		}
 		winner_costs(by, nr, D.strip);
 	}
@@ -1912,7 +1972,7 @@
 	if ((rc = P.dense_prepare(D))) return rc;
 	if (cancelled(c)) return fail(SRH_E_CANCELLED, "cancelled");
 	const int nr = std::min((int)D.rows, P.y1 - P.y0);
-	P.dense_band_inputs(D, P.y0, nr);
+	if ((rc = P.dense_band_inputs(D, P.y0, nr, form))) return rc;
 	if (nr != P.y1 - P.y0) return fail(SRH_E_UNSUPPORTED, "cost rows: the rows asked for do not fit one band (%d of %d)", nr, P.y1 - P.y0);
 	if (cost_out) {
 		const size_t nd = (size_t)nr*((P.W + 31)/32)*32*(size_t)D.cstride;
diff --git a/stereoreconstruction_amd/csrc/srh_dense.hip b/stereoreconstruction_amd/csrc/srh_dense.hip
--- a/stereoreconstruction_amd/csrc/srh_dense.hip
+++ b/stereoreconstruction_amd/csrc/srh_dense.hip
@@ -1256,29 +1256,29 @@
 #endif
 #define SC_MW 1024
 
+#define LF_BLOCKS 512
 __global__ void twoview_lazy_fill_kernel(const ViewDev *__restrict__ views, int ref, int oth, srh_params P, int y0, int nrows,
-                                         const PixRange *__restrict__ prange, const double *__restrict__ wbuf, size_t wstride,
+                                         const PixRange *__restrict__ prange, const uint32_t *__restrict__ filllist,
+                                         const double *__restrict__ wbuf, size_t wstride,
                                          int ncb, int lanes, int pad, double *__restrict__ cost, int cstride, Counters *__restrict__ cnt)
 {
+	const uint32_t nfill = filllist[0];
+	if (nfill == 0) return;
 	const ViewDev &L = views[ref];
 	const ViewDev &Rv = views[oth];
 	const int W = L.w;
-	const size_t q = (size_t)blockIdx.x*blockDim.x + threadIdx.x;
 	unsigned n_lazy = 0;
-	if (q < (size_t)nrows*W) {
-		const int x = (int)(q % W), trow = (int)(q / W), y = y0 + trow;
+	for (uint32_t f = blockIdx.x*blockDim.x + threadIdx.x; f < nfill; f += gridDim.x*blockDim.x) {
+		const uint32_t q = filllist[1 + f];
+		const int x = (int)(q % (uint32_t)W), trow = (int)(q / (uint32_t)W), y = y0 + trow;
 		const PixRange pr = prange[q];
-		if (pr.hi >= pr.lo) {
-			const int cover = dense_cover_hi(pr.lo, pr.hi, ncb, lanes, pad != 0);
-			if (cover < pr.hi) {
-				const int R = P.window_radius, T = (2*R + 1)*(2*R + 1);
-				const double *wq = wbuf + wbuf_offset(W, T, trow, x);
-				double *crow = cost + ((size_t)trow*((W + DC_TP - 1)/DC_TP) + (x/DC_TP))*(size_t)cstride*DC_TP + (x % DC_TP);
-				for (int c = cover + 1; c <= pr.hi; ++c) {
-					crow[(size_t)(c - pr.lo)*DC_TP] = tv_cost(L, Rv, wq, wstride, P, x, y, c, y);
-					++n_lazy;
-				}
-			}
+		const int cover = dense_cover_hi(pr.lo, pr.hi, ncb, lanes, pad != 0);
+		const int R = P.window_radius, T = (2*R + 1)*(2*R + 1);
+		const double *wq = wbuf + wbuf_offset(W, T, trow, x);
+		double *crow = cost + ((size_t)trow*((W + DC_TP - 1)/DC_TP) + (x/DC_TP))*(size_t)cstride*DC_TP + (x % DC_TP);
+		for (int c = cover + 1; c <= pr.hi; ++c) {
+			crow[(size_t)(c - pr.lo)*DC_TP] = tv_cost(L, Rv, wq, wstride, P, x, y, c, y);
+			++n_lazy;
 		}
 	}
 	block_count_add(&cnt->n_eval_device, n_lazy);
@@ -1287,26 +1287,27 @@
 template <int R>
 __global__ __launch_bounds__(256)
 void twoview_lazy_fill_planes_kernel(int W, srh_params P, int y0, int nrows, const PixRange *__restrict__ prange,
+                                     const uint32_t *__restrict__ filllist,
                                      const double *__restrict__ wbuf, int wimg, const double *__restrict__ ref_tvp,
                                      const double *__restrict__ oth_tvp, int ncb, int lanes, int pad,
                                      double *__restrict__ cost, int cstride, Counters *__restrict__ cnt)
 {
-	const size_t q = (size_t)blockIdx.x*blockDim.x + threadIdx.x;
+	const uint32_t nfill = filllist[0];
+	if (nfill == 0) return;
 	unsigned n_lazy = 0;
-	if (q < (size_t)nrows*W) {
-		const int x = (int)(q % W), trow = (int)(q / W), y = y0 + trow;
+	for (uint32_t f = blockIdx.x*blockDim.x + threadIdx.x; f < nfill; f += gridDim.x*blockDim.x) {
+		const uint32_t q = filllist[1 + f];
+		const int x = (int)(q % (uint32_t)W), trow = (int)(q / (uint32_t)W), y = y0 + trow;
 		const PixRange pr = prange[q];
-		const int cover = pr.hi >= pr.lo ? dense_cover_hi(pr.lo, pr.hi, ncb, lanes, pad != 0) : pr.hi;
-		if (cover < pr.hi) {
-			const int SP = padded_stride(W);
-			const WindowAt wa = window_at<R>(wbuf, wimg, W, trow, x);
-			const double *lp = ref_tvp + (size_t)(y + SRH_PADY - R)*SP + (x + SRH_PADL - R);
-			double *crow = cost + ((size_t)trow*((W + DC_TP - 1)/DC_TP) + (x/DC_TP))*(size_t)cstride*DC_TP + (x % DC_TP);
-			for (int c = cover + 1; c <= pr.hi; ++c) {
-				const double *rp = oth_tvp + (size_t)(y + SRH_PADY - R)*SP + (c + SRH_PADL - R);
-				crow[(size_t)(c - pr.lo)*DC_TP] = window_exact_cost<R>(wa.wq, wa.wrow, wa.wcol, lp, rp, SP, SP, P);
-				++n_lazy;
-			}
+		const int cover = dense_cover_hi(pr.lo, pr.hi, ncb, lanes, pad != 0);
+		const int SP = padded_stride(W);
+		const WindowAt wa = window_at<R>(wbuf, wimg, W, trow, x);
+		const double *lp = ref_tvp + (size_t)(y + SRH_PADY - R)*SP + (x + SRH_PADL - R);
+		double *crow = cost + ((size_t)trow*((W + DC_TP - 1)/DC_TP) + (x/DC_TP))*(size_t)cstride*DC_TP + (x % DC_TP);
+		for (int c = cover + 1; c <= pr.hi; ++c) {
+			const double *rp = oth_tvp + (size_t)(y + SRH_PADY - R)*SP + (c + SRH_PADL - R);
+			crow[(size_t)(c - pr.lo)*DC_TP] = window_exact_cost<R>(wa.wq, wa.wrow, wa.wcol, lp, rp, SP, SP, P);
+			++n_lazy;
 		}
 	}
 	block_count_add(&cnt->n_eval_device, n_lazy);
@@ -1351,19 +1352,19 @@
 }
 
 void launch_twoview_lazy_fill(hipStream_t st, const ViewDev *views, int ref, int oth, int width, const srh_params &P,
-                              int y0, int nrows, const PixRange *prange, const double *wbuf, size_t wstride,
+                              int y0, int nrows, const PixRange *prange, const uint32_t *filllist, const double *wbuf, size_t wstride,
                               const double *ref_tvp, const double *oth_tvp, bool wimg,
                               int lanes, bool padded, double *cost, int cstride, Counters *cnt)
 {
 	const size_t n = (size_t)nrows*width;
-	const dim3 grid((unsigned)((n + 255)/256)), block(256);
+	const dim3 grid((unsigned)std::min<size_t>((n + 255)/256, LF_BLOCKS)), block(256);
 	const int pad = padded ? 1 : 0;
 	if (ref_tvp && P.window_radius == 5)
-		hipLaunchKernelGGL(twoview_lazy_fill_planes_kernel<5>, grid, block, 0, st, width, P, y0, nrows, prange, wbuf, wimg ? 1 : 0, ref_tvp, oth_tvp, 8, lanes, pad, cost, cstride, cnt);
+		hipLaunchKernelGGL(twoview_lazy_fill_planes_kernel<5>, grid, block, 0, st, width, P, y0, nrows, prange, filllist, wbuf, wimg ? 1 : 0, ref_tvp, oth_tvp, 8, lanes, pad, cost, cstride, cnt);
 	else if (ref_tvp && P.window_radius == 2)
-		hipLaunchKernelGGL(twoview_lazy_fill_planes_kernel<2>, grid, block, 0, st, width, P, y0, nrows, prange, wbuf, wimg ? 1 : 0, ref_tvp, oth_tvp, 8, lanes, pad, cost, cstride, cnt);
+		hipLaunchKernelGGL(twoview_lazy_fill_planes_kernel<2>, grid, block, 0, st, width, P, y0, nrows, prange, filllist, wbuf, wimg ? 1 : 0, ref_tvp, oth_tvp, 8, lanes, pad, cost, cstride, cnt);
 	else
-		hipLaunchKernelGGL(twoview_lazy_fill_kernel, grid, block, 0, st, views, ref, oth, P, y0, nrows, prange, wbuf, wstride, 8, lanes, pad, cost, cstride, cnt);
+		hipLaunchKernelGGL(twoview_lazy_fill_kernel, grid, block, 0, st, views, ref, oth, P, y0, nrows, prange, filllist, wbuf, wstride, 8, lanes, pad, cost, cstride, cnt);
 }
 
 __device__ __forceinline__ unsigned wave_sum_u32(unsigned v) {
@@ -1968,23 +1969,35 @@
 
 #define RSW_MAXD 1024
 #define RSW_MAXC 6144
-template <bool WTA>
-__global__ __launch_bounds__(64)
-void twoview_rescan_wave_kernel(const ViewDev *__restrict__ views, int ref, int oth, srh_params P, int y0,
-                                const double *__restrict__ tnum, const double *__restrict__ cost, int cstride,
-                                const PixRange *__restrict__ prange, const uint32_t *__restrict__ cflag, int cap,
-                                Counters *__restrict__ cnt, int32_t *__restrict__ wout)
+#define RD_THREADS 512
+#define RD_GRID 512
+template <int R, bool WTA>
+__global__ __launch_bounds__(RD_THREADS)
+void twoview_redo_kernel(const ViewDev *__restrict__ views, int ref, int oth, srh_params P, int y0,
+                         const double *__restrict__ tnum, const double *__restrict__ wbuf, int wimg,
+                         const double *__restrict__ ref_tvp, const double *__restrict__ oth_tvp,
+                         double *__restrict__ cost, int cstride,
+                         const PixRange *__restrict__ prange, const uint32_t *__restrict__ cflag, int cap,
+                         Counters *__restrict__ cnt, int32_t *__restrict__ wout)
 {
 	const ViewDev &L = views[ref];
 	const ViewDev &Rv = views[oth];
 	const int W = L.w, OW = Rv.w, OH = Rv.h;
-	const int lane = threadIdx.x;
+	const int tid = threadIdx.x;
 	__shared__ double sx[RSW_MAXD], sy[RSW_MAXD];
 	__shared__ unsigned short scol[RSW_MAXC];
-	__shared__ double scost[RSW_MAXC];
+	__shared__ double srow[4096];
 	__shared__ unsigned char smask[4096 + 64];
 	__shared__ int s_n;
 	const uint32_t nflag = cflag[0];
+	if (blockIdx.x == 0 && tid == 0 && nflag > (uint32_t)cap) atomicAdd(&cnt->cert_overflow, 1ull);
+	unsigned n_cols = 0;
+#ifdef SRH_PROFILE_PHASES
+	unsigned long long rph[6] = {0, 0, 0, 0, 0, 0}, rt = __builtin_readcyclecounter();
+#define RD_STAMP(k) do { const unsigned long long tn_ = __builtin_readcyclecounter(); rph[k] += tn_ - rt; rt = tn_; } while (0)
+#else
+#define RD_STAMP(k)
+#endif
 	for (uint32_t f = blockIdx.x; f < nflag && f < (uint32_t)cap; f += gridDim.x) {
 		const uint32_t q = cflag[1 + f];
 		const int x = (int)(q % (uint32_t)W), trow = (int)(q / (uint32_t)W), y = y0 + trow;
@@ -1996,7 +2009,7 @@
 		const bool walk = !(fabs(nd) < 1e-10);
 		if (walk) {
 			const SharedDivisor nd_sd = shared_divisor(nd);
-			for (int d = lane; d < P.num_depth_levels; d += 64) {
+			for (int d = tid; d < P.num_depth_levels; d += RD_THREADS) {
 				double x2, y2;
 				const bool ok = pinhole_project_label_sd(ray, nd_sd, tnum[d], Rv.cam, P.image_scale, x2, y2);
 				sx[d] = ok ? x2 : __builtin_nan("");
@@ -2004,9 +2017,11 @@
 			}
 		}
 		const int span = hi >= lo ? hi - lo + 1 : 0;
-		for (int k = lane; k < span && k < 4096; k += 64) smask[k] = (y >= 0 && y < OH) ? Rv.mask[(size_t)y*OW + lo + k] : 0;
+		for (int k = tid; k < span && k < 4096; k += RD_THREADS) smask[k] = (y >= 0 && y < OH) ? Rv.mask[(size_t)y*OW + lo + k] : 0;
 		__syncthreads();
-		if (lane == 0) {
+		RD_STAMP(0);
+		double *crow = cost + ((size_t)trow*((W + DC_TP - 1)/DC_TP) + (x/DC_TP))*(size_t)cstride*DC_TP + (x % DC_TP);
+		if (tid == 0) {
 			int n = 0;
 			bool over = false;
 			if (walk) {
@@ -2044,17 +2059,27 @@
 			}
 			if (over) { atomicAdd(&cnt->cert_overflow, 1ull); n = RSW_MAXC; }
 			s_n = n;
-		}
+		} else if (tid >= 64) {
+			const int SP = padded_stride(W);
+			const WindowAt wa = window_at<R>(wbuf, wimg, W, trow, x);
+			const double *lp = ref_tvp + (size_t)(y + SRH_PADY - R)*SP + (x + SRH_PADL - R);
+			for (int c = lo + (tid - 64); c <= hi; c += RD_THREADS - 64) {
+				const double *rp = oth_tvp + (size_t)(y + SRH_PADY - R)*SP + (c + SRH_PADL - R);
+				const double cv = window_exact_cost<R>(wa.wq, wa.wrow, wa.wcol, lp, rp, SP, SP, P);
+				crow[(size_t)(c - lo)*DC_TP] = cv;
+				if (c - lo < 4096) srow[c - lo] = cv;
+				++n_cols;
+			}
+		}
+		RD_STAMP(1);
 		__syncthreads();
-		const int n = s_n;
-		const double *crow = cost + ((size_t)trow*((W + DC_TP - 1)/DC_TP) + (x/DC_TP))*(size_t)cstride*DC_TP + (x % DC_TP);
-		for (int k = lane; k < n; k += 64) scost[k] = crow[(size_t)scol[k]*DC_TP];
-		__syncthreads();
-		if (lane == 0) {
+		RD_STAMP(2);
+		if (tid == 0) {
+			const int n = s_n;
 			double minCost = __builtin_inf(), secondBest = __builtin_inf();
 			int wcol = -1, pcol = -1;
 			for (int k = 0; k < n; ++k) {
-				const double cv = scost[k];
+				const double cv = srow[scol[k]];
 				if (cv + P.wta_margin < minCost) { secondBest = minCost; minCost = cv; if (WTA) pcol = wcol; wcol = scol[k]; }
 			}
 			double depth = __builtin_nan("");
@@ -2065,7 +2090,36 @@
 			                   pcol >= 0 ? lo + pcol : -1, pcol >= 0 ? y : -1);
 		}
 		__syncthreads();
-	}
+		RD_STAMP(3);
+#ifdef SRH_PROFILE_PHASES
+		++rph[4];
+#endif
+	}
+#ifdef SRH_PROFILE_PHASES
+	if (tid == 0) for (int k = 0; k < 5; ++k) atomicAdd(&cnt->dbg_redo[k], rph[k]);
+	if (tid == 64) atomicAdd(&cnt->dbg_redo[5], rph[1]);
+#endif
+#undef RD_STAMP
+	block_count_add(&cnt->n_eval_device, n_cols);
+}
+
+bool twoview_redo_takes(const srh_params &P, int cstride) {
+	return P.num_depth_levels <= RSW_MAXD && cstride <= 4096 && (P.window_radius == 5 || P.window_radius == 2);
+}
+
+bool launch_twoview_redo(hipStream_t st, const ViewDev *views, int ref, int oth, int width, const srh_params &P, int y0,
+                         const double *tnum, const double *wbuf, bool wimg, const double *ref_tvp, const double *oth_tvp,
+                         double *cost, int cstride, const PixRange *prange, const uint32_t *cflag, int cap, Counters *cnt, int32_t *wout)
+{
+	if (!twoview_redo_takes(P, cstride)) return false;
+	if (cap <= 0) return true;
+	const dim3 grid((unsigned)(cap < RD_GRID ? cap : RD_GRID)), block(RD_THREADS);
+#define SRH_REDO(R_, W_) hipLaunchKernelGGL((twoview_redo_kernel<R_, W_>), grid, block, 0, st, views, ref, oth, P, y0, tnum, wbuf, wimg ? 1 : 0, \
+                                            ref_tvp, oth_tvp, cost, cstride, prange, cflag, cap, cnt, wout)
+	if (P.window_radius == 5) { if (wout) SRH_REDO(5, true); else SRH_REDO(5, false); }
+	else                      { if (wout) SRH_REDO(2, true); else SRH_REDO(2, false); }
+#undef SRH_REDO
+	return true;
 }
 
 void launch_scan_template(hipStream_t st, const ViewDev *views, int ref, int oth, const srh_params &P, int y0, int nrows,
@@ -2100,12 +2154,6 @@
 		if (tp) { if (wout) SRH_TSCAN(true, true, cflag, pexact); else SRH_TSCAN(true, false, cflag, pexact); }
 		if (wout) SRH_SCAN(true, false, true, wgrid, cflag, 0, pexact, tilelist);
 		else      SRH_SCAN(true, false, false, wgrid, cflag, 0, pexact, tilelist);
-	} else if (nlist > 0 && P.num_depth_levels <= RSW_MAXD && cstride <= 4096) {
-		const dim3 rgrid((unsigned)(nlist < 2048 ? nlist : 2048));
-		if (wout) hipLaunchKernelGGL(twoview_rescan_wave_kernel<true>, rgrid, dim3(64), 0, st,
-		                             views, ref, oth, P, y0, tnum, cost, cstride, prange, cflag, nlist, cnt, wout);
-		else      hipLaunchKernelGGL(twoview_rescan_wave_kernel<false>, rgrid, dim3(64), 0, st,
-		                             views, ref, oth, P, y0, tnum, cost, cstride, prange, cflag, nlist, cnt, wout);
 	} else if (nlist > 0) {
 		const unsigned lgrid = (unsigned)((nlist + SC_TW - 1)/SC_TW);
 		if (wout) SRH_SCAN(false, true, true, lgrid, cflag, nlist, nullptr, nullptr);
diff --git a/stereoreconstruction_amd/csrc/srh_internal.hpp b/stereoreconstruction_amd/csrc/srh_internal.hpp
--- a/stereoreconstruction_amd/csrc/srh_internal.hpp
+++ b/stereoreconstruction_amd/csrc/srh_internal.hpp
@@ -125,6 +125,7 @@
 	unsigned long long dbg_cycles, dbg_blocks, dbg_total_cycles, dbg_waves;
 	unsigned long long dbg_phase[8];
 	unsigned long long dbg_wave[64];
+	unsigned long long dbg_redo[6];
 };
 
 #define SRH_MAX_NEIGH 8
@@ -186,8 +187,12 @@
                           const double *tnum, void *tpl);
 bool launch_twoview_refill(hipStream_t st, int width, const srh_params &P, int y0, const PixRange *prange, const uint32_t *cflag, int cap,
                            const double *wbuf, bool wimg, const double *ref_tvp, const double *oth_tvp, double *cost, int cstride, Counters *cnt);
+bool twoview_redo_takes(const srh_params &P, int cstride);
+bool launch_twoview_redo(hipStream_t st, const ViewDev *views, int ref, int oth, int width, const srh_params &P, int y0,
+                         const double *tnum, const double *wbuf, bool wimg, const double *ref_tvp, const double *oth_tvp,
+                         double *cost, int cstride, const PixRange *prange, const uint32_t *cflag, int cap, Counters *cnt, int32_t *wout);
 void launch_twoview_lazy_fill(hipStream_t st, const ViewDev *views, int ref, int oth, int width, const srh_params &P,
-                              int y0, int nrows, const PixRange *prange, const double *wbuf, size_t wstride,
+                              int y0, int nrows, const PixRange *prange, const uint32_t *filllist, const double *wbuf, size_t wstride,
                               const double *ref_tvp, const double *oth_tvp,
                               bool wimg,
                               int lanes, bool padded,
@@ -196,7 +201,9 @@
 void launch_padded_plane(hipStream_t st, const double *gray_tv, int w, int h, double *out);
 void launch_padded_full(hipStream_t st, const double *gray_tv, int w, int h, int R, uint8_t *out);
 void launch_pixel_range(hipStream_t st, const ViewDev *views, int ref, int oth, int width, const srh_params &P,
-                        int y0, int nrows, const double *tnum, int cstride, PixRange *prange);
+                        int y0, int nrows, const double *tnum, int cstride, PixRange *prange,
+                        int lanes = 8, bool padded = true,
+                        uint32_t *filllist = nullptr);
 int  strip_chunk_columns();
 int  strip_block_lanes(int cstride, int form);
 bool launch_twoview_strip_cost(hipStream_t st, const ViewDev *views, int ref, int oth, int width, int height,
diff --git a/stereoreconstruction_amd/csrc/srh_strip.hip b/stereoreconstruction_amd/csrc/srh_strip.hip
--- a/stereoreconstruction_amd/csrc/srh_strip.hip
+++ b/stereoreconstruction_amd/csrc/srh_strip.hip
@@ -60,28 +60,41 @@
 }
 
 __global__ void pixel_range_kernel(const ViewDev *__restrict__ views, int ref, int oth, srh_params P, int y0, int nrows,
-                                   const double *__restrict__ tnum, int cstride, PixRange *__restrict__ prange)
+                                   const double *__restrict__ tnum, int cstride, PixRange *__restrict__ prange,
+                                   int ncb, int lanes, int pad, uint32_t *__restrict__ filllist)
 {
 	const ViewDev &L = views[ref];
 	const int W = L.w;
 	const size_t q = (size_t)blockIdx.x*blockDim.x + threadIdx.x;
-	if (q >= (size_t)nrows*W) return;
-	const int x = (int)(q % W), y = y0 + (int)(q / W);
+	const bool in = q < (size_t)nrows*W;
 	int lo = 0, hi = -1;
-	if (L.mask[(size_t)y*W + x] == 1) {
-		const Ray ray = cam_unproject(L.cam, (x + 0.5) / P.image_scale, (y + 0.5) / P.image_scale);
-		pinhole_column_range(ray, L.cam, views[oth], P, tnum, cstride, lo, hi);
-	}
-	PixRange r; r.lo = lo; r.hi = hi;
-	prange[q] = r;
+	if (in) {
+		const int x = (int)(q % W), y = y0 + (int)(q / W);
+		if (L.mask[(size_t)y*W + x] == 1) {
+			const Ray ray = cam_unproject(L.cam, (x + 0.5) / P.image_scale, (y + 0.5) / P.image_scale);
+			pinhole_column_range(ray, L.cam, views[oth], P, tnum, cstride, lo, hi);
+		}
+		PixRange r; r.lo = lo; r.hi = hi;
+		prange[q] = r;
+	}
+	if (!filllist) return;
+	const bool left = in && hi >= lo && dense_cover_hi(lo, hi, ncb, lanes, pad != 0) < hi;
+	const unsigned long long m = __ballot(left);
+	if (m == 0) return;
+	const int lane = (int)(threadIdx.x & 63), leader = __ffsll((long long)m) - 1;
+	unsigned base = 0;
+	if (lane == leader) base = atomicAdd(&filllist[0], (unsigned)__popcll(m));
+	base = (unsigned)__shfl((int)base, leader);
+	if (left) filllist[1 + base + (unsigned)__popcll(m & ((1ull << lane) - 1ull))] = (uint32_t)q;
 }
 
 void launch_pixel_range(hipStream_t st, const ViewDev *views, int ref, int oth, int width, const srh_params &P,
-                        int y0, int nrows, const double *tnum, int cstride, PixRange *prange)
+                        int y0, int nrows, const double *tnum, int cstride, PixRange *prange,
+                        int lanes, bool padded, uint32_t *filllist)
 {
 	const size_t n = (size_t)nrows*width;
 	hipLaunchKernelGGL(pixel_range_kernel, dim3((unsigned)((n + 255)/256)), dim3(256), 0, st,
-	                   views, ref, oth, P, y0, nrows, tnum, cstride, prange);
+	                   views, ref, oth, P, y0, nrows, tnum, cstride, prange, 8, lanes, padded ? 1 : 0, filllist);
 }
 
 int strip_chunk_columns() { return ST_CHUNK; }
```
